# showlab/UniVTG

Measured on NVIDIA H100. Metric: video-query pairs/sec (fwd+bwd), higher is better.
Workload: dtype f16

## Files before the change

### __graft_entry__.py

```python
import os
import shutil
import subprocess
import sys

ROOT = os.path.dirname(os.path.abspath(__file__))
CSRC = os.path.join(ROOT, "univtg_b200", "csrc")
LIBDIR = os.path.join(ROOT, "univtg_b200", "lib")
LIB = os.path.join(LIBDIR, "libunivtg_b200.so")
SOURCES = ["gemm.cu", "rowops.cu", "attention.cu", "attention_bwd.cu", "backward.cu", "loss.cu", "optim.cu", "postproc.cu", "train.cu", "api.cu", "clip.cu",
           "hostio.cu", "metrics.cu", "task_eval.cu", "teacher.cu"]

NVCC_FLAGS = [
    "-gencode", "arch=compute_90a,code=sm_90a",
    "-lineinfo", "-O3", "-std=c++17",
    "-Xcompiler", "-fPIC",
    "--expt-relaxed-constexpr",
]


def _nvcc():
    for cand in (shutil.which("nvcc"), "/usr/local/cuda/bin/nvcc"):
        if cand and os.path.exists(cand):
            return cand
    raise RuntimeError("nvcc not found: the univtg_b200 CUDA library cannot be built")


def _needs_rebuild(srcs):
    if not os.path.exists(LIB):
        return True
    t = os.path.getmtime(LIB)
    deps = list(srcs)
    for f in os.listdir(CSRC):
        if f.endswith((".h", ".cuh")):
            deps.append(os.path.join(CSRC, f))
    deps.append(os.path.join(ROOT, "include", "univtg_b200.h"))
    return any(os.path.getmtime(d) > t for d in deps)


def build(force=False, verbose=False):
    srcs = [os.path.join(CSRC, s) for s in SOURCES if os.path.exists(os.path.join(CSRC, s))]
    if force or _needs_rebuild(srcs):
        os.makedirs(LIBDIR, exist_ok=True)
        nvcc = _nvcc()
        objs = []
        procs = []
        for s in srcs:
            o = os.path.join(LIBDIR, os.path.basename(s) + ".o")
            objs.append(o)
            cmd = [nvcc] + NVCC_FLAGS + ["-c", s, "-o", o]
            if verbose:
                cmd.insert(1, "-Xptxas")
                cmd.insert(2, "-v")
            procs.append((cmd, subprocess.Popen(cmd, stdout=subprocess.PIPE, stderr=subprocess.STDOUT, text=True)))
        for cmd, p in procs:
            out, _ = p.communicate()
            if verbose or p.returncode != 0:
                sys.stdout.write(out)
            if p.returncode != 0:
                raise RuntimeError("nvcc failed: " + " ".join(cmd))
        link = [nvcc, "-shared", "-gencode", "arch=compute_90a,code=sm_90a", "-o", LIB] + objs
        subprocess.check_call(link)
        for o in objs:
            os.remove(o)
    sys.path.insert(0, ROOT)
    import univtg_b200

    univtg_b200.load_library()


def smoke():
    sys.path.insert(0, ROOT)
    import torch

    assert torch.cuda.is_available(), "smoke() needs a GPU"
    from oracle import univtg_oracle as O
    from univtg_b200 import build_model, synth
    from univtg_b200.optim import FlatAdamW

    cfg = dict(synth.CONFIGS["tiny"], nheads=2, hidden_dim=256)
    args = synth.reference_args(cfg, device="cuda:0")
    model, crit = build_model(args)
    sd = synth.make_state_dict(cfg, seed=3)
    model.load_state_dict(sd, strict=True)
    model.to("cuda:0").eval()
    crit.to("cuda:0")
    inp = synth.make_inputs(cfg, seed=4, ragged=True)
    cinp = {k: v.cuda() for k, v in inp.items()}
    with torch.no_grad():
        out = model(**cinp)
    torch.cuda.synchronize()
    emu = O.forward(sd, cfg, **inp, opq=O.round_fp16)
    exact = O.forward(sd, cfg, **inp)
    for k in ("pred_logits", "pred_spans", "saliency_scores"):
        got = out[k].double().cpu()
        torch.testing.assert_close(got, emu[k], rtol=1e-4, atol=2e-5, msg=lambda m: f"smoke {k} vs fp16-emulating oracle: {m}")
        torch.testing.assert_close(got, exact[k], rtol=1e-3, atol=1e-4, msg=lambda m: f"smoke {k} vs exact oracle: {m}")

    tgt = synth.make_targets(inp, seed=5)
    ctgt = {k: (v.cuda() if torch.is_tensor(v) else v) for k, v in tgt.items()}
    model.train()
    crit.train()
    model.reference_rng_order = True
    model.keep_last_draw = True
    opt = FlatAdamW(model, lr=1e-3, weight_decay=1e-2, max_grad_norm=0.1)
    before = [p.detach().clone() for p in model._abi_params()]
    torch.manual_seed(11)
    tout = model(**cinp)
    loss = crit(tout, ctgt)
    total = crit.weighted_total(loss)
    opt.zero_grad()
    total.backward()
    grads = [p.grad.detach().clone() for p in model._abi_params()]
    opt.step()
    torch.cuda.synchronize()
    scales, masks = model._last_draw
    leaves = {k: v.double().requires_grad_(True) for k, v in sd.items()}
    oout = O.forward(leaves, cfg, **inp, dp_scale=scales.cpu(), drop_masks=[m.cpu() for m in masks])
    oloss = O.criterion(oout, tgt)
    O.weighted_total(oloss, crit.weight_dict).backward()
    for k, v in oloss.items():
        assert abs(float(loss[k]) - float(v)) <= 2e-3 * max(1.0, abs(float(v))), f"smoke train {k}: {float(loss[k])} vs oracle {float(v)}"
    named = dict(model.named_parameters())
    for n_ in ("transformer.encoder.layers.1.linear1.weight", "transformer.encoder.layers.0.self_attn.in_proj_weight",
               "input_vid_proj.0.net.1.weight", "span_embed.layers.1.weight", "class_embed.layers.2.weight"):
        g, og = named[n_].grad.double().cpu(), leaves[n_].grad
        rel = float((g - og).norm() / og.norm())
        assert rel < 8e-2, f"smoke train gradient {n_}: rel-L2 {rel:.3e} vs oracle autograd"
    ref_params = [b.clone().requires_grad_(True) for b in before]
    for rp, g in zip(ref_params, grads):
        rp.grad = g.clone()
    torch.nn.utils.clip_grad_norm_(ref_params, 0.1)
    ref_opt = torch.optim.AdamW(ref_params, lr=1e-3, weight_decay=1e-2)
    ref_opt.step()
    for p, rp in zip(model._abi_params(), ref_params):
        torch.testing.assert_close(p.detach(), rp.detach(), rtol=2e-5, atol=2e-7, msg=lambda m: f"smoke AdamW update: {m}")
    print("smoke ok:", {k: tuple(v.shape) for k, v in out.items()}, "train losses", {k: round(float(v), 5) for k, v in loss.items()})


if __name__ == "__main__":
    build(force="--force" in sys.argv, verbose="-v" in sys.argv)
    print("built", LIB)
```

### include/univtg_b200.h

```cpp
#ifndef UNIVTG_B200_H_
#define UNIVTG_B200_H_

#include <stddef.h>
#include <stdint.h>

#ifdef __cplusplus
extern "C" {
#endif

#define UNIVTG_ABI_VERSION 2
#define UNIVTG_ADAMW_SCRATCH_FLOATS 2048

typedef struct univtg_config {
  int32_t hidden_dim;
  int32_t nheads;
  int32_t dim_feedforward;
  int32_t enc_layers;
  int32_t n_input_proj;
  int32_t v_feat_dim;
  int32_t t_feat_dim;
  int32_t operand_format;
} univtg_config;

typedef struct univtg_shape {
// ... 48 lines not shown
  const float* table;
  int32_t max_q_l;
  const float* ln_weight;
  const float* ln_bias;
  const float* drop_mul;
  void* scratch;
} univtg_txt_pos;
int univtg_plan_set_txt_pos(univtg_plan* plan, const univtg_txt_pos* txt_pos);
size_t univtg_txt_pos_scratch_bytes(const univtg_config* cfg, const univtg_shape* shape);

int univtg_backward(univtg_plan* plan, void* train_ws, const float* src_txt, const float* src_vid, const float* droppath_scale,
                    const float* const* drop_masks, const univtg_rng* rng, const float* g_logits, const float* g_spans,
                    const float* g_vid_mem_proj, const float* g_txt_mem_proj, float grad_scale, float* const* grads,
                    int32_t n_grads, void* stream);

int univtg_backward_stages(const univtg_config* cfg, int32_t* ranges, int32_t max_stages);
int univtg_plan_set_backward_sm_budget(univtg_plan* plan, int32_t num_sms);
int univtg_plan_set_grad_events(univtg_plan* plan, void* const* events, int32_t n);

size_t univtg_loss_scratch_bytes(int32_t B, int32_t Lv);
int univtg_loss_forward(const float* pred_logits, const float* pred_spans, const float* vid_mem_proj, const float* txt_mem_proj,
                        const float* timestamp, const float* timestamp_mask, const float* timestamp_window,
                        const float* span_labels_nn, const float* saliency_scores, const int64_t* saliency_pos_idx, int32_t B,
                        int32_t Lv, int32_t d, float eos_coef, float temperature, float* losses5, void* scratch, void* stream);
int univtg_loss_backward(const float* w5, const float* vid_mem_proj, const float* txt_mem_proj, const int64_t* saliency_pos_idx,
                         int32_t B, int32_t Lv, int32_t d, const void* scratch, float* d_logits, float* d_spans,
                         float* d_vid_mem_proj, float* d_txt_mem_proj, void* stream);

int univtg_qfvs_loss_forward(const float* pred_logits, const float* vid_mem_proj, const float* txt_mem_proj, const float* src_vid_mask,
                             const uint8_t* mask_gt, const float* saliency_scores, int32_t has_pos_labels, int32_t B, int32_t Lv,
                             int32_t d, float temperature, float* losses5, void* scratch, void* stream);
int univtg_qfvs_loss_backward(const float* w5, const float* vid_mem_proj, const float* txt_mem_proj, int32_t B, int32_t Lv,
                              int32_t d, void* scratch, float* d_logits, float* d_vid_mem_proj, float* d_txt_mem_proj, void* stream);

int univtg_forward_num_launches(const univtg_plan* plan);
int64_t univtg_launch_count(void);

int univtg_plan_set_profiling(univtg_plan* plan, int32_t enable);
int univtg_plan_read_profile(univtg_plan* plan, float* ms, int32_t* kinds, int32_t cap);


int univtg_op_gemm(const void* a, const void* b, int32_t M, int32_t N, int32_t K, int32_t a_mn, int32_t b_mn, int32_t fmt,
                   int32_t bn, int32_t ksplit, const float* bias, int32_t act, float alpha, float* out32, void* out16,
                   void* stream);
int univtg_op_gemm_cluster(const void* a, const void* b, int32_t M, int32_t N, int32_t K, int32_t a_mn, int32_t b_mn,
                           int32_t fmt, int32_t bn, int32_t ksplit, const float* bias, int32_t act, float alpha, float* out32,
                           void* out16, void* stream);
typedef struct univtg_gemm_problem {
  const void* a;
  int32_t lda, a_mn;
  const void* b;
  int32_t ldb, b_mn;
  int32_t M, N, K, ksplit;
  int32_t a_fmt, b_fmt, out_fmt;
  int32_t conv, tap;
  const float* bias;
  int32_t act;
  float alpha;
  const float* row_scale;
  int32_t rps_in, rps_out, row_off, zero_sep, skip_sep;
  const float* resid;
  int32_t ld_resid;
  const float* addtab;
  int32_t ld_addtab;
  float* out32;
  int32_t ld32;
  float* out32_id;
  int32_t ld32_id;
  void* out16;
  void* out16p;
  int32_t ld16, accumulate;
  const void* mask16;
  int32_t ld_mask, mask_mul;
  void* dact16;
  int32_t ld_dact;
  float* colsum;
  float colsum_scale;
  int32_t vec_ok;
} univtg_gemm_problem;
int univtg_op_gemm_group(univtg_gemm_problem* problems, int32_t num, int32_t fmt, int32_t bn, int32_t cluster, int32_t* full,
                         void* stream);

typedef struct univtg_ln_bwd {
  const float* dout;
  int32_t ld_dout;
  const float* y;
  int32_t ld_y;
  const void* y16;
  int32_t y_fmt;
  const float* mean;
  const float* rstd;
  const float* gamma;
  int32_t rows, d;
  const float* row_scale;
  int32_t L, relu_mask_y;
  float* dy32;
  void* dbr16;
  int32_t ld16, fmt16;
  float* dgamma;
  float* dbeta;
  float* colsum;
  float pgrad_scale;
  const float* dout_mul;
} univtg_ln_bwd;
int univtg_op_layernorm_bwd(const univtg_ln_bwd* args, const univtg_rng* rng, int32_t mask_index, int32_t* kernel_used, void* stream);

typedef struct univtg_head_final_bwd {
  const float* g_logits;
  const float* g_spans;
  const float* pred_logits;
  const float* pred_spans;
  const void* h_cls;
  const void* h_span;
  const float* w_cls;
  const float* w_span;
  float* dz;
  void* dh_cls;
  void* dh_span;
  float* gw_cls;
  float* gb_cls;
  float* gw_span;
  float* gb_span;
  float* cs_cls;
  float* cs_span;
  float in_scale, pgrad_scale;
  int32_t B, Lv, d, fmt_act, fmt_grad;
} univtg_head_final_bwd;
int univtg_op_head_final_bwd(const univtg_head_final_bwd* args, void* stream);
int univtg_op_colsum16(const void* in16, int32_t ld, int32_t rows, int32_t cols, int32_t fmt, float* colsum, float scale, void* txt16,
                       int32_t L, int32_t Lv, int32_t txt_cols, void* stream);
int univtg_op_cvt16_colsum(const float* in32, int32_t ld_in, void* out16, int32_t ld_out, int32_t rows, int32_t cols, int32_t fmt,
                           float* colsum, float colsum_scale, void* txt16, int32_t L, int32_t Lv, int32_t txt_cols, void* stream);
int univtg_op_stream_gather(const float* dx, int32_t L, int32_t off, const float* extra, float extra_scale, void* out16, float* colsum,
                            float colsum_scale, int32_t B, int32_t Ls, int32_t d, int32_t fmt, void* stream);
int univtg_op_pool_bwd(const float* x_txt, const float* alpha, const float* w, const float* g_pooled, float* dx_txt, float* gw,
                       float out_scale, int32_t B, int32_t Lt, int32_t d, void* stream);
typedef struct univtg_txt_pos_bwd {
  const float* dpos;
  const float* xt;
  const float* table;
  const float* gamma;
  const float* mean;
  const float* rstd;
  const float* mul32;
  float* dx;
  float* dtable;
  float* dgamma;
  float* dbeta;
  float pgrad_scale;
  int32_t B, Lt, L, Lv, d;
} univtg_txt_pos_bwd;
int univtg_op_txt_pos_bwd(const univtg_txt_pos_bwd* args, const univtg_rng* rng, int32_t mask_index, void* stream);
int univtg_debug_gemm_timeline(void* buf);
int univtg_debug_choose_tile(const int32_t* Ms, const int32_t* Ns, const int32_t* kblocks, int32_t num, int32_t num_sms, int32_t step,
                             int32_t max_split, int32_t* bn, int32_t* ksplit);
int univtg_adamw_step(float* params, float* grads, float* exp_avg, float* exp_avg_sq, size_t n, float lr, float beta1,
                      float beta2, float eps, float weight_decay, int32_t step, float max_grad_norm,
                      int32_t write_clipped_grads, float* scratch3, const univtg_config* cfg, void* packed, void* stream);
int univtg_adamw_step_dev(float* params, float* grads, float* exp_avg, float* exp_avg_sq, size_t n, const float* lr_dev,
                          float beta1, float beta2, float eps, float weight_decay, int32_t* step_dev, float max_grad_norm,
                          int32_t write_clipped_grads, float* scratch3, const univtg_config* cfg, void* packed,
                          const float* bc_table, int32_t table_len, void* stream);
int univtg_adamw_bias_table(float beta1, float beta2, int32_t len, float* out_host);
int32_t univtg_adamw_bias_table_len(float beta1, float beta2);
int univtg_pack_vectors(const univtg_config* cfg, const float* const* params, int32_t n_params, void* packed, void* stream);

int univtg_host_assemble_batch(void* dst_vid, void* dst_txt, float* dst_vmask, float* dst_tmask, const void* src_vid,
                               const void* src_txt, const int64_t* vid_row0, const int64_t* txt_row0, const int32_t* vid_len,
                               const int32_t* txt_len, int32_t B, int32_t Lv, int32_t Lt, int32_t Dv, int32_t Dt, int32_t threads);

int univtg_host_register(void* base, size_t bytes, int32_t enable);
int univtg_h2d_gather_batch(void* dev_vid, void* dev_txt, float* dev_vmask, float* dev_tmask, float* mask_stage, const void* src_vid,
                            const void* src_txt, const int64_t* vid_row0, const int64_t* txt_row0, const int32_t* vid_len,
                            const int32_t* txt_len, int32_t B, int32_t Lv, int32_t Lt, int32_t Dv, int32_t Dt, void* stream);

int univtg_decode_mr(const float* pred_logits, const float* pred_spans, const float* timestamp, const float* timestamp_mask,
                     const float* duration, int32_t B, int32_t Lv, int32_t sort, float* windows, double* windows_r4, int32_t* order,
                     void* stream);
int univtg_temporal_nms(const double* windows, int32_t B, int32_t n, int32_t max_before_nms, double nms_thd, int32_t max_after_nms,
                        double* out, int32_t* counts, void* stream);

int univtg_eval_mr(const double* pred, const int32_t* n_pred, const double* gt, const int32_t* n_gt, int32_t Q, int32_t G, double* ap,
                   double* iou_r1, double* iou_r5, uint8_t* kept, void* stream);
int univtg_eval_hl(const double* sal, const int32_t* n_sal, const uint16_t* labels, const int32_t* n_clips, int32_t Q, int32_t S,
                   int32_t C, double* scratch, double* ap, double* hit, void* stream);

int univtg_eval_hl_topk(const float* scores, const int32_t* n_score, const int32_t* n_cut, const float* labels,
                        const int32_t* n_label, int32_t V, int32_t S, int32_t C, int32_t A, int32_t median, double* ap,
                        void* stream);
int univtg_qfvs_match(const uint64_t* a, const int32_t* a_off, const uint64_t* b, const int32_t* b_off, int32_t Q,
                      int32_t max_side, double* s, void* stream);

int univtg_op_layernorm(const float* in, int32_t rows, int32_t d, const float* gamma, const float* beta, float eps,
                        int32_t fmt, float* out32, void* out16, int32_t ld16, void* stream);
int univtg_op_attention(const void* qkv, const float* key_mask, void* out, float* lse, int32_t B, int32_t L, int32_t H,
                        int32_t dh, int32_t fmt, int32_t impl, void* stream);

typedef struct univtg_ln_fwd {
  const float* in;
  const void* in16;
  int32_t in_fmt, ld_in;
  const void* add16;
  int32_t ld_add16;
  float* sum_out;
  int32_t rows, d;
  const float* gamma;
  const float* beta;
  float eps;
  int32_t fmt;
  int64_t lo;
  int32_t L, Lv;
  float* out32;
  void* out16;
  void* out16p;
  int32_t ld16;
  const float* pos;
  const float* pos_txt;
  void* outc;
  const float* mul32;
  float* mean_out;
  float* rstd_out;
} univtg_ln_fwd;
int univtg_op_layernorm_fwd(const univtg_ln_fwd* args, const univtg_rng* rng, int32_t mask_index, int32_t* kernel_used, void* stream);

typedef struct univtg_txt_pos_fwd {
  const float* xt;
  const float* table;
  const float* gamma;
  const float* beta;
  const float* mul32;
  float* pos;
  float* mean_out;
  float* rstd_out;
  void* xpos16;
  int32_t B, Lt, L, Lv, d, fmt;
  int64_t lo;
} univtg_txt_pos_fwd;
int univtg_op_txt_pos(const univtg_txt_pos_fwd* args, const univtg_rng* rng, int32_t mask_index, void* stream);

int univtg_op_sine_pos(const float* vid_mask, const float* txt_mask, const float* dim_t, float* pos, float* key_mask, int32_t B, int32_t Lv,
                       int32_t Lt, int32_t d, const univtg_rng* rng, int32_t n_sites, float* dp_out, void* stream);

int univtg_op_pool_saliency(const float* x_txt, const float* x_vid, const float* txt_mask, const float* vid_mask, const float* w,
                            float* pooled, float* saliency, float* alpha_out, float* logits, int32_t B, int32_t Lt, int32_t Lv, int32_t d,
                            void* stream);

int univtg_op_conv_head_final(const void* h_cls, const void* h_span, const float* w_cls, const float* w_span, const float* b_cls,
                              const float* b_span, float* pred_logits, float* pred_spans, int32_t B, int32_t Lv, int32_t d, int32_t fmt,
                              void* stream);

typedef struct univtg_attn_fwd {
  const void* qkv;
  const float* key_mask;
  void* out;
  float* lse;
  int32_t B, L, H, dh, fmt, impl, causal;
} univtg_attn_fwd;
int univtg_op_attention_fwd(const univtg_attn_fwd* args, const univtg_rng* rng, float p, int32_t layer, int32_t* kernel_used, void* stream);

int univtg_op_attention_bwd(const void* qkv, const void* dO, const void* O, const float* key_mask, const float* lse,
                            float* delta_ws, float* dqkv32, int32_t B, int32_t L, int32_t H, int32_t dh, int32_t fmt_act,
                            int32_t impl, void* stream);

int univtg_op_attn_delta(const void* dO, int32_t fmt_do, const void* O, int32_t fmt_o, float* delta, int32_t B, int32_t L, int32_t H,
                         int32_t dh, int32_t* vec_used, void* stream);

typedef struct univtg_attn_bwd {
  const void* qkv;
  const void* dO;
  const float* key_mask;
  const float* lse;
  const float* delta;
  float* dqkv32;
  void* dqkv16;
  int32_t B, L, H, dh, fmt, impl;
} univtg_attn_bwd;
int univtg_op_attention_bwd_full(const univtg_attn_bwd* args, const univtg_rng* rng, float p, int32_t layer, int32_t* kernel_used,
                                 int32_t* dq_mode, void* stream);

typedef struct univtg_clip_config {
  int32_t embed_dim;
  int32_t vision_width;
  int32_t vision_layers;
  int32_t patch_size;
  int32_t image_resolution;
  int32_t text_width;
  int32_t text_layers;
  int32_t context_length;
  int32_t vocab_size;
  int32_t operand_format;
} univtg_clip_config;
int univtg_clip_num_params(const univtg_clip_config* cfg);
size_t univtg_clip_packed_bytes(const univtg_clip_config* cfg);
int univtg_clip_pack_weights(const univtg_clip_config* cfg, const void* const* params, int32_t n_params, int32_t src_dtype,
                             void* packed, void* stream);
size_t univtg_clip_workspace_bytes(const univtg_clip_config* cfg, int32_t n_images, int32_t n_texts, int32_t text_len);
int univtg_clip_encode_image(const univtg_clip_config* cfg, const void* packed, const void* pixels, int32_t pixel_kind, int32_t n,
                             void* ws, size_t ws_bytes, float* out, void* stream);
int univtg_clip_encode_text(const univtg_clip_config* cfg, const void* packed, const int64_t* tokens, int32_t n, int32_t ctx_used,
                            void* ws, size_t ws_bytes, float* last_hidden, float* pooled, void* stream);
int univtg_clip_num_launches(const univtg_clip_config* cfg, int32_t tower, int32_t text_outputs);

size_t univtg_teacher_class_bytes(int32_t C, int32_t D);
int univtg_teacher_prepare_classes(const float* cls, int32_t C, int32_t D, void* cls_ws, void* stream);
size_t univtg_teacher_chunk_bytes(int32_t V, int64_t S, int32_t C, int32_t D);
int univtg_teacher_label(const float* cls, const void* cls_ws, int32_t C, int32_t D, const float* feats, const int32_t* offsets,
// ... 8 lines not shown
```

### univtg_b200/_lib.py

```python
import ctypes
import os

_HERE = os.path.dirname(os.path.abspath(__file__))
LIB_PATH = os.environ.get("UNIVTG_LIB") or os.path.join(_HERE, "lib", "libunivtg_b200.so")
_lib = None

c_int = ctypes.c_int32
c_void_p = ctypes.c_void_p
c_size_t = ctypes.c_size_t
c_float = ctypes.c_float


class Config(ctypes.Structure):

    _fields_ = [
        ("hidden_dim", c_int),
        ("nheads", c_int),
        ("dim_feedforward", c_int),
        ("enc_layers", c_int),
        ("n_input_proj", c_int),
        ("v_feat_dim", c_int),
        ("t_feat_dim", c_int),
        ("operand_format", c_int),
    ]
# ... 7 lines not shown
class Rng(ctypes.Structure):

    _fields_ = [("seed", ctypes.c_uint64), ("input_dropout", c_float), ("droppath", c_float)]


class TxtPos(ctypes.Structure):

    _fields_ = [("table", c_void_p), ("max_q_l", c_int), ("ln_weight", c_void_p), ("ln_bias", c_void_p), ("drop_mul", c_void_p),
                ("scratch", c_void_p)]


class GemmProblem(ctypes.Structure):

    _fields_ = [("a", c_void_p), ("lda", c_int), ("a_mn", c_int), ("b", c_void_p), ("ldb", c_int), ("b_mn", c_int), ("M", c_int),
                ("N", c_int), ("K", c_int), ("ksplit", c_int), ("a_fmt", c_int), ("b_fmt", c_int), ("out_fmt", c_int), ("conv", c_int),
                ("tap", c_int), ("bias", c_void_p), ("act", c_int), ("alpha", c_float), ("row_scale", c_void_p), ("rps_in", c_int),
                ("rps_out", c_int), ("row_off", c_int), ("zero_sep", c_int), ("skip_sep", c_int), ("resid", c_void_p),
                ("ld_resid", c_int), ("addtab", c_void_p), ("ld_addtab", c_int), ("out32", c_void_p), ("ld32", c_int),
                ("out32_id", c_void_p), ("ld32_id", c_int), ("out16", c_void_p), ("out16p", c_void_p), ("ld16", c_int),
                ("accumulate", c_int), ("mask16", c_void_p), ("ld_mask", c_int), ("mask_mul", c_int), ("dact16", c_void_p),
                ("ld_dact", c_int), ("colsum", c_void_p), ("colsum_scale", c_float), ("vec_ok", c_int)]


class LnBwd(ctypes.Structure):

    _fields_ = [("dout", c_void_p), ("ld_dout", c_int), ("y", c_void_p), ("ld_y", c_int), ("y16", c_void_p), ("y_fmt", c_int),
                ("mean", c_void_p), ("rstd", c_void_p), ("gamma", c_void_p), ("rows", c_int), ("d", c_int), ("row_scale", c_void_p),
                ("L", c_int), ("relu_mask_y", c_int), ("dy32", c_void_p), ("dbr16", c_void_p), ("ld16", c_int), ("fmt16", c_int),
                ("dgamma", c_void_p), ("dbeta", c_void_p), ("colsum", c_void_p), ("pgrad_scale", c_float), ("dout_mul", c_void_p)]


class HeadFinalBwd(ctypes.Structure):

    _fields_ = [(n, c_void_p) for n in ("g_logits", "g_spans", "pred_logits", "pred_spans", "h_cls", "h_span", "w_cls", "w_span", "dz",
                                        "dh_cls", "dh_span", "gw_cls", "gb_cls", "gw_span", "gb_span", "cs_cls", "cs_span")] + \
        [("in_scale", c_float), ("pgrad_scale", c_float), ("B", c_int), ("Lv", c_int), ("d", c_int), ("fmt_act", c_int), ("fmt_grad", c_int)]


class TxtPosBwd(ctypes.Structure):

    _fields_ = [(n, c_void_p) for n in ("dpos", "xt", "table", "gamma", "mean", "rstd", "mul32", "dx", "dtable", "dgamma", "dbeta")] + \
        [("pgrad_scale", c_float), ("B", c_int), ("Lt", c_int), ("L", c_int), ("Lv", c_int), ("d", c_int)]


class LnFwd(ctypes.Structure):

    _fields_ = [("in_", c_void_p), ("in16", c_void_p), ("in_fmt", c_int), ("ld_in", c_int), ("add16", c_void_p), ("ld_add16", c_int),
                ("sum_out", c_void_p), ("rows", c_int), ("d", c_int), ("gamma", c_void_p), ("beta", c_void_p), ("eps", c_float),
                ("fmt", c_int), ("lo", ctypes.c_int64), ("L", c_int), ("Lv", c_int), ("out32", c_void_p), ("out16", c_void_p),
                ("out16p", c_void_p), ("ld16", c_int), ("pos", c_void_p), ("pos_txt", c_void_p), ("outc", c_void_p), ("mul32", c_void_p),
                ("mean_out", c_void_p), ("rstd_out", c_void_p)]


class TxtPosFwd(ctypes.Structure):

    _fields_ = [(n, c_void_p) for n in ("xt", "table", "gamma", "beta", "mul32", "pos", "mean_out", "rstd_out", "xpos16")] + \
        [(n, c_int) for n in ("B", "Lt", "L", "Lv", "d", "fmt")] + [("lo", ctypes.c_int64)]


class AttnFwd(ctypes.Structure):

    _fields_ = [("qkv", c_void_p), ("key_mask", c_void_p), ("out", c_void_p), ("lse", c_void_p)] + \
        [(n, c_int) for n in ("B", "L", "H", "dh", "fmt", "impl", "causal")]


class AttnBwd(ctypes.Structure):

    _fields_ = [(n, c_void_p) for n in ("qkv", "dO", "key_mask", "lse", "delta", "dqkv32", "dqkv16")] + \
        [(n, c_int) for n in ("B", "L", "H", "dh", "fmt", "impl")]


class ClipConfig(ctypes.Structure):

    _fields_ = [(n, c_int) for n in ("embed_dim", "vision_width", "vision_layers", "patch_size", "image_resolution", "text_width",
                                     "text_layers", "context_length", "vocab_size", "operand_format")]


SIGNATURES = {
    "univtg_last_error": (ctypes.c_char_p, []),
    "univtg_abi_version": (c_int, []),
    "univtg_num_params": (c_int, [ctypes.POINTER(Config)]),
    "univtg_packed_bytes": (c_size_t, [ctypes.POINTER(Config)]),
    "univtg_pack_weights": (c_int, [ctypes.POINTER(Config), ctypes.POINTER(c_void_p), c_int, c_void_p, c_void_p]),
    "univtg_workspace_bytes": (c_size_t, [ctypes.POINTER(Config), ctypes.POINTER(Shape)]),
    "univtg_prepare_workspace": (c_int, [ctypes.POINTER(Config), ctypes.POINTER(Shape), c_void_p, c_int, c_void_p]),
    "univtg_plan_create": (c_int, [ctypes.POINTER(Config), ctypes.POINTER(Shape), c_void_p, c_void_p, c_void_p, c_void_p,
                                   ctypes.POINTER(c_void_p)]),
    "univtg_plan_destroy": (None, [c_void_p]),
    "univtg_forward": (c_int, [c_void_p] * 12),
    "univtg_forward_num_launches": (c_int, [c_void_p]),
    "univtg_launch_count": (ctypes.c_int64, []),
    "univtg_host_register": (c_int, [c_void_p, c_size_t, c_int]),
    "univtg_h2d_gather_batch": (c_int, [c_void_p] * 11 + [c_int, c_int, c_int, c_int, c_int, c_void_p]),
    "univtg_host_assemble_batch": (c_int, [c_void_p, c_void_p, c_void_p, c_void_p, c_void_p, c_void_p, c_void_p, c_void_p, c_void_p,
                                           c_void_p, c_int, c_int, c_int, c_int, c_int, c_int]),
    "univtg_train_workspace_bytes": (c_size_t, [ctypes.POINTER(Config), ctypes.POINTER(Shape)]),
    "univtg_forward_train": (c_int, [c_void_p, c_void_p, c_void_p, c_void_p, c_void_p, c_void_p, c_void_p,
                                     ctypes.POINTER(c_void_p), ctypes.POINTER(Rng), c_void_p, c_void_p, c_void_p, c_void_p, c_void_p,
                                     c_void_p]),
    "univtg_backward": (c_int, [c_void_p, c_void_p, c_void_p, c_void_p, c_void_p, ctypes.POINTER(c_void_p), ctypes.POINTER(Rng),
                                c_void_p, c_void_p, c_void_p, c_void_p, c_float, ctypes.POINTER(c_void_p), c_int, c_void_p]),
    "univtg_dropout_mask": (c_int, [ctypes.POINTER(Rng), c_int, c_size_t, c_size_t, c_void_p, c_void_p]),
    "univtg_droppath_scales": (c_int, [ctypes.POINTER(Rng), c_int, c_int, c_void_p, c_void_p]),
    "univtg_plan_set_attention_dropout": (c_int, [c_void_p, c_float]),
    "univtg_plan_set_txt_pos": (c_int, [c_void_p, ctypes.POINTER(TxtPos)]),
    "univtg_txt_pos_scratch_bytes": (c_size_t, [ctypes.POINTER(Config), ctypes.POINTER(Shape)]),
    "univtg_attention_dropout_mask": (c_int, [ctypes.POINTER(Rng), c_float, c_int, c_int, c_int, c_int, c_void_p, c_void_p]),
    "univtg_loss_scratch_bytes": (c_size_t, [c_int, c_int]),
    "univtg_loss_forward": (c_int, [c_void_p] * 10 + [c_int, c_int, c_int, c_float, c_float, c_void_p, c_void_p, c_void_p]),
    "univtg_loss_backward": (c_int, [c_void_p, c_void_p, c_void_p, c_void_p, c_int, c_int, c_int, c_void_p, c_void_p, c_void_p,
                                     c_void_p, c_void_p, c_void_p]),
    "univtg_qfvs_loss_forward": (c_int, [c_void_p] * 6 + [c_int, c_int, c_int, c_int, c_float, c_void_p, c_void_p, c_void_p]),
    "univtg_qfvs_loss_backward": (c_int, [c_void_p, c_void_p, c_void_p, c_int, c_int, c_int, c_void_p, c_void_p, c_void_p, c_void_p,
                                          c_void_p]),
    "univtg_backward_stages":(c_int, [ctypes.POINTER(Config), c_void_p, c_int]),
    "univtg_plan_set_grad_events": (c_int, [c_void_p, ctypes.POINTER(c_void_p), c_int]),
    "univtg_plan_set_backward_sm_budget": (c_int, [c_void_p, c_int]),
    "univtg_decode_mr": (c_int, [c_void_p, c_void_p, c_void_p, c_void_p, c_void_p, c_int, c_int, c_int, c_void_p, c_void_p, c_void_p,
                                 c_void_p]),
    "univtg_temporal_nms": (c_int, [c_void_p, c_int, c_int, c_int, ctypes.c_double, c_int, c_void_p, c_void_p, c_void_p]),
    "univtg_eval_mr": (c_int, [c_void_p] * 4 + [c_int, c_int] + [c_void_p] * 5),
    "univtg_eval_hl": (c_int, [c_void_p] * 4 + [c_int, c_int, c_int] + [c_void_p] * 4),
    "univtg_eval_hl_topk": (c_int, [c_void_p] * 5 + [c_int] * 5 + [c_void_p, c_void_p]),
    "univtg_qfvs_match": (c_int, [c_void_p] * 4 + [c_int, c_int, c_void_p, c_void_p]),
    "univtg_adamw_step": (c_int, [c_void_p, c_void_p, c_void_p, c_void_p, ctypes.c_size_t, c_float, c_float, c_float, c_float,
                                  c_float, c_int, c_float, c_int, c_void_p, ctypes.POINTER(Config), c_void_p, c_void_p]),
    "univtg_pack_vectors": (c_int, [ctypes.POINTER(Config), ctypes.POINTER(c_void_p), c_int, c_void_p, c_void_p]),
    "univtg_adamw_step_dev": (c_int, [c_void_p, c_void_p, c_void_p, c_void_p, ctypes.c_size_t, c_void_p, c_float, c_float, c_float,
                                      c_float, c_void_p, c_float, c_int, c_void_p, ctypes.POINTER(Config), c_void_p, c_void_p, c_int,
                                      c_void_p]),
    "univtg_adamw_bias_table": (c_int, [c_float, c_float, c_int, c_void_p]),
    "univtg_adamw_bias_table_len": (c_int, [c_float, c_float]),
    "univtg_plan_set_seed_source": (c_int, [c_void_p, c_void_p]),
    "univtg_rng_advance": (c_int, [ctypes.c_uint64, c_void_p, c_void_p, c_void_p]),
    "univtg_rng_seed_at": (ctypes.c_uint64, [ctypes.c_uint64, ctypes.c_uint64]),
    "univtg_plan_set_profiling": (c_int, [c_void_p, c_int]),
    "univtg_plan_set_input_format": (c_int, [c_void_p, c_int]),
    "univtg_plan_read_profile": (c_int, [c_void_p, c_void_p, c_void_p, c_int]),
    "univtg_op_gemm": (c_int, [c_void_p, c_void_p, c_int, c_int, c_int, c_int, c_int, c_int, c_int, c_int, c_void_p, c_int,
                               c_float, c_void_p, c_void_p, c_void_p]),
    "univtg_op_gemm_cluster": (c_int, [c_void_p, c_void_p, c_int, c_int, c_int, c_int, c_int, c_int, c_int, c_int, c_void_p, c_int,
                                       c_float, c_void_p, c_void_p, c_void_p]),
    "univtg_op_gemm_group": (c_int, [ctypes.POINTER(GemmProblem), c_int, c_int, c_int, c_int, c_void_p, c_void_p]),
    "univtg_op_layernorm_bwd": (c_int, [ctypes.POINTER(LnBwd), ctypes.POINTER(Rng), c_int, c_void_p, c_void_p]),
    "univtg_op_head_final_bwd": (c_int, [ctypes.POINTER(HeadFinalBwd), c_void_p]),
    "univtg_op_colsum16": (c_int, [c_void_p, c_int, c_int, c_int, c_int, c_void_p, c_float, c_void_p, c_int, c_int, c_int, c_void_p]),
    "univtg_op_cvt16_colsum": (c_int, [c_void_p, c_int, c_void_p, c_int, c_int, c_int, c_int, c_void_p, c_float, c_void_p, c_int, c_int,
                                       c_int, c_void_p]),
    "univtg_op_stream_gather": (c_int, [c_void_p, c_int, c_int, c_void_p, c_float, c_void_p, c_void_p, c_float, c_int, c_int, c_int,
                                        c_int, c_void_p]),
    "univtg_op_pool_bwd": (c_int, [c_void_p] * 6 + [c_float, c_int, c_int, c_int, c_void_p]),
    "univtg_op_txt_pos_bwd": (c_int, [ctypes.POINTER(TxtPosBwd), ctypes.POINTER(Rng), c_int, c_void_p]),
    "univtg_debug_gemm_timeline": (c_int, [c_void_p]),
    "univtg_debug_choose_tile": (c_int, [c_void_p, c_void_p, c_void_p, c_int, c_int, c_int, c_int, c_void_p, c_void_p]),
    "univtg_op_layernorm": (c_int, [c_void_p, c_int, c_int, c_void_p, c_void_p, c_float, c_int, c_void_p, c_void_p, c_int,
                                    c_void_p]),
    "univtg_op_attention": (c_int, [c_void_p, c_void_p, c_void_p, c_void_p, c_int, c_int, c_int, c_int, c_int, c_int,
                                    c_void_p]),
    "univtg_op_attention_bwd": (c_int, [c_void_p] * 7 + [c_int, c_int, c_int, c_int, c_int, c_int, c_void_p]),
    "univtg_op_attn_delta": (c_int, [c_void_p, c_int, c_void_p, c_int, c_void_p, c_int, c_int, c_int, c_int, c_void_p, c_void_p]),
    "univtg_op_attention_bwd_full": (c_int, [ctypes.POINTER(AttnBwd), ctypes.POINTER(Rng), c_float, c_int, c_void_p, c_void_p,
                                             c_void_p]),
    "univtg_op_layernorm_fwd": (c_int, [ctypes.POINTER(LnFwd), ctypes.POINTER(Rng), c_int, c_void_p, c_void_p]),
    "univtg_op_txt_pos": (c_int, [ctypes.POINTER(TxtPosFwd), ctypes.POINTER(Rng), c_int, c_void_p]),
    "univtg_op_sine_pos": (c_int, [c_void_p] * 5 + [c_int, c_int, c_int, c_int, ctypes.POINTER(Rng), c_int, c_void_p, c_void_p]),
    "univtg_op_pool_saliency": (c_int, [c_void_p] * 9 + [c_int, c_int, c_int, c_int, c_void_p]),
    "univtg_op_conv_head_final": (c_int, [c_void_p] * 8 + [c_int, c_int, c_int, c_int, c_void_p]),
    "univtg_op_attention_fwd": (c_int, [ctypes.POINTER(AttnFwd), ctypes.POINTER(Rng), c_float, c_int, c_void_p, c_void_p]),
    "univtg_clip_num_params": (c_int, [ctypes.POINTER(ClipConfig)]),
    "univtg_clip_packed_bytes": (c_size_t, [ctypes.POINTER(ClipConfig)]),
    "univtg_clip_pack_weights": (c_int, [ctypes.POINTER(ClipConfig), ctypes.POINTER(c_void_p), c_int, c_int, c_void_p, c_void_p]),
    "univtg_clip_workspace_bytes": (c_size_t, [ctypes.POINTER(ClipConfig), c_int, c_int, c_int]),
    "univtg_clip_encode_image": (c_int, [ctypes.POINTER(ClipConfig), c_void_p, c_void_p, c_int, c_int, c_void_p, c_size_t, c_void_p,
                                         c_void_p]),
    "univtg_clip_encode_text": (c_int, [ctypes.POINTER(ClipConfig), c_void_p, c_void_p, c_int, c_int, c_void_p, c_size_t, c_void_p,
                                        c_void_p, c_void_p]),
    "univtg_clip_num_launches": (c_int, [ctypes.POINTER(ClipConfig), c_int, c_int]),
    "univtg_teacher_class_bytes": (c_size_t, [c_int, c_int]),
    "univtg_teacher_prepare_classes": (c_int, [c_void_p, c_int, c_int, c_void_p, c_void_p]),
    "univtg_teacher_chunk_bytes": (c_size_t, [c_int, ctypes.c_int64, c_int, c_int]),
    "univtg_teacher_label": (c_int, [c_void_p, c_void_p, c_int, c_int, c_void_p, c_void_p, c_int, ctypes.c_int64, c_int,
                                     ctypes.c_double, c_void_p, c_size_t, c_void_p, c_void_p]),
    "univtg_debug_py_floordiv": (c_int, [c_void_p, ctypes.c_int64, ctypes.c_double, c_void_p]),
}


def load_library():
    global _lib
    if _lib is not None:
        return _lib
    if not os.path.exists(LIB_PATH):
        raise RuntimeError(
            f"{LIB_PATH} not found: build it with `python __graft_entry__.py` (nvcc, sm_90a). "
            "univtg_b200 has no CPU or PyTorch fallback.")
    lib = ctypes.CDLL(LIB_PATH)
    for name, (res, args) in SIGNATURES.items():
        fn = getattr(lib, name)
        fn.restype = res
        fn.argtypes = args
    if lib.univtg_abi_version() != 2:
        raise RuntimeError("univtg_b200: ABI version mismatch between header and library")
    _lib = lib
    return lib


def last_error():
    lib = load_library()
    msg = lib.univtg_last_error()
    return msg.decode() if msg else ""


def check(rc, what):
    if rc != 0:
        raise RuntimeError(f"univtg_b200: {what} failed (rc={rc}): {last_error()}")


def ptr(t):
    if t is None:
        return None
    return c_void_p(t.data_ptr())


def stream_ptr():
    import torch

    return c_void_p(torch.cuda.current_stream().cuda_stream)
```

### univtg_b200/csrc/api.cu

```cuda
#include <math.h>
#include <stdio.h>
#include <string.h>

#include <new>
#include <vector>

#include "plan.h"
#include "ptx.cuh"

extern "C" {

const char* univtg_last_error(void) { return uv::last_error(); }
int univtg_abi_version(void) { return UNIVTG_ABI_VERSION; }

int univtg_num_params(const univtg_config* cfg) {
  if (!check_cfg(cfg)) return -1;
  return ParamIndex(*cfg).count();
}

size_t univtg_packed_bytes(const univtg_config* cfg) {
  if (!check_cfg(cfg)) return 0;
  return planes(*cfg) * make_layout(*cfg).total;
}

// ... 620 lines not shown
      if (l == c.enc_layers - 1) a.outc = W.hA;
      rc = marked(launch_layernorm(a, st), 0);
      if (rc) return rc;
    }
  }

  auto conv_problem = [&](GemmProblem& p, const uint16_t* A, int lda, const uint16_t* Wc, int N, const float* bias, uint16_t* out,
                          int ldo, int bn) -> int {
    const int r = conv_fwd_problem(p, P->Mh, A, lda, d, Wc, N, bn, ws_lo, pk_lo);
    p.bias = bias;
    p.act = ACT_RELU;
    p.rps_in = Lv + 1;
    p.rps_out = Lv + 1;
    p.row_off = 1;
    p.zero_sep = 1;
    p.out16 = out;
    p.ld16 = ldo;
    return r;
  };
  group(1);
  rc = conv_problem(g.p[0], W.hA, d, W16(Lw.conv1_w), 2 * d, F32(Lw.conv1_b), W.h1, 2 * d, P->bn_conv1);
  if (rc) return rc;
  rc = marked(launch_gemm_group(g, P->bn_conv1, sms, st), 1);
  if (rc) return rc;
  group(2);
  rc |= conv_problem(g.p[0], W.h1, 2 * d, W16(Lw.conv2c_w), d, F32(Lw.conv2c_b), W.hc2, d, P->bn_conv2);
  rc |= conv_problem(g.p[1], W.h1 + d, 2 * d, W16(Lw.conv2s_w), d, F32(Lw.conv2s_b), W.hs2, d, P->bn_conv2);
  if (rc) return rc;
  rc = marked(launch_gemm_group(g, P->bn_conv2, sms, st), 1);
  if (rc) return rc;
  {
    HeadFinalArgs a;
    a.h_cls = W.hc2;
    a.h_span = W.hs2;
    a.w_cls = F32(Lw.conv3c_w);
    a.w_span = F32(Lw.conv3s_w);
    a.b_cls = F32(Lw.conv3c_b);
    a.b_span = F32(Lw.conv3s_b);
    a.pred_logits = pred_logits;
    a.pred_spans = pred_spans;
    a.B = P->B;
    a.Lv = Lv;
    a.d = d;
    a.fmt = fmt;
    a.split = split;
    a.lo = ws_lo;
    rc = marked(launch_conv_head_final(a, st), 0);
    if (rc) return rc;
  }
  {
    PoolSalArgs a;
    a.x_txt = W.txtproj32;
    a.x_vid = vid_mem_proj;
    a.txt_mask = src_txt_mask;
    a.vid_mask = src_vid_mask;
    a.w = F32(Lw.pool_w);
    a.pooled = txt_mem_proj;
    a.saliency = saliency_scores;
    a.alpha_out = W.pool_alpha;
    a.logits_ws = W.pool_logits;
    a.B = P->B;
    a.Lt = Lt;
    a.Lv = Lv;
    a.d = d;
    rc = marked(launch_pool_saliency(a, st), 0);
    if (rc) return rc;
  }
  if (W.pred_logits) {
    cudaMemcpyAsync(W.pred_logits, pred_logits, (size_t)P->Mv * 4, cudaMemcpyDeviceToDevice, st);
    cudaMemcpyAsync(W.pred_spans, pred_spans, (size_t)P->Mv * 8, cudaMemcpyDeviceToDevice, st);
  }
  return 0;
}

extern "C" {

int univtg_forward(univtg_plan* P, const float* src_txt, const float* src_txt_mask, const float* src_vid,
                   const float* src_vid_mask, const float* droppath_scale, float* pred_logits, float* pred_spans,
                   float* vid_mem_proj, float* txt_mem_proj, float* saliency_scores, void* stream) {
  if (!P || !src_txt || !src_txt_mask || !src_vid || !src_vid_mask || !pred_logits || !pred_spans || !vid_mem_proj ||
      !txt_mem_proj || !saliency_scores) {
    set_error("univtg_forward: null argument");
    return 1;
  }
  return run_forward(P, make_infer_ws(P->cfg, P->shp, P->lay, P->ws), src_txt, src_txt_mask, src_vid, src_vid_mask, droppath_scale,
                     nullptr, nullptr, pred_logits, pred_spans, vid_mem_proj, txt_mem_proj, saliency_scores, (cudaStream_t)stream);
}

static int op_gemm_impl(const void* a, const void* b, int32_t M, int32_t N, int32_t K, int32_t a_mn, int32_t b_mn, int32_t fmt,
                        int32_t bn, int32_t ksplit, const float* bias, int32_t act, float alpha, float* out32, void* out16,
                        int32_t cluster, void* stream) {
  if (!a || !b || M < 1 || N < 1 || K < 1 || bn < 32 || bn > 256 || bn % 16 != 0) {
    set_error("univtg_op_gemm: bad argument");
    return 1;
  }
  if (cluster == 2 && b_mn) {
    set_error("univtg_op_gemm_cluster: cluster launches need a K-major B operand (b_mn = 0)");
    return 1;
  }
  const bool split = fmt == 2;
  if (split && (a_mn || b_mn || cluster == 2)) {
    set_error("univtg_op_gemm: fmt 2 (fp16x3) needs K-major A and B (a_mn = b_mn = 0) and no cluster");
    return 1;
  }
  if (split && ksplit > 1 && out16) {
    set_error("univtg_op_gemm: fmt 2 (fp16x3) out16 cannot be combined with ksplit > 1");
    return 1;
  }
  GemmGroup g;
  reset_group(g, 1, split ? 0 : fmt, split ? 1 : 0, split ? (long long)M * N : 0);
  g.cluster = cluster;
  GemmProblem& p = g.p[0];
  const uint16_t *a16 = reinterpret_cast<const uint16_t*>(a), *b16 = reinterpret_cast<const uint16_t*>(b);
  const Mat16 A = a_mn ? Mat16{a16, K, M, M} : Mat16{a16, M, K, K};
  const Mat16 Bm = b_mn ? Mat16{b16, K, N, N} : Mat16{b16, N, K, K};
  const int rc = setup_gemm(p, A, a_mn, Bm, b_mn, M, N, K, cluster == 2 ? bn / 2 : bn, split ? (long long)M * K : 0,
                            split ? (long long)N * K : 0);
  if (rc) return rc;
  p.ksplit = ksplit < 1 ? 1 : ksplit;
  p.bias = bias;
  p.act = act;
  p.alpha = alpha;
  p.out32 = out32;
  p.ld32 = N;
  p.out16 = reinterpret_cast<uint16_t*>(out16);
  p.ld16 = N;
  int dev = 0, sms = 0;
  cudaGetDevice(&dev);
  cudaDeviceGetAttribute(&sms, cudaDevAttrMultiProcessorCount, dev);
  return launch_gemm_group(g, bn, sms, (cudaStream_t)stream);
}

int univtg_op_gemm(const void* a, const void* b, int32_t M, int32_t N, int32_t K, int32_t a_mn, int32_t b_mn, int32_t fmt,
                   int32_t bn, int32_t ksplit, const float* bias, int32_t act, float alpha, float* out32, void* out16,
                   void* stream) {
  return op_gemm_impl(a, b, M, N, K, a_mn, b_mn, fmt, bn, ksplit, bias, act, alpha, out32, out16, 1, stream);
}

int univtg_op_gemm_cluster(const void* a, const void* b, int32_t M, int32_t N, int32_t K, int32_t a_mn, int32_t b_mn,
                           int32_t fmt, int32_t bn, int32_t ksplit, const float* bias, int32_t act, float alpha, float* out32,
                           void* out16, void* stream) {
  return op_gemm_impl(a, b, M, N, K, a_mn, b_mn, fmt, bn, ksplit, bias, act, alpha, out32, out16, 2, stream);
}

int univtg_debug_choose_tile(const int32_t* Ms, const int32_t* Ns, const int32_t* kblocks, int32_t num, int32_t num_sms, int32_t step,
                              int32_t max_split, int32_t* bn, int32_t* ksplit) {
  if (!Ms || !Ns || !kblocks || !bn || !ksplit || num < 1 || num > GEMM_MAX_GROUP || num_sms < 1 || (step != 16 && step != 64) || max_split < 1) {
    set_error("univtg_debug_choose_tile: bad argument");
    return 1;
  }
  const uv::TileChoice t = uv::choose_tile(Ms, Ns, kblocks, num, num_sms, step, max_split);
  *bn = t.bn;
  *ksplit = t.ksplit;
  return 0;
}

int univtg_debug_gemm_timeline(void* buf) {
  uv::set_gemm_timeline_buffer(reinterpret_cast<unsigned long long*>(buf));
  return 0;
}

int univtg_op_layernorm(const float* in, int32_t rows, int32_t d, const float* gamma, const float* beta, float eps,
                        int32_t fmt, float* out32, void* out16, int32_t ld16, void* stream) {
  if (!in || !gamma || !beta || rows < 1 || d < 1) {
    set_error("univtg_op_layernorm: bad argument");
    return 1;
  }
  LnArgs a;
  memset(&a, 0, sizeof(a));
  a.in = in;
  a.ld_in = d;
  a.rows = rows;
  a.d = d;
  a.gamma = gamma;
  a.beta = beta;
  a.eps = eps;
  a.fmt = fmt == 2 ? 0 : fmt;
  a.out32 = out32;
  a.out16 = reinterpret_cast<uint16_t*>(out16);
  a.ld16 = out16 ? ld16 : d;
  a.split = fmt == 2;
  a.lo = fmt == 2 ? (long long)rows * a.ld16 : 0;
  return launch_layernorm(a, (cudaStream_t)stream);
}

int univtg_op_layernorm_fwd(const univtg_ln_fwd* q, const univtg_rng* rng, int32_t mask_index, int32_t* kernel_used, void* stream) {
  const char* fn = "univtg_op_layernorm_fwd";
  UV_REQ(q != nullptr, "%s: null args", fn);
  UV_REQ((q->in || q->in16) && q->gamma && q->beta, "%s: null in / in16, gamma or beta", fn);
  UV_REQ(q->rows >= 1 && q->d >= 1, "%s: rows %d / d %d", fn, q->rows, q->d);
  UV_REQ(q->ld_in >= q->d, "%s: ld_in %d smaller than d %d", fn, q->ld_in, q->d);
  UV_REQ(!q->in16 || q->in_fmt == 0 || q->in_fmt == 1, "%s: in_fmt %d (0 fp16, 1 bf16)", fn, q->in_fmt);
  UV_REQ(q->fmt >= 0 && q->fmt <= 2, "%s: fmt %d (0 fp16, 1 bf16, 2 fp16x3)", fn, q->fmt);
  UV_REQ(!q->add16 || q->ld_add16 >= q->d, "%s: ld_add16 %d smaller than d %d", fn, q->ld_add16, q->d);
  UV_REQ(!q->add16 || q->d % 4 != 0 || q->ld_add16 % 4 == 0, "%s: ld_add16 %d must be a multiple of 4 (64-bit loads)", fn, q->ld_add16);
  UV_REQ(!q->sum_out || q->add16, "%s: sum_out needs add16", fn);
  UV_REQ(!(q->out16 || q->out16p) || q->ld16 >= q->d, "%s: ld16 %d smaller than d %d", fn, q->ld16, q->d);
  UV_REQ(q->L >= 0 && q->Lv >= 0 && q->Lv <= q->L && (q->L == 0 || q->rows % q->L == 0), "%s: L %d / Lv %d (rows %% L == 0)", fn, q->L,
         q->Lv);
  UV_REQ(!(q->pos || q->pos_txt || q->outc) || q->L >= 1, "%s: pos, pos_txt and outc need the token structure (L >= 1)", fn);
  UV_REQ(!q->pos || q->out16p, "%s: pos is only used with out16p", fn);
  UV_REQ(q->fmt != 2 || (q->lo > 0 && q->lo % 4 == 0), "%s: fmt 2 needs lo > 0, a multiple of 4", fn);
  UV_REQ(q->fmt != 2 || (!q->mul32 && !(rng && rng->input_dropout > 0.f)), "%s: fmt 2 (fp16x3) takes no dropout (mul32 / rng)", fn);
  UV_REQ(!rng || !(rng->input_dropout > 0.f) || mask_index >= 0, "%s: mask_index %d", fn, mask_index);
  UV_REQ(al_(q->in, 16) && al_(q->gamma, 16) && al_(q->beta, 16) && al_(q->sum_out, 16) && al_(q->out32, 16) && al_(q->pos, 16) &&
             al_(q->pos_txt, 16) && al_(q->mul32, 16) && al_(q->mean_out, 4) && al_(q->rstd_out, 4),
         "%s: fp32 pointers must be 16-byte aligned", fn);
  UV_REQ(al_(q->in16, 8) && al_(q->add16, 8) && al_(q->out16, 8) && al_(q->out16p, 8) && al_(q->outc, 8),
         "%s: in16, add16, out16, out16p and outc must be 8-byte aligned", fn);
  LnArgs a;
  memset(&a, 0, sizeof(a));
  a.in = q->in;
  a.ld_in = q->ld_in;
  a.in16 = reinterpret_cast<const uint16_t*>(q->in16);
  a.in_fmt = q->in_fmt;
  a.add16 = reinterpret_cast<const uint16_t*>(q->add16);
  a.ld_add16 = q->ld_add16;
  a.sum_out = q->sum_out;
  a.rows = q->rows;
  a.d = q->d;
  a.gamma = q->gamma;
  a.beta = q->beta;
  a.eps = q->eps;
  a.fmt = q->fmt == 2 ? 0 : q->fmt;
  a.split = q->fmt == 2;
  a.lo = q->fmt == 2 ? (long long)q->lo : 0;
  a.L = q->L;
  a.Lv = q->Lv;
  a.out32 = q->out32;
  a.out16 = reinterpret_cast<uint16_t*>(q->out16);
  a.out16p = reinterpret_cast<uint16_t*>(q->out16p);
  a.ld16 = (q->out16 || q->out16p) ? q->ld16 : q->d;
  a.pos = q->pos;
  a.pos_txt = q->pos_txt;
  a.outc = reinterpret_cast<uint16_t*>(q->outc);
  a.mul32 = q->mul32;
  if (!a.mul32 && rng && rng->input_dropout > 0.f) a.drop = make_drop_spec(rng->seed, (unsigned int)mask_index, rng->input_dropout);
  a.mean_out = q->mean_out;
  a.rstd_out = q->rstd_out;
  int used = -1;
  const int rc = launch_layernorm(a, (cudaStream_t)stream, &used);
  if (kernel_used) *kernel_used = used;
  return rc;
}

int univtg_op_txt_pos(const univtg_txt_pos_fwd* q, const univtg_rng* rng, int32_t mask_index, void* stream) {
  const char* fn = "univtg_op_txt_pos";
  UV_REQ(q != nullptr, "%s: null args", fn);
  UV_REQ(q->xt && q->table && q->gamma && q->beta && q->pos && q->xpos16, "%s: null xt, table, gamma, beta, pos or xpos16", fn);
  UV_REQ((q->mean_out == nullptr) == (q->rstd_out == nullptr), "%s: mean_out and rstd_out must both be given or both be NULL", fn);
  UV_REQ(q->B >= 1 && q->Lt >= 1 && q->Lv >= 0 && q->L >= q->Lv + q->Lt, "%s: B %d / Lt %d / L %d / Lv %d (L >= Lv + Lt)", fn, q->B,
         q->Lt, q->L, q->Lv);
  UV_REQ(q->fmt >= 0 && q->fmt <= 2, "%s: fmt %d (0 fp16, 1 bf16, 2 fp16x3)", fn, q->fmt);
  UV_REQ(q->fmt != 2 || (q->lo > 0 && q->lo % 2 == 0), "%s: fmt 2 needs lo > 0, a multiple of 2", fn);
  UV_REQ(q->fmt != 2 || (!q->mul32 && !(rng && rng->input_dropout > 0.f)), "%s: fmt 2 (fp16x3) takes no dropout (mul32 / rng)", fn);
  UV_REQ(!rng || !(rng->input_dropout > 0.f) || mask_index >= 0, "%s: mask_index %d", fn, mask_index);
  UV_REQ(al_(q->xt, 8) && al_(q->table, 8) && al_(q->gamma, 8) && al_(q->beta, 8) && al_(q->mul32, 8) && al_(q->pos, 8) &&
             al_(q->mean_out, 4) && al_(q->rstd_out, 4) && al_(q->xpos16, 4),
         "%s: fp32 pointers must be 8-byte and xpos16 4-byte aligned", fn);
  TxtPosArgs a;
  memset(&a, 0, sizeof(a));
  a.xt = q->xt;
  a.table = q->table;
  a.gamma = q->gamma;
  a.beta = q->beta;
  a.mul32 = q->mul32;
  if (!a.mul32 && rng && rng->input_dropout > 0.f) a.drop = make_drop_spec(rng->seed, (unsigned int)mask_index, rng->input_dropout);
  a.pos = q->pos;
  a.mean_out = q->mean_out;
  a.rstd_out = q->rstd_out;
  a.xpos16 = reinterpret_cast<uint16_t*>(q->xpos16);
  a.B = q->B;
  a.Lt = q->Lt;
  a.L = q->L;
  a.Lv = q->Lv;
  a.d = q->d;
  a.fmt = q->fmt == 2 ? 0 : q->fmt;
  a.split = q->fmt == 2;
  a.lo = q->fmt == 2 ? (long long)q->lo : 0;
  return launch_txt_pos(a, (cudaStream_t)stream);
}

int univtg_op_sine_pos(const float* vid_mask, const float* txt_mask, const float* dim_t, float* pos, float* key_mask, int32_t B, int32_t Lv,
                       int32_t Lt, int32_t d, const univtg_rng* rng, int32_t n_sites, float* dp_out, void* stream) {
  const char* fn = "univtg_op_sine_pos";
  UV_REQ(vid_mask && dim_t && pos, "%s: null vid_mask, dim_t or pos", fn);
  UV_REQ(B >= 1 && Lv >= 1 && Lv <= 12288 && Lt >= 0, "%s: B %d / Lv %d / Lt %d (1 <= Lv <= 12288)", fn, B, Lv, Lt);
  UV_REQ(d >= 2 && d % 2 == 0, "%s: d %d must be even (sin / cos column pairs)", fn, d);
  UV_REQ(!key_mask || Lt == 0 || txt_mask, "%s: key_mask needs txt_mask", fn);
  UV_REQ(!dp_out || (rng && n_sites >= 1), "%s: dp_out needs rng and n_sites >= 1", fn);
  UV_REQ(al_(pos, 8) && al_(vid_mask, 4) && al_(txt_mask, 4) && al_(dim_t, 4) && al_(key_mask, 4) && al_(dp_out, 4),
         "%s: pos must be 8-byte aligned", fn);
  return launch_sine_pos(vid_mask, txt_mask, dim_t, pos, key_mask, B, Lv, Lt, d, (cudaStream_t)stream, dp_out, dp_out ? n_sites : 0,
                         rng ? rng->seed : 0ull, rng ? 1.0f - rng->droppath : 1.f);
}

int univtg_op_pool_saliency(const float* x_txt, const float* x_vid, const float* txt_mask, const float* vid_mask, const float* w,
                            float* pooled, float* saliency, float* alpha_out, float* logits, int32_t B, int32_t Lt, int32_t Lv, int32_t d,
                            void* stream) {
  const char* fn = "univtg_op_pool_saliency";
  UV_REQ(x_txt && x_vid && txt_mask && vid_mask && w && pooled && saliency && logits, "%s: null pointer argument", fn);
  UV_REQ(B >= 1 && Lt >= 1 && Lt <= 12288 && Lv >= 1, "%s: B %d / Lt %d / Lv %d (1 <= Lt <= 12288)", fn, B, Lt, Lv);
  UV_REQ(d >= 4 && d % 4 == 0, "%s: d %d must be a positive multiple of 4 (128-bit loads)", fn, d);
  UV_REQ(al_(x_txt, 16) && al_(x_vid, 16) && al_(w, 16) && al_(pooled, 16) && al_(saliency, 4) && al_(alpha_out, 4) && al_(logits, 4) &&
             al_(txt_mask, 4) && al_(vid_mask, 4),
         "%s: x_txt, x_vid, w and pooled must be 16-byte aligned", fn);
// ... 117 lines not shown
```

### univtg_b200/csrc/gemm.cu

```cuda
#include <stdarg.h>
#include <stdio.h>
#include <stdlib.h>
#include <string.h>

#include "kernels.h"
#include "ptx.cuh"
#include "wgmma.cuh"

namespace uv {

template <int CL>
struct GemmCfg {
  static constexpr int kMaxStages = 8;
  static constexpr int kABytes = GEMM_BM * 128;
  static constexpr int kRingBytes = 4 * (kABytes + 256 * 128);
  static constexpr int kEpiStride = 36;
  static constexpr int kEpiFloats = 2 * 64 * kEpiStride;
  static constexpr int kSmemBytes = 1024  + kRingBytes + kEpiFloats * 4 + 256;
  __host__ __device__ static constexpr int stage_bytes(int bn) { return kABytes + bn * 128; }
  __host__ __device__ static constexpr int num_stages(int bn) {
    return kRingBytes / stage_bytes(bn) < kMaxStages ? kRingBytes / stage_bytes(bn) : kMaxStages;
  }
};

constexpr int kGemmThreads = 384;

struct TileInfo {
  int p, m_blk, n_blk, kb0, kb1, split;
};

template <int CL, bool SPLIT>
__device__ __forceinline__ bool decode_tile(const GemmGroup& g, int bn, int t, int rank, TileInfo& ti) {
  for (int p = 0; p < g.num; ++p) {
    const GemmProblem& pr = g.p[p];
    const int tm_real = (pr.M + GEMM_BM - 1) / GEMM_BM;
    const int tm = (tm_real + CL - 1) / CL;
    const int tn = (pr.N + bn - 1) / bn;
    const int cnt = tm * tn * pr.ksplit;
    if (t < cnt) {
      ti.p = p;
      ti.n_blk = t % tn;
      const int rest = t / tn;
      ti.m_blk = (rest % tm) * CL + rank;
      ti.split = rest / tm;
      const int total_kb = pr.taps * pr.kblk_per_tap * (SPLIT ? 3 : 1);
      const int per = (total_kb + pr.ksplit - 1) / pr.ksplit;
      ti.kb0 = ti.split * per;
      ti.kb1 = min(total_kb, ti.kb0 + per);
      return true;
    }
    t -= cnt;
  }
  return false;
}

__device__ __forceinline__ void stamp(unsigned long long* dbg, int slot) {
  if (dbg != nullptr) {
    unsigned long long t;
    asm volatile("mov.u64 %0, %globaltimer;" : "=l"(t));
    dbg[(size_t)blockIdx.x * 8 + slot] = t;
  }
}

template <int N, int OFF, int BF, int TA, int TB>
__device__ __forceinline__ void mma_cols(float* acc, uint64_t da, uint64_t db, uint32_t scale_d) {
  constexpr int W = N >= 256 ? 256 : N >= 128 ? 128 : N >= 64 ? 64 : N >= 32 ? 32 : 16;
  WG<W, BF>::template ss<TA, TB>(acc + OFF / 2, da, db, scale_d);
  if constexpr (N > W) {
    constexpr uint32_t adv = TB ? (W / 64) * 8192 / 16 : W * 128 / 16;
    mma_cols<N - W, OFF + W, BF, TA, TB>(acc, da, db + adv, scale_d);
  }
}

struct Ring {
  uint8_t* base;
  uint64_t* full;
  uint64_t* empty;
  int stage_bytes, stages;
  int stage;
  uint32_t phase;
};

template <int CL>
__device__ __forceinline__ void release_stage(const Ring& ring, int s, int tid, int crank) {
  if (tid == 0) {
    mbar_arrive(&ring.empty[s]);
    if (CL > 1) mbar_arrive_cluster(mapa_shared(smem_u32(&ring.empty[s]), (uint32_t)(crank ^ 1)));
  }
}

template <int CL, int BN, int BF, int TA, int TB>
__device__ __forceinline__ void tile_mainloop(float* acc, Ring& ring, int kb0, int kb1, int cw, int tid, int crank) {
  const uint64_t da_hi = TA ? make_smem_desc_sw128(0, 8192, 1024) : make_smem_desc_sw128(0, 16, 1024);
  const uint64_t db_hi = TB ? make_smem_desc_sw128(0, 8192, 1024) : make_smem_desc_sw128(0, 16, 1024);
  constexpr uint32_t a_step = TA ? 128u : 2u, b_step = TB ? 128u : 2u;
  int prev = -1;
  for (int kb = kb0; kb < kb1; ++kb) {
    mbar_wait(&ring.full[ring.stage], ring.phase);
    const uint32_t sa = smem_u32(ring.base + ring.stage * ring.stage_bytes);
    const uint64_t da = da_hi + (uint64_t)((sa + cw * 8192) >> 4);
    const uint64_t db = db_hi + (uint64_t)((sa + GemmCfg<CL>::kABytes) >> 4);
    wgmma_fence();
#pragma unroll
    for (int k = 0; k < GEMM_BK / 16; ++k)
      mma_cols<BN, 0, BF, TA, TB>(acc, da + k * a_step, db + k * b_step, (kb > kb0 || k > 0) ? 1u : 0u);
    wgmma_commit();
    wgmma_wait<1>();
    if (prev >= 0) release_stage<CL>(ring, prev, tid, crank);
    prev = ring.stage;
    if (++ring.stage == ring.stages) {
      ring.stage = 0;
      ring.phase ^= 1;
    }
  }
  wgmma_wait<0>();
#pragma unroll
  for (int i = 0; i < BN / 2; ++i) reg_fence(acc[i]);
  if (prev >= 0) release_stage<CL>(ring, prev, tid, crank);
}

template <int CL, bool SPLIT, int BN>
__device__ __forceinline__ void tile_mainloop_any(float* acc, Ring& ring, int bf, int a_mn, int b_mn, int kb0, int kb1, int cw, int tid,
                                                  int crank) {
  if constexpr (SPLIT) {
    tile_mainloop<CL, BN, 0, 0, 0>(acc, ring, kb0, kb1, cw, tid, crank);
  } else {
    if constexpr (CL == 1 && BN % 64 == 0) {
      if (b_mn) {
        if (bf) {
          if (a_mn) tile_mainloop<CL, BN, 1, 1, 1>(acc, ring, kb0, kb1, cw, tid, crank);
          else tile_mainloop<CL, BN, 1, 0, 1>(acc, ring, kb0, kb1, cw, tid, crank);
        } else {
          if (a_mn) tile_mainloop<CL, BN, 0, 1, 1>(acc, ring, kb0, kb1, cw, tid, crank);
          else tile_mainloop<CL, BN, 0, 0, 1>(acc, ring, kb0, kb1, cw, tid, crank);
        }
        return;
      }
    }
    if (bf) {
      if (a_mn) tile_mainloop<CL, BN, 1, 1, 0>(acc, ring, kb0, kb1, cw, tid, crank);
      else tile_mainloop<CL, BN, 1, 0, 0>(acc, ring, kb0, kb1, cw, tid, crank);
    } else {
      if (a_mn) tile_mainloop<CL, BN, 0, 1, 0>(acc, ring, kb0, kb1, cw, tid, crank);
      else tile_mainloop<CL, BN, 0, 0, 0>(acc, ring, kb0, kb1, cw, tid, crank);
    }
  }
}

struct EpiRow {
  bool valid;
  float rsc;
  const float* resid_row;
  const float* aux_row;
  const uint16_t* mask_row;
  const float* add_row;
  float* o32_row;
  float* o32i_row;
  uint16_t* o16_row;
  uint16_t* o16p_row;
  float* pre_row;
  uint16_t* dact_row;
};

__device__ __forceinline__ void ld16f(const float* p, float (&v)[16]) {
#pragma unroll
  for (int q = 0; q < 4; ++q) {
    const float4 t4 = reinterpret_cast<const float4*>(p)[q];
    v[4 * q] = t4.x; v[4 * q + 1] = t4.y; v[4 * q + 2] = t4.z; v[4 * q + 3] = t4.w;
  }
}

template <bool FULL, bool SPLIT>
__device__ __forceinline__ void epi_step(const GemmProblem& pr, const EpiRow& r, float (&v)[16], int n0, int fmt, int lane,
                                         long long lo16) {
  const int pN = pr.N;
  const int act = pr.act;
  const int ofmt = pr.out_fmt < 0 ? fmt : pr.out_fmt;
  const bool vec = FULL ? pr.vec_ok != 0 : true;
  const bool atomic = (pr.accumulate != 0) || (pr.ksplit > 1);
  const bool mask_mul = FULL && pr.mask_mul != 0;
  const float rsc = r.rsc;
  if (FULL && r.pre_row != nullptr && r.valid) {
    if (vec) {
      st_global_256f(r.pre_row + n0, v[0], v[1], v[2], v[3], v[4], v[5], v[6], v[7]);
      st_global_256f(r.pre_row + n0 + 8, v[8], v[9], v[10], v[11], v[12], v[13], v[14], v[15]);
    } else {
#pragma unroll
      for (int q = 0; q < 4; ++q)
        if (n0 + 4 * q < pN)
          *reinterpret_cast<float4*>(r.pre_row + n0 + 4 * q) = make_float4(v[4 * q], v[4 * q + 1], v[4 * q + 2], v[4 * q + 3]);
    }
  }
  if (FULL && act == ACT_GELU && r.dact_row != nullptr) {
    float dg[16];
#pragma unroll
    for (int j = 0; j < 16; ++j) {
      float gj;
      gelu_erf_both(v[j], gj, dg[j]);
      v[j] = gj * rsc;
    }
    if (r.valid) {
      if (vec) {
        uint32_t w8[8];
#pragma unroll
        for (int q = 0; q < 8; ++q) w8[q] = cvt16x2(dg[2 * q], dg[2 * q + 1], ofmt);
        st_global_256(r.dact_row + n0, w8);
      } else {
#pragma unroll
        for (int j = 0; j < 16; ++j)
          if (n0 + j < pN) r.dact_row[n0 + j] = cvt16(dg[j], ofmt);
      }
    }
  } else if (act == ACT_GELU) {
#pragma unroll
    for (int j = 0; j < 16; ++j) v[j] = gelu_erf(v[j]) * rsc;
  } else if (act == ACT_RELU) {
#pragma unroll
    for (int j = 0; j < 16; ++j) v[j] = fmaxf(v[j], 0.f) * rsc;
  } else if (act == ACT_QUICKGELU) {
#pragma unroll
    for (int j = 0; j < 16; ++j) v[j] = v[j] / (1.f + expf(-1.702f * v[j])) * rsc;
  } else {
#pragma unroll
    for (int j = 0; j < 16; ++j) v[j] *= rsc;
  }
  if (vec) {
    if (r.valid) {
      if (r.resid_row != nullptr) {
        float rv[16];
        ld16f(r.resid_row + n0, rv);
#pragma unroll
        for (int j = 0; j < 16; ++j) v[j] += rv[j];
      }
      if (FULL && r.aux_row != nullptr) {
        float av[16];
        ld16f(r.aux_row + n0, av);
        if (pr.aux_mode == 1) {
#pragma unroll
          for (int j = 0; j < 16; ++j) v[j] *= gelu_erf_grad(av[j]);
        } else {
#pragma unroll
          for (int j = 0; j < 16; ++j) v[j] *= av[j];
        }
      }
      if (FULL && r.mask_row != nullptr) {
#pragma unroll
        for (int q = 0; q < 2; ++q) {
          const uint4 mk = reinterpret_cast<const uint4*>(r.mask_row + n0)[q];
          const uint32_t w4[4] = {mk.x, mk.y, mk.z, mk.w};
#pragma unroll
          for (int e = 0; e < 4; ++e) {
            if (mask_mul) {
              v[8 * q + 2 * e] *= ld16((uint16_t)(w4[e] & 0xffff), fmt);
              v[8 * q + 2 * e + 1] *= ld16((uint16_t)(w4[e] >> 16), fmt);
            } else {
              if (!pos16((uint16_t)(w4[e] & 0xffff))) v[8 * q + 2 * e] = 0.f;
              if (!pos16((uint16_t)(w4[e] >> 16))) v[8 * q + 2 * e + 1] = 0.f;
            }
          }
        }
      }
      if (r.o32_row != nullptr) {
        if (FULL && atomic) {
#pragma unroll
          for (int q = 0; q < 4; ++q)
            red_add_f32x4(r.o32_row + n0 + 4 * q, make_float4(v[4 * q], v[4 * q + 1], v[4 * q + 2], v[4 * q + 3]));
        } else {
          st_global_256f(r.o32_row + n0, v[0], v[1], v[2], v[3], v[4], v[5], v[6], v[7]);
          st_global_256f(r.o32_row + n0 + 8, v[8], v[9], v[10], v[11], v[12], v[13], v[14], v[15]);
        }
      }
      if ((FULL || SPLIT) && r.o32i_row != nullptr) {
        st_global_256f(r.o32i_row + n0, v[0], v[1], v[2], v[3], v[4], v[5], v[6], v[7]);
        st_global_256f(r.o32i_row + n0 + 8, v[8], v[9], v[10], v[11], v[12], v[13], v[14], v[15]);
      }
      if (r.o16_row != nullptr) {
        uint32_t w8[8];
#pragma unroll
        for (int q = 0; q < 8; ++q) w8[q] = cvt16x2(v[2 * q], v[2 * q + 1], ofmt);
        st_global_256(r.o16_row + n0, w8);
        if constexpr (SPLIT) {
#pragma unroll
          for (int q = 0; q < 8; ++q) w8[q] = cvt16x2_lo(v[2 * q], v[2 * q + 1]);
          st_global_256(r.o16_row + lo16 + n0, w8);
        }
      }
      if (r.o16p_row != nullptr) {
        float p[16];
#pragma unroll
        for (int j = 0; j < 16; ++j) p[j] = v[j];
        if (r.add_row != nullptr) {
          float av[16];
          ld16f(r.add_row + n0, av);
#pragma unroll
          for (int j = 0; j < 16; ++j) p[j] += av[j];
        }
        uint32_t w8[8];
#pragma unroll
        for (int q = 0; q < 8; ++q) w8[q] = cvt16x2(p[2 * q], p[2 * q + 1], ofmt);
        st_global_256(r.o16p_row + n0, w8);
        if constexpr (SPLIT) {
#pragma unroll
          for (int q = 0; q < 8; ++q) w8[q] = cvt16x2_lo(p[2 * q], p[2 * q + 1]);
          st_global_256(r.o16p_row + lo16 + n0, w8);
        }
      }
    } else {
#pragma unroll
      for (int j = 0; j < 16; ++j) v[j] = 0.f;
    }
  } else if constexpr (FULL) {
    const int cs32 = pr.cs32 > 1 ? pr.cs32 : 1;
#pragma unroll
    for (int j = 0; j < 16; ++j) {
      const int n = n0 + j;
      float x = v[j];
      if (r.valid && n < pN) {
        if (r.resid_row != nullptr) x += r.resid_row[n];
        if (r.aux_row != nullptr) x *= (pr.aux_mode == 1) ? gelu_erf_grad(r.aux_row[n]) : r.aux_row[n];
        if (r.mask_row != nullptr) {
          if (mask_mul) x *= ld16(r.mask_row[n], fmt);
          else if (!pos16(r.mask_row[n])) x = 0.f;
        }
        if (r.o32_row != nullptr) {
          float* dst = r.o32_row + (size_t)n * cs32;
          if (atomic) atomicAdd(dst, x);
          else *dst = x;
        }
        if (r.o32i_row != nullptr) r.o32i_row[n] = x;
        if (r.o16_row != nullptr) {
          r.o16_row[n] = cvt16(x, ofmt);
          if constexpr (SPLIT) r.o16_row[lo16 + n] = cvt16_lo(x);
        }
        if (r.o16p_row != nullptr) {
          const float xp = x + (r.add_row ? r.add_row[n] : 0.f);
          r.o16p_row[n] = cvt16(xp, ofmt);
          if constexpr (SPLIT) r.o16p_row[lo16 + n] = cvt16_lo(xp);
        }
      } else {
        x = 0.f;
      }
      v[j] = x;
    }
  }
  if (FULL && pr.colsum != nullptr) {
    const float sj = warp_colsum16(v, lane);
    if (lane < 16 && n0 + lane < pN) atomicAdd(pr.colsum + n0 + lane, sj * pr.colsum_scale);
  }
}

template <int CL, bool FULL, bool SPLIT, int BN>
__device__ __forceinline__ void consumer_tiles(const GemmGroup& g, Ring& ring, float* epi_buf, int tile0, int tstep, int crank, int cw,
                                               int lane) {
  using Cfg = GemmCfg<CL>;
  const int tid = threadIdx.x & 127;
  const int fr = 16 * (tid >> 5) + (lane >> 2);
  const int fc = 2 * (lane & 3);
  const int erow = tid & 63, ehalf = tid >> 6;
  float* ebuf = epi_buf + cw * 64 * Cfg::kEpiStride;
  const int fmt = g.fmt;
  float acc[BN / 2];
#pragma unroll
  for (int i = 0; i < BN / 2; ++i) acc[i] = 0.f;
  TileInfo ti;
  bool first_tile = true;
  for (int t = tile0; decode_tile<CL, SPLIT>(g, BN, t, crank, ti); t += tstep) {
    const GemmProblem& pr = g.p[ti.p];
    const int bf = pr.a_fmt < 0 ? fmt : pr.a_fmt;
    if (first_tile && g.dbg != nullptr && ti.kb0 < ti.kb1) {
      mbar_wait(&ring.full[ring.stage], ring.phase);
      if (tid == 0 && cw == 0) stamp(g.dbg, 3);
    }
    tile_mainloop_any<CL, SPLIT, BN>(acc, ring, bf, pr.a_mn, pr.b_mn, ti.kb0, ti.kb1, cw, tid, crank);
    if (tid == 0 && cw == 0) stamp(g.dbg, 4);
    first_tile = false;

    const int pM = pr.M, pN = pr.N, rps_in = pr.rps_in;
    const int m = ti.m_blk * GEMM_BM + cw * 64 + erow;
    int b = 0, l = m;
    if (rps_in > 0) {
      b = m / rps_in;
      l = m - b * rps_in;
    }
    const bool is_sep = (rps_in > 0) && (l == rps_in - 1);
    EpiRow r;
    r.valid = (m < pM) && !(pr.skip_sep && is_sep);
    r.rsc = pr.alpha;
    if (pr.row_scale != nullptr && m < pM) r.rsc *= pr.row_scale[b];
    if (pr.zero_sep && is_sep) r.rsc = 0.f;
    const size_t orow = (size_t)((rps_in > 0 ? b * pr.rps_out + l : m) + pr.row_off);
    r.resid_row = pr.resid ? pr.resid + orow * pr.ld_resid : nullptr;
    r.aux_row = (FULL && pr.aux32) ? pr.aux32 + orow * pr.ld_aux : nullptr;
    r.mask_row = (FULL && pr.mask16) ? pr.mask16 + orow * pr.ld_mask : nullptr;
    r.add_row = pr.addtab ? pr.addtab + (size_t)m * pr.ld_addtab : nullptr;
    r.o32_row = pr.out32 ? pr.out32 + orow * pr.ld32 : nullptr;
    r.o32i_row = ((FULL || SPLIT) && pr.out32_id) ? pr.out32_id + (size_t)m * pr.ld32_id : nullptr;
    r.o16_row = pr.out16 ? pr.out16 + orow * pr.ld16 : nullptr;
    r.o16p_row = pr.out16p ? pr.out16p + orow * pr.ld16 : nullptr;
    r.pre_row = (FULL && pr.pre32) ? pr.pre32 + orow * pr.ld_pre : nullptr;
    r.dact_row = (FULL && pr.dact16) ? pr.dact16 + orow * pr.ld_dact : nullptr;
    const float* __restrict__ bias = (ti.split == 0) ? pr.bias : nullptr;
    const int nt0 = ti.n_blk * BN;
#pragma unroll 1
    for (int cc = 0; cc < (BN + 31) / 32 && nt0 + cc * 32 < pN; ++cc) {
#pragma unroll
      for (int c = 0; c < (BN + 31) / 32; ++c) {
        if (c == cc) {
#pragma unroll
          for (int ii = 0; ii < 4; ++ii) {
            const int i = 4 * c + ii;
            if (8 * i < BN) {
              *reinterpret_cast<float2*>(ebuf + fr * Cfg::kEpiStride + 8 * ii + fc) = make_float2(acc[4 * i], acc[4 * i + 1]);
              *reinterpret_cast<float2*>(ebuf + (fr + 8) * Cfg::kEpiStride + 8 * ii + fc) = make_float2(acc[4 * i + 2], acc[4 * i + 3]);
            }
          }
        }
      }
      named_bar_sync(1 + cw, 128);
      const int n0 = nt0 + cc * 32 + ehalf * 16;
      if (cc * 32 + ehalf * 16 < BN && n0 < pN) {
        float v[16];
        ld16f(ebuf + erow * Cfg::kEpiStride + ehalf * 16, v);
        if (bias != nullptr) {
#pragma unroll
          for (int j = 0; j < 16; ++j) v[j] += (n0 + j < pN) ? __ldg(bias + n0 + j) : 0.f;
        }
        epi_step<FULL, SPLIT>(pr, r, v, n0, fmt, lane, g.lo16);
      }
      named_bar_sync(1 + cw, 128);
    }
    if (tid == 0 && cw == 1) stamp(g.dbg, 6);
  }
}

template <int CL, bool FULL, bool SPLIT = false>
__global__ void __launch_bounds__(kGemmThreads, 1) gemm_wgmma_kernel(const __grid_constant__ GemmGroup g) {
  using Cfg = GemmCfg<CL>;
  const int BN = g.bn;
  const int kStageBytes = Cfg::stage_bytes(BN);
  const int kStages = Cfg::num_stages(BN);
  const int crank = (CL > 1) ? (int)cluster_ctarank() : 0;
  const int tile0 = (CL > 1) ? (int)(blockIdx.x / CL) : (int)blockIdx.x;
  const int tstep = (int)(gridDim.x / CL);
  extern __shared__ __align__(1024) uint8_t smem_raw[];
  const uint32_t raw_addr = smem_u32(smem_raw);
  const uint32_t align_off = (1024u - (raw_addr & 1023u)) & 1023u;
  uint8_t* smem = smem_raw + align_off;

  uint8_t* stage_base = smem;
  float* epi_buf = reinterpret_cast<float*>(smem + Cfg::kRingBytes);
  uint64_t* bars = reinterpret_cast<uint64_t*>(epi_buf + Cfg::kEpiFloats);
  uint64_t* full_bar = bars;
  uint64_t* empty_bar = bars + Cfg::kMaxStages;

  const int warp = threadIdx.x >> 5;
  const int lane = threadIdx.x & 31;
  const int wg = threadIdx.x >> 7;
  if (threadIdx.x == 0) stamp(g.dbg, 0);

  if (warp == 8 && lane == 0) {
    for (int p = 0; p < g.num; ++p) {
      tma_prefetch_desc(&g.p[p].tm_a);
      tma_prefetch_desc(&g.p[p].tm_b);
    }
  }
  if (warp == 0 && lane == 0) {
    for (int s = 0; s < kStages; ++s) {
      mbar_init(&full_bar[s], 1);
      mbar_init(&empty_bar[s], 2 * CL);
    }
    fence_barrier_init();
  }
  __syncthreads();
  if (CL > 1) cluster_sync_all();
  pdl_launch_dependents();
  pdl_wait();
  if (threadIdx.x == 0) stamp(g.dbg, 1);

  if (wg == 2) {
    setmaxnreg_dec<40>();
    if (warp == 8) {
      int stage = 0;
      uint32_t phase = 0;
      TileInfo ti;
      for (int t = tile0; decode_tile<CL, SPLIT>(g, BN, t, crank, ti); t += tstep) {
        const GemmProblem& pr = g.p[ti.p];
        const int m0 = ti.m_blk * GEMM_BM;
        const int n0 = ti.n_blk * BN;
        for (int kb = ti.kb0; kb < ti.kb1; ++kb) {
          int kbt = kb, plane_a = 0, plane_b = 0;
          if constexpr (SPLIT) {
            const int per_product = pr.taps * pr.kblk_per_tap;
            const int prod = kb / per_product;
            kbt = kb - prod * per_product;
            plane_a = prod == 1;
            plane_b = prod == 2;
          }
          const int tap = kbt / pr.kblk_per_tap;
          const int kk = (kbt - tap * pr.kblk_per_tap) * GEMM_BK;
          mbar_wait(&empty_bar[stage], phase ^ 1);
          uint8_t* sa = stage_base + stage * kStageBytes;
          uint8_t* sb = sa + Cfg::kABytes;
          const int a0 = pr.ca.base0 + m0 * pr.ca.mn0s + tap * pr.ca.tap0 + kk * pr.ca.k0s;
          const int a1 = pr.ca.base1 + m0 * pr.ca.mn1s + tap * pr.ca.tap1 + kk * pr.ca.k1s;
          const int b0 = pr.cb.base0 + n0 * pr.cb.mn0s + tap * pr.cb.tap0 + kk * pr.cb.k0s;
          const int b1 = pr.cb.base1 + n0 * pr.cb.mn1s + tap * pr.cb.tap1 + kk * pr.cb.k1s;
          if (elect_one()) {
            mbar_arrive_expect_tx(&full_bar[stage], Cfg::kABytes + BN * 128);
            if constexpr (SPLIT) {
              tma_load_3d(sa, &pr.tm_a, &full_bar[stage], a0, a1, plane_a);
              tma_load_3d(sb, &pr.tm_b, &full_bar[stage], b0, b1, plane_b);
            } else if (!pr.a_mn) {
              tma_load_2d(sa, &pr.tm_a, &full_bar[stage], a0, a1);
            } else {
#pragma unroll
              for (int j = 0; j < GEMM_BM / 64; ++j) tma_load_2d(sa + j * 8192, &pr.tm_a, &full_bar[stage], a0 + 64 * j, a1);
            }
            if constexpr (SPLIT) {
            } else if (CL == 1) {
              if (!pr.b_mn) {
                tma_load_2d(sb, &pr.tm_b, &full_bar[stage], b0, b1);
              } else if (pr.b_3d) {
                tma_load_3d(sb, &pr.tm_b, &full_bar[stage], 0, b1, b0 >> 6);
              } else {
                for (int j = 0; j < BN / 64; ++j) tma_load_2d(sb + j * 8192, &pr.tm_b, &full_bar[stage], b0 + 64 * j, b1);
              }
            } else {
              const int hr = BN / 2;
              tma_load_2d_mc(sb + crank * hr * 128, &pr.tm_b, &full_bar[stage], b0, b1 + crank * hr, (uint16_t)0x3);
            }
          }
          __syncwarp();
          if (++stage == kStages) {
            stage = 0;
            phase ^= 1;
          }
        }
      }
      if (lane == 0) stamp(g.dbg, 2);
    }
  } else {
    setmaxnreg_inc<232>();
    Ring ring{stage_base, full_bar, empty_bar, kStageBytes, kStages, 0, 0u};
    switch (BN >> 4) {
#define UV_BN_CASE(k) \
  case k: consumer_tiles<CL, FULL, SPLIT, 16 * k>(g, ring, epi_buf, tile0, tstep, crank, wg, lane); break;
#define UV_BN_CASE_ODD(k) \
  case k: if constexpr (CL == 1) consumer_tiles<CL, FULL, SPLIT, 16 * k>(g, ring, epi_buf, tile0, tstep, crank, wg, lane); break;
      UV_BN_CASE(2) UV_BN_CASE_ODD(3) UV_BN_CASE(4) UV_BN_CASE_ODD(5) UV_BN_CASE(6) UV_BN_CASE_ODD(7) UV_BN_CASE(8)
      UV_BN_CASE_ODD(9) UV_BN_CASE(10) UV_BN_CASE_ODD(11) UV_BN_CASE(12) UV_BN_CASE_ODD(13) UV_BN_CASE(14) UV_BN_CASE_ODD(15)
      UV_BN_CASE(16)
#undef UV_BN_CASE_ODD
#undef UV_BN_CASE
      default: __trap();
    }
  }

  __syncthreads();
  if (CL > 1) cluster_sync_all();
  if (threadIdx.x == 0) stamp(g.dbg, 7);
}

static unsigned long long* g_timeline = nullptr;
void set_gemm_timeline_buffer(unsigned long long* buf) { g_timeline = buf; }
bool pdl_enabled() {
  static int on = -1;
  if (on < 0) {
    const char* e = getenv("UNIVTG_PDL");
    on = (e != nullptr && e[0] == '0') ? 0 : 1;
  }
  return on == 1;
}
long long* launch_counter() {
  static long long n = 0;
  return &n;
}
static thread_local char g_err[512] = "";
const char* last_error() { return g_err; }
void set_error(const char* fmt, ...) {
  va_list ap;
  va_start(ap, fmt);
  vsnprintf(g_err, sizeof(g_err), fmt, ap);
  va_end(ap);
}

typedef CUresult (*EncodeTiledFn)(CUtensorMap*, CUtensorMapDataType, cuuint32_t, void*, const cuuint64_t*, const cuuint64_t*,
                                  const cuuint32_t*, const cuuint32_t*, CUtensorMapInterleave, CUtensorMapSwizzle,
                                  CUtensorMapL2promotion, CUtensorMapFloatOOBfill);

static EncodeTiledFn get_encode_fn() {
  static EncodeTiledFn fn = nullptr;
  if (fn) return fn;
  void* p = nullptr;
  cudaDriverEntryPointQueryResult q;
  cudaError_t e = cudaGetDriverEntryPoint("cuTensorMapEncodeTiled", &p, cudaEnableDefault, &q);
  if (e != cudaSuccess || q != cudaDriverEntryPointSuccess || p == nullptr) {
    set_error("cuTensorMapEncodeTiled entry point unavailable (cudaError %d)", (int)e);
    return nullptr;
  }
  fn = reinterpret_cast<EncodeTiledFn>(p);
  return fn;
}

struct TmapKey {
  const void* base;
  uint64_t rows, cols, ld;
  uint32_t box_rows, box_cols, kind;
  uint64_t plane;
  bool operator==(const TmapKey& o) const {
    return base == o.base && rows == o.rows && cols == o.cols && ld == o.ld && box_rows == o.box_rows && box_cols == o.box_cols && kind == o.kind &&
           plane == o.plane;
  }
};
struct TmapSlot {
  TmapKey key;
  CUtensorMap map;
  bool used;
};
constexpr int kTmapCacheSlots = 4096;
static thread_local TmapSlot* g_tmap_cache = nullptr;
static inline TmapSlot* tmap_slot(const TmapKey& k) {
  if (g_tmap_cache == nullptr) g_tmap_cache = static_cast<TmapSlot*>(calloc(kTmapCacheSlots, sizeof(TmapSlot)));
  uint64_t h = reinterpret_cast<uintptr_t>(k.base) * 0x9E3779B97F4A7C15ull;
  h ^= (k.rows * 0xC2B2AE3D27D4EB4Full) ^ (k.cols << 17) ^ (k.ld << 29) ^ ((uint64_t)k.box_rows << 41) ^ ((uint64_t)k.box_cols << 47) ^ ((uint64_t)k.kind << 55);
  h ^= k.plane * 0x94D049BB133111EBull;
  h ^= h >> 29;
  return g_tmap_cache ? &g_tmap_cache[h & (kTmapCacheSlots - 1)] : nullptr;
}

static int make_tmap_cached(CUtensorMap* out, const TmapKey& key, cuuint32_t rank, const cuuint64_t* dims, const cuuint64_t* strides,
                            const cuuint32_t* box) {
  TmapSlot* slot = tmap_slot(key);
  if (slot != nullptr && slot->used && slot->key == key) {
    *out = slot->map;
    return 0;
  }
  EncodeTiledFn fn = get_encode_fn();
  if (!fn) return 1;
  const char* what = key.kind == 4 ? "fp16x3 pair" : key.kind == 3 ? "3-D MN-major B" : "2-D";
  bool aligned = (reinterpret_cast<uintptr_t>(key.base) & 15) == 0;
  for (cuuint32_t i = 0; i + 1 < rank; ++i) aligned = aligned && strides[i] % 16 == 0;
  if (!aligned) {
    set_error("tensor map (%s): base %p, pitch %llu B and lo-plane offset %llu B must be 16-byte aligned", what, key.base,
              (unsigned long long)(key.ld * 2), (unsigned long long)(key.plane * 2));
    return 2;
  }
  const cuuint32_t estr[3] = {1, 1, 1};
  CUresult r = fn(out, CU_TENSOR_MAP_DATA_TYPE_UINT16, rank, const_cast<void*>(key.base), dims, strides, box, estr,
                  CU_TENSOR_MAP_INTERLEAVE_NONE, CU_TENSOR_MAP_SWIZZLE_128B, CU_TENSOR_MAP_L2_PROMOTION_L2_256B,
                  CU_TENSOR_MAP_FLOAT_OOB_FILL_NONE);
  if (r != CUDA_SUCCESS) {
    set_error("cuTensorMapEncodeTiled (%s) failed: CUresult %d (rows %llu cols %llu ld %llu lo %llu box %ux%u)", what, (int)r,
              (unsigned long long)key.rows, (unsigned long long)key.cols, (unsigned long long)key.ld, (unsigned long long)key.plane,
              key.box_rows, key.box_cols);
    return 3;
  }
  if (slot != nullptr) {
    slot->key = key;
    slot->map = *out;
    slot->used = true;
  }
  return 0;
}

int make_tmap_2d(CUtensorMap* out, const void* base, uint64_t rows, uint64_t cols, uint64_t ld_elems, uint32_t box_rows,
                 uint32_t box_cols) {
  const cuuint64_t dims[2] = {cols, rows}, strides[1] = {ld_elems * 2};
  const cuuint32_t box[2] = {box_cols, box_rows};
  return make_tmap_cached(out, TmapKey{base, rows, cols, ld_elems, box_rows, box_cols, 2u, 0}, 2, dims, strides, box);
}

int make_tmap_split(CUtensorMap* out, const void* base, uint64_t rows, uint64_t cols, uint64_t ld_elems, uint32_t box_rows,
                    uint32_t box_cols, uint64_t lo_elems) {
  const cuuint64_t dims[3] = {cols, rows, 2}, strides[2] = {ld_elems * 2, lo_elems * 2};
  const cuuint32_t box[3] = {box_cols, box_rows, 1};
  return make_tmap_cached(out, TmapKey{base, rows, cols, ld_elems, box_rows, box_cols, 4u, lo_elems}, 3, dims, strides, box);
}

int make_tmap_b_mn(GemmProblem& p, const void* base, uint64_t rows, uint64_t cols, uint64_t ld_elems, int bn) {
  p.b_3d = 0;
  if (cols % 64 != 0 || bn % 64 != 0 || bn < 64) return make_tmap_2d(&p.tm_b, base, rows, cols, ld_elems, 64, 64);
  const cuuint64_t dims[3] = {64, rows, cols / 64}, strides[2] = {ld_elems * 2, 128};
  const cuuint32_t box[3] = {64, 64, (cuuint32_t)(bn / 64)};
  const int rc = make_tmap_cached(&p.tm_b, TmapKey{base, rows, cols, ld_elems, (uint32_t)bn, 64u, 3u, 0}, 3, dims, strides, box);
  if (rc == 0) p.b_3d = bn / 64;
  return rc;
}

int launch_gemm_group(GemmGroup& g, int bn, int num_sms, cudaStream_t stream, int* used_full) {
  using Cfg = GemmCfg<1>;
  static_assert(GemmCfg<1>::kSmemBytes == GemmCfg<2>::kSmemBytes, "both variants use the same dynamic shared memory size");
  if (g.num < 1 || g.num > GEMM_MAX_GROUP) {
    set_error("gemm group size %d out of range", g.num);
    return (int)cudaErrorInvalidValue;
  }
  if (bn < 32 || bn > 256 || bn % 16 != 0) {
    set_error("unsupported BN %d (multiple of 16 in [32, 256])", bn);
    return (int)cudaErrorInvalidValue;
  }
  const int cl = g.cluster == 2 ? 2 : 1;
  static bool attr_set = false;
  if (!attr_set) {
    cudaError_t e = cudaFuncSetAttribute(gemm_wgmma_kernel<1, true>, cudaFuncAttributeMaxDynamicSharedMemorySize, Cfg::kSmemBytes);
    if (e == cudaSuccess)
      e = cudaFuncSetAttribute(gemm_wgmma_kernel<1, false>, cudaFuncAttributeMaxDynamicSharedMemorySize, Cfg::kSmemBytes);
    if (e == cudaSuccess)
      e = cudaFuncSetAttribute(gemm_wgmma_kernel<2, true>, cudaFuncAttributeMaxDynamicSharedMemorySize, Cfg::kSmemBytes);
    if (e == cudaSuccess)
      e = cudaFuncSetAttribute(gemm_wgmma_kernel<2, false>, cudaFuncAttributeMaxDynamicSharedMemorySize, Cfg::kSmemBytes);
    if (e == cudaSuccess)
      e = cudaFuncSetAttribute(gemm_wgmma_kernel<1, false, true>, cudaFuncAttributeMaxDynamicSharedMemorySize, Cfg::kSmemBytes);
    if (e != cudaSuccess) {
      set_error("cudaFuncSetAttribute(gemm, smem=%d): %s", Cfg::kSmemBytes, cudaGetErrorString(e));
      return (int)e;
    }
    attr_set = true;
  }
  if (cl == 2 && (bn % 32 != 0)) {
    set_error("cluster GEMM needs BN %% 32 == 0 (got %d)", bn);
    return (int)cudaErrorInvalidValue;
  }
  if (g.split && (cl != 1 || g.fmt != 0)) {
    set_error("fp16x3 gemm group: needs cluster 1 and group format 0 (got cluster %d, fmt %d)", cl, g.fmt);
    return (int)cudaErrorInvalidValue;
  }
  int total = 0;
  for (int p = 0; p < g.num; ++p) {
    const GemmProblem& pr = g.p[p];
    if (g.split && (pr.a_mn || pr.b_mn || pr.a_fmt > 0 || pr.b_fmt > 0 || pr.out_fmt > 0)) {
      set_error("gemm problem %d: fp16x3 problems need K-major fp16 operands and output", p);
      return (int)cudaErrorInvalidValue;
    }
    if (pr.ksplit < 1 || pr.taps < 1 || pr.kblk_per_tap < 1 || pr.ksplit > pr.taps * pr.kblk_per_tap * (g.split ? 3 : 1)) {
      set_error("gemm problem %d: bad k configuration (taps %d kblk %d ksplit %d)", p, pr.taps, pr.kblk_per_tap, pr.ksplit);
      return (int)cudaErrorInvalidValue;
    }
    if (!pr.b_mn && pr.b_box_rows != bn / cl) {
      set_error("gemm problem %d: B tensor-map box has %d rows but the launch uses bn %d (cluster %d)", p, pr.b_box_rows, bn, cl);
      return (int)cudaErrorInvalidValue;
    }
    if (cl == 2 && pr.b_mn) {
      set_error("gemm problem %d: cluster launches need a K-major B operand", p);
      return (int)cudaErrorInvalidValue;
    }
    if (pr.b_mn && pr.b_3d != 0 && pr.b_3d != bn / 64) {
      set_error("gemm problem %d: 3-D B tensor map was built for bn %d (got bn %d)", p, 64 * pr.b_3d, bn);
      return (int)cudaErrorInvalidValue;
    }
    if (pr.b_mn && bn % (64 * cl) != 0) {
      set_error("gemm problem %d: MN-major B needs BN %% %d == 0 (got %d)", p, 64 * cl, bn);
      return (int)cudaErrorInvalidValue;
    }
    if (pr.ksplit > 1 || pr.accumulate) {
      const char* bad = pr.dact16 ? "dact16" : pr.act != ACT_NONE ? "act" : pr.resid ? "resid" : pr.out16 ? "out16"
                        : pr.out16p ? "out16p" : pr.out32_id ? "out32_id" : nullptr;
      if (bad != nullptr) {
        set_error("gemm problem %d: %s cannot be combined with %s (each split would apply it to a partial sum)", p, bad,
                  pr.ksplit > 1 ? "ksplit > 1" : "accumulate");
        return (int)cudaErrorInvalidValue;
      }
    }
    const int fa = pr.a_fmt < 0 ? g.fmt : pr.a_fmt, fb = pr.b_fmt < 0 ? g.fmt : pr.b_fmt;
    if (fa != fb) {
      set_error("gemm problem %d: A and B must share one 16-bit format (wgmma), got %d and %d", p, fa, fb);
      return (int)cudaErrorInvalidValue;
    }
    const int total_kb = pr.taps * pr.kblk_per_tap * (g.split ? 3 : 1);
    const int per = (total_kb + pr.ksplit - 1) / pr.ksplit;
    if ((pr.ksplit - 1) * per >= total_kb) {
      set_error("gemm problem %d: ksplit %d leaves an empty split for %d k-blocks", p, pr.ksplit, total_kb);
      return (int)cudaErrorInvalidValue;
    }
    total += ((((pr.M + GEMM_BM - 1) / GEMM_BM) + cl - 1) / cl) * ((pr.N + bn - 1) / bn) * pr.ksplit;
    auto al16 = [](const void* q) { return (reinterpret_cast<uintptr_t>(q) & 15) == 0; };
    GemmProblem& w = g.p[p];
    w.vec_ok = (pr.N % 16 == 0) && (pr.cs32 <= 1) && (!pr.aux32 || (al16(pr.aux32) && pr.ld_aux % 4 == 0)) &&
               (!pr.pre32 || (al16(pr.pre32) && pr.ld_pre % 4 == 0)) && (!pr.dact16 || (al16(pr.dact16) && pr.ld_dact % 8 == 0)) && (!pr.mask16 || (al16(pr.mask16) && pr.ld_mask % 8 == 0)) &&
               (!pr.resid || (al16(pr.resid) && pr.ld_resid % 4 == 0)) && (!pr.addtab || (al16(pr.addtab) && pr.ld_addtab % 4 == 0)) &&
               (!pr.out32 || (al16(pr.out32) && pr.ld32 % 4 == 0)) && (!pr.out32_id || (al16(pr.out32_id) && pr.ld32_id % 4 == 0)) &&
               ((!pr.out16 && !pr.out16p) || (pr.ld16 % 8 == 0 && al16(pr.out16) && al16(pr.out16p) && g.lo16 % 8 == 0));
    auto al32 = [](const void* q) { return (reinterpret_cast<uintptr_t>(q) & 31) == 0; };
    if (w.vec_ok && (!pr.pre32 || (al32(pr.pre32) && pr.ld_pre % 8 == 0)) && (!pr.dact16 || (al32(pr.dact16) && pr.ld_dact % 16 == 0)) && (!pr.aux32 || (al32(pr.aux32) && pr.ld_aux % 8 == 0)) && (!pr.addtab || (al32(pr.addtab) && pr.ld_addtab % 8 == 0)) && (!pr.resid || (al32(pr.resid) && pr.ld_resid % 8 == 0)) &&
        (!pr.out32 || (al32(pr.out32) && pr.ld32 % 8 == 0)) && (!pr.out32_id || (al32(pr.out32_id) && pr.ld32_id % 8 == 0)) &&
        ((!pr.out16 && !pr.out16p) || (pr.ld16 % 16 == 0 && al32(pr.out16) && al32(pr.out16p) && g.lo16 % 16 == 0)))
      w.vec_ok = 2;
  }
  if (total == 0) return 0;
  bool full = false;
  for (int p = 0; p < g.num; ++p) {
    const GemmProblem& pr = g.p[p];
    full = full || pr.vec_ok != 2 || pr.pre32 || pr.dact16 || pr.aux32 || pr.mask16 || pr.accumulate || pr.ksplit > 1 ||
           (pr.out32_id && !g.split) || pr.colsum || pr.cs32 > 1;
  }
  if (g.split && full) {
    set_error("fp16x3 gemm group: needs the lean epilogue (N %% 16 == 0, 32-byte aligned outputs and lo planes, no training options or split-K)");
    return (int)cudaErrorInvalidValue;
  }
  if (used_full) *used_full = full ? 1 : 0;
  g.bn = bn;
  g.dbg = g_timeline;
  cudaError_t e;
  if (cl == 1) {
    const int grid = total < num_sms ? total : num_sms;
    if (g.split) {
      launch_k(gemm_wgmma_kernel<1, false, true>, dim3(grid), dim3(kGemmThreads), Cfg::kSmemBytes, stream, g);
    } else if (full) {
      launch_k(gemm_wgmma_kernel<1, true>, dim3(grid), dim3(kGemmThreads), Cfg::kSmemBytes, stream, g);
    } else {
      launch_k(gemm_wgmma_kernel<1, false>, dim3(grid), dim3(kGemmThreads), Cfg::kSmemBytes, stream, g);
    }
    e = cudaGetLastError();
  } else {
    const int max_clusters = num_sms / 2;
    const int clusters = total < max_clusters ? total : max_clusters;
    cudaLaunchConfig_t cfg;
    memset(&cfg, 0, sizeof(cfg));
    cfg.gridDim = dim3(2 * clusters);
    cfg.blockDim = dim3(kGemmThreads);
    cfg.dynamicSmemBytes = Cfg::kSmemBytes;
    cfg.stream = stream;
    cudaLaunchAttribute attr[2];
    attr[0].id = cudaLaunchAttributeClusterDimension;
    attr[0].val.clusterDim.x = 2;
    attr[0].val.clusterDim.y = 1;
    attr[0].val.clusterDim.z = 1;
    attr[1].id = cudaLaunchAttributeProgrammaticStreamSerialization;
    attr[1].val.programmaticStreamSerializationAllowed = 1;
    cfg.attrs = attr;
    cfg.numAttrs = pdl_enabled() ? 2 : 1;
    ++*launch_counter();
    e = full ? cudaLaunchKernelEx(&cfg, gemm_wgmma_kernel<2, true>, g) : cudaLaunchKernelEx(&cfg, gemm_wgmma_kernel<2, false>, g);
  }
  if (e != cudaSuccess) {
    set_error("gemm launch failed: %s", cudaGetErrorString(e));
    return (int)e;
  }
  return 0;
}

TileChoice choose_tile(const int* Ms, const int* Ns, const int* kblocks, int num, int num_sms, int step, int max_split) {
  TileChoice best{256, 1};
  double best_t = -1.0;
  for (int ks = 1; ks <= max_split; ks *= 2) {
    bool ok = true;
    for (int p = 0; p < num; ++p) ok = ok && (ks == 1 || ks * 4 <= kblocks[p]);
    if (!ok) break;
    for (int bn = 256; bn >= 64; bn -= step) {
      long tiles = 0;
      long load[256];
      const int ncta = num_sms < 256 ? num_sms : 256;
      for (int i = 0; i < ncta; ++i) load[i] = 0;
      for (int p = 0; p < num; ++p) {
        const long t = (long)((Ms[p] + GEMM_BM - 1) / GEMM_BM) * ((Ns[p] + bn - 1) / bn) * ks;
        const int kb = (kblocks[p] + ks - 1) / ks;
        for (long i = 0; i < t; ++i) load[(tiles + i) % ncta] += kb;
        tiles += t;
      }
      long kb_cta = 0;
      for (int i = 0; i < ncta; ++i) kb_cta = load[i] > kb_cta ? load[i] : kb_cta;
      const long rounds = (tiles + ncta - 1) / ncta;
      const double epi = 0.5 + bn * (ks > 1 ? 3.0 : 2.0) / 256.0;
      const double t = 1.0 + (0.15 + 0.0018 * bn) * (double)kb_cta + epi * (1.0 + 0.3 * (double)(rounds - 1));
      if (best_t < 0 || t < best_t - 1e-9) {
        best_t = t;
        best = TileChoice{bn, ks};
      }
    }
  }
  return best;
}

}
```

### univtg_b200/csrc/kernels.h

```cpp
#pragma once
#include <string.h>
#include <cuda.h>
#include <cuda_runtime.h>
#include <stdint.h>

namespace uv {

constexpr int GEMM_BM = 128;
constexpr int GEMM_BK = 64;
constexpr int GEMM_MAX_GROUP = 4;

enum Act { ACT_NONE = 0, ACT_RELU = 1, ACT_GELU = 2, ACT_QUICKGELU = 3 };

struct OperandCoord {
  int base0, mn0s, tap0, k0s;
  int base1, mn1s, tap1, k1s;
};

struct GemmProblem {
  CUtensorMap tm_a;
  CUtensorMap tm_b;
  OperandCoord ca, cb;
  int a_mn, b_mn;
  int b_box_rows;
  int M, N;
  int taps;
  int kblk_per_tap;
  int ksplit;
  const float* bias;
  float alpha;
  int act;
  const float* row_scale;
  int rps_in;
  int rps_out;
  int row_off;
  int zero_sep;
  const float* resid;
  int ld_resid;
  const float* addtab;
  int ld_addtab;
  float* out32;
  int ld32;
  float* out32_id;
  int ld32_id;
  uint16_t* out16;
  uint16_t* out16p;
  int ld16;
  int accumulate;
  int a_fmt, b_fmt;
  int out_fmt;
  const float* aux32;
  int ld_aux;
  int aux_mode;
  const uint16_t* mask16;
  int ld_mask;
  float* pre32;
  int ld_pre;
  uint16_t* dact16;
  int ld_dact;
  int mask_mul;
  float colsum_scale;
  float* colsum;
  int cs32;
  int skip_sep;
  int b_3d;
  int vec_ok;
};

struct GemmGroup {
  int num;
  int fmt;
  int bn;
  int cluster;
  int split;
  long long lo16;
  unsigned long long* dbg;
  GemmProblem p[GEMM_MAX_GROUP];
};

int launch_gemm_group(GemmGroup& g, int bn, int num_sms, cudaStream_t stream, int* used_full = nullptr);
struct TileChoice {
  int bn, ksplit;
};
TileChoice choose_tile(const int* Ms, const int* Ns, const int* kblocks, int num, int num_sms, int step, int max_split);
int make_tmap_b_mn(GemmProblem& p, const void* base, uint64_t rows, uint64_t cols, uint64_t ld_elems, int bn);

int make_tmap_2d(CUtensorMap* out, const void* base, uint64_t rows, uint64_t cols, uint64_t ld_elems, uint32_t box_rows,
                 uint32_t box_cols);

int make_tmap_split(CUtensorMap* out, const void* base, uint64_t rows, uint64_t cols, uint64_t ld_elems, uint32_t box_rows,
                    uint32_t box_cols, uint64_t lo_elems);

void set_gemm_timeline_buffer(unsigned long long* buf);
const char* last_error();
void set_error(const char* fmt, ...);
bool pdl_enabled();
long long* launch_counter();
template <typename... KArgs, typename... Args>
inline cudaError_t launch_k(void (*kern)(KArgs...), dim3 grid, dim3 block, size_t smem, cudaStream_t stream, Args&&... args) {
  ++*launch_counter();
  cudaLaunchConfig_t cfg;
  memset(&cfg, 0, sizeof(cfg));
  cfg.gridDim = grid;
  cfg.blockDim = block;
  cfg.dynamicSmemBytes = smem;
  cfg.stream = stream;
  cudaLaunchAttribute attr[1];
  attr[0].id = cudaLaunchAttributeProgrammaticStreamSerialization;
  attr[0].val.programmaticStreamSerializationAllowed = 1;
  cfg.attrs = attr;
  cfg.numAttrs = pdl_enabled() ? 1 : 0;
  return cudaLaunchKernelEx(&cfg, kern, static_cast<KArgs>(args)...);
}

struct PackSeg {
  long long start4, end4;
  void* dst;
  int kind, rows, cols, ld;
};
constexpr int kMaxPackSegs = 40;
struct PackSegTable {
  int n, fmt;
  PackSeg s[kMaxPackSegs];
};

struct AdamDevState {
  const float* lr;
  int32_t* step;
  const float* bc_table;
  int32_t table_len;
};
void adamw_bias_row(float beta1, float beta2, int32_t step, float* bc1, float* bc2_sqrt);
int adamw_step_impl(float* params, float* grads, float* exp_avg, float* exp_avg_sq, size_t n, float lr, float beta1, float beta2,
                    float eps, float weight_decay, int32_t step, float max_grad_norm, int32_t write_clipped_grads, float* scratch3,
                    const PackSegTable* segs, void* stream, const AdamDevState* dev = nullptr);


}
```

### univtg_b200/csrc/plan.h

```cpp
#pragma once
#include <math.h>
#include <stdio.h>
#include <string.h>

#include "../../include/univtg_b200.h"
#include "backward.h"
#include "kernels.h"
#include "loss.h"
#include "ptx.cuh"
#include "rowops.h"

using namespace uv;

namespace {

inline size_t align_up(size_t v, size_t a) { return (v + a - 1) / a * a; }

#define UV_REQ(cond, ...)      \
  do {                         \
    if (!(cond)) {             \
      set_error(__VA_ARGS__);  \
      return 1;                \
    }                          \
  } while (0)
// ... 280 lines not shown
  float *pmean_v[3], *prstd_v[3], *pmean_t[3], *prstd_t[3];
  float *p_vid32[3], *p_txt32[3];
  float* txtproj32;
  float* pool_alpha;
  float *pos, *key_mask, *pool_logits;
  float* dp_scale;
  uint16_t *xin16[17], *xpos16[17];
  uint16_t *qkv16[16], *attn16[16], *x1_16[16], *h16[16];
  float *lse[16], *y1[16], *mean1[16], *rstd1[16], *y2[16], *mean2[16], *rstd2[16];
  uint16_t* dgelu16[16];
  float *x32, *x1_32;
  uint16_t *hA, *h1, *hc2, *hs2;
  uint16_t* br16;
  float *pred_logits, *pred_spans;
  size_t total;
};

constexpr int kMaxMarks = 640;
struct univtg_plan {
  univtg_config cfg;
  univtg_shape shp;
  PackedLayout lay;
  const uint8_t* packed;
  uint8_t* ws;
  const float* dim_t;
  int num_sms;
  int in_fmt;
  int num_sms_bwd;
  float attn_dropout;
  const unsigned long long* seed_dev = nullptr;
  int txt_pos_on;
  long long pk_lo, ws_lo;
  univtg_txt_pos txt_pos;
  int B, Lv, Lt, L, d, ff, H, dh, M, Mv, Mt, Mh;
  int bn_proj[3];
  int bn_qkv, bn_out, bn_ffn1, bn_ffn2, bn_conv1, bn_conv2;
  int launches;
  int n_grad_events;
  cudaEvent_t grad_events[24];
  int profiling;
  int n_marks;
  cudaEvent_t marks[kMaxMarks];
  int mark_kind[kMaxMarks];
};

namespace {
inline uv::DropSpec plan_drop_spec(const univtg_plan* P, const univtg_rng* rng, unsigned int stream, float p) {
  uv::DropSpec s = uv::make_drop_spec(rng->seed, stream, p);
  s.seed_ptr = P->seed_dev;
  return s;
}

inline void prof_begin(univtg_plan* P, cudaStream_t st) {
  if (!P->profiling) return;
  P->n_marks = 0;
  if (!P->marks[0]) cudaEventCreate(&P->marks[0]);
  cudaEventRecord(P->marks[0], st);
  P->mark_kind[0] = -1;
  P->n_marks = 1;
}
inline void prof_mark(univtg_plan* P, cudaStream_t st, int kind) {
  if (!P->profiling || P->n_marks >= kMaxMarks) return;
  const int i = P->n_marks;
  if (!P->marks[i]) cudaEventCreate(&P->marks[i]);
  cudaEventRecord(P->marks[i], st);
  P->mark_kind[i] = kind;
  P->n_marks = i + 1;
}
inline int gemm_launch(univtg_plan* P, GemmGroup& g, int bn, int sms, cudaStream_t st) {
  prof_mark(P, st, 3);
  const int rc = launch_gemm_group(g, bn, sms, st);
  prof_mark(P, st, 1);
  return rc;
}

inline void reset_group(GemmGroup& g, int num, int fmt, int split = 0, long long lo16 = 0) {
  memset(&g, 0, sizeof(g));
  g.num = num;
  g.fmt = fmt;
  g.split = split;
  g.lo16 = lo16;
}

inline int attention_bwd_simt_max_L() {
  int dev = 0, optin = 0;
  if (cudaGetDevice(&dev) != cudaSuccess || cudaDeviceGetAttribute(&optin, cudaDevAttrMaxSharedMemoryPerBlockOptin, dev) != cudaSuccess ||
      optin <= 0) {
    cudaGetLastError();
    optin = 227 * 1024;
  }
  return (int)((size_t)optin / attention_bwd_simt_smem(1));
}

inline AttnBwdArgs attention_bwd_args(const void* qkv, const void* dO, const float* key_mask, const float* lse, const float* delta,
                                      float* dqkv32, int B, int L, int H, int dh, int fmt) {
  AttnBwdArgs a;
  memset(&a, 0, sizeof(a));
  a.qkv = reinterpret_cast<const uint16_t*>(qkv);
  a.dO = reinterpret_cast<const uint16_t*>(dO);
  a.key_mask = key_mask;
  a.lse = lse;
  a.delta = delta;
  a.dqkv32 = dqkv32;
  a.scale = 1.0f / sqrtf((float)dh);
  a.B = B;
  a.L = L;
  a.H = H;
  a.dh = dh;
  a.d = H * dh;
  a.fmt_act = a.fmt_grad = fmt;
  return a;
}

inline int attention_bwd_route(AttnBwdArgs& a, bool tc, uint16_t* dqkv16, cudaStream_t st, int* dq_mode, int* kernel_used = nullptr,
                               univtg_plan* P = nullptr) {
  const int M = a.B * a.L, d = a.d;
  a.dq_atomic = (!tc || a.L > 128) ? 1 : 0;
  a.dqkv16 = a.dq_atomic ? nullptr : dqkv16;
  if (dq_mode) *dq_mode = a.dq_atomic ? 2 : (a.dqkv16 ? 0 : 1);
  if (a.dq_atomic) cudaMemsetAsync(a.dqkv32, 0, (size_t)M * 3 * d * 4, st);
  if (!tc) return launch_attention_bwd_simt(a, st, kernel_used);
  if (make_tmap_2d(&a.tm_qkv, a.qkv, (uint64_t)M, (uint64_t)3 * d, (uint64_t)3 * d, 128, 64)) return 1;
  if (make_tmap_2d(&a.tm_do, a.dO, (uint64_t)M, (uint64_t)d, (uint64_t)d, 128, 64)) return 1;
  if (P) prof_mark(P, st, 3);
  const int rc = launch_attention_bwd(a, st, kernel_used);
  if (P) prof_mark(P, st, 2);
  return rc;
}
}

namespace {

void init_problem(GemmProblem& p) {
  memset(&p, 0, sizeof(p));
  p.taps = 1;
  p.ksplit = 1;
  p.alpha = 1.f;
  p.a_fmt = p.b_fmt = p.out_fmt = -1;
  p.colsum_scale = 1.f;
  p.ca = OperandCoord{0, 0, 0, 1, 0, 1, 0, 0};
  p.cb = OperandCoord{0, 0, 0, 1, 0, 1, 0, 0};
}

struct Mat16 {
  const uint16_t* p;
  int rows, cols, ld;
};

inline int make_tmap_op(CUtensorMap* m, const void* base, uint64_t rows, uint64_t cols, uint64_t ld, uint32_t box_rows, uint32_t box_cols,
                        long long lo) {
  return lo ? make_tmap_split(m, base, rows, cols, ld, box_rows, box_cols, (uint64_t)lo) : make_tmap_2d(m, base, rows, cols, ld, box_rows, box_cols);
}

int setup_gemm(GemmProblem& p, Mat16 A, int a_mn, Mat16 B, int b_mn, int M, int N, int K, int bn, long long lo_a = 0,
               long long lo_b = 0) {
  init_problem(p);
  if ((lo_a || lo_b) && (a_mn || b_mn || !lo_a || !lo_b)) {
    set_error("fp16x3 GEMM operands must both be split and K-major");
    return 1;
  }
  p.M = M;
  p.N = N;
  p.a_mn = a_mn;
  p.b_mn = b_mn;
  p.kblk_per_tap = (K + 63) / 64;
  int rc = 0;
  if (!a_mn) {
    rc |= make_tmap_op(&p.tm_a, A.p, (uint64_t)A.rows, (uint64_t)A.cols, (uint64_t)A.ld, GEMM_BM, 64, lo_a);
  } else {
    rc |= make_tmap_2d(&p.tm_a, A.p, (uint64_t)A.rows, (uint64_t)A.cols, (uint64_t)A.ld, 64, 64);
    p.ca = OperandCoord{0, 1, 0, 0, 0, 0, 0, 1};
  }
  if (!b_mn) {
    rc |= make_tmap_op(&p.tm_b, B.p, (uint64_t)B.rows, (uint64_t)B.cols, (uint64_t)B.ld, (uint32_t)bn, 64, lo_b);
    p.b_box_rows = bn;
  } else {
    rc |= make_tmap_b_mn(p, B.p, (uint64_t)B.rows, (uint64_t)B.cols, (uint64_t)B.ld, bn);
    p.cb = OperandCoord{0, 1, 0, 0, 0, 0, 0, 1};
  }
  return rc;
}

int conv_fwd_problem(GemmProblem& p, int Mh, const uint16_t* X, int lda, int Cin, const uint16_t* Wp, int N, int bn, long long lo_a = 0,
                     long long lo_b = 0) {
  init_problem(p);
  p.M = Mh;
  p.N = N;
  p.taps = 3;
  p.kblk_per_tap = Cin / 64;
  p.ca = OperandCoord{0, 0, 0, 1, 0, 1, 1, 0};
  p.cb = OperandCoord{0, 0, Cin, 1, 0, 1, 0, 0};
  int r = make_tmap_op(&p.tm_a, X, (uint64_t)Mh + 2, (uint64_t)Cin, (uint64_t)lda, GEMM_BM, 64, lo_a);
  r |= make_tmap_op(&p.tm_b, Wp, (uint64_t)N, (uint64_t)3 * Cin, (uint64_t)3 * Cin, (uint32_t)bn, 64, lo_b);
  p.b_box_rows = bn;
  return r;
}

int conv_dgrad_problem(GemmProblem& p, int Mh, const uint16_t* dY, int ldy, int Kc, const uint16_t* Wp, int Cin, int bn) {
  init_problem(p);
  p.M = Mh;
  p.N = Cin;
  p.taps = 3;
  p.kblk_per_tap = Kc / 64;
  p.b_mn = 1;
  p.ca = OperandCoord{0, 0, 0, 1, 0, 1, 1, 0};
  p.cb = OperandCoord{2 * Cin, 1, -Cin, 0, 0, 0, 0, 1};
  int r = make_tmap_2d(&p.tm_a, dY, (uint64_t)Mh + 2, (uint64_t)Kc, (uint64_t)ldy, GEMM_BM, 64);
  r |= make_tmap_b_mn(p, Wp, (uint64_t)Kc, (uint64_t)3 * Cin, (uint64_t)3 * Cin, bn);
  return r;
}
int conv_wgrad_problem(GemmProblem& p, int Mh, const uint16_t* dY, int ldy, int Nc, const uint16_t* X, int ldx, int Cin, int t, int bn) {
  init_problem(p);
  p.M = Nc;
  p.N = Cin;
  p.a_mn = 1;
  p.b_mn = 1;
  p.kblk_per_tap = (Mh + 63) / 64;
  p.ca = OperandCoord{0, 1, 0, 0, 1, 0, 0, 1};
  p.cb = OperandCoord{0, 1, 0, 0, t, 0, 0, 1};
  int r = make_tmap_2d(&p.tm_a, dY, (uint64_t)Mh + 2, (uint64_t)Nc, (uint64_t)ldy, 64, 64);
  r |= make_tmap_b_mn(p, X, (uint64_t)Mh + 2, (uint64_t)Cin, (uint64_t)ldx, bn);
  return r;
}

inline int setup_linear(GemmProblem& p, const uint16_t* A, int M, int K, int lda, const uint16_t* W, int N, int ldw, int bn,
                        long long lo_a = 0, long long lo_w = 0) {
  return setup_gemm(p, Mat16{A, M, K, lda}, 0, Mat16{W, N, K, ldw}, 0, M, N, K, bn, lo_a, lo_w);
}

struct MNK {
  int M, N, K;
};
inline TileChoice tile_for(int sms, int step, int max_split, MNK a, MNK b = MNK{0, 0, 0}, MNK c3 = MNK{0, 0, 0}) {
  const int Ms[3] = {a.M, b.M, c3.M}, Ns[3] = {a.N, b.N, c3.N}, kb[3] = {(a.K + 63) / 64, (b.K + 63) / 64, (c3.K + 63) / 64};
  const int num = c3.M > 0 ? 3 : (b.M > 0 ? 2 : 1);
  return choose_tile(Ms, Ns, kb, num, sms, step, max_split);
}

FwdBufs make_infer_ws(const univtg_config& c, const univtg_shape& s, const PackedLayout& L, uint8_t* base) {
  FwdBufs w;
  memset(&w, 0, sizeof(w));
  Cursor cur;
  const size_t d = c.hidden_dim, ff = c.dim_feedforward;
  const size_t B = s.batch, Lv = s.l_vid, Lt = s.l_txt, Lc = Lv + Lt;
  const size_t M = B * Lc, Mv = B * Lv, Mt = B * Lt, Mh = B * (Lv + 1);
  auto take16 = [&](size_t elems) { return reinterpret_cast<uint16_t*>(base + cur.take(elems * 2)); };
  auto take32 = [&](size_t elems) { return reinterpret_cast<float*>(base + cur.take(elems * 4)); };
  for (int i = 0; i < c.n_input_proj; ++i) {
    w.a_vid[i] = take16(Mv * L.vid[i].kpad);
    w.a_txt[i] = take16(Mt * L.txt[i].kpad);
  }
  float* p_vid32 = take32(Mv * d);
  float* p_txt32 = take32(Mt * d);
  w.txtproj32 = take32(Mt * d);
  w.pos = take32(Mv * d);
  w.key_mask = take32(B * Lc);
  w.pool_logits = take32(B * Lt);
  w.x32 = w.x1_32 = take32(M * d);
  w.br16 = take16(M * d);
  uint16_t* x16 = take16(M * d);
  uint16_t* xpos16 = take16(M * d);
  uint16_t* qkv16 = take16(M * 3 * d);
  uint16_t* attn16 = take16(M * d);
  uint16_t* h16 = take16(M * ff);
  w.hA = take16((Mh + 2) * d);
  w.h1 = take16((Mh + 2) * 2 * d);
  w.hc2 = take16((Mh + 2) * d);
  w.hs2 = take16((Mh + 2) * d);
  w.total = cur.off;
  for (int i = 0; i < c.n_input_proj; ++i) {
    w.p_vid32[i] = p_vid32;
    w.p_txt32[i] = p_txt32;
  }
  for (int l = 0; l <= c.enc_layers; ++l) {
    w.xin16[l] = x16;
    w.xpos16[l] = xpos16;
  }
  for (int l = 0; l < c.enc_layers; ++l) {
    w.qkv16[l] = qkv16;
    w.attn16[l] = attn16;
    w.x1_16[l] = x16;
    w.h16[l] = h16;
  }
  return w;
}

struct TxtPosWs {
  float* pos;
  float *mean, *rstd;
  float* dpos;
  uint16_t* dqk16;
  size_t total;
};
inline TxtPosWs make_txt_pos_ws(const univtg_config& c, const univtg_shape& s, void* base_) {
  TxtPosWs w;
  memset(&w, 0, sizeof(w));
  uint8_t* base = reinterpret_cast<uint8_t*>(base_);
  Cursor cur;
  const size_t d = c.hidden_dim, Mt = (size_t)s.batch * s.l_txt;
  w.pos = reinterpret_cast<float*>(base + cur.take(Mt * d * 4));
  if (s.training) {
    w.mean = reinterpret_cast<float*>(base + cur.take(Mt * 4));
    w.rstd = reinterpret_cast<float*>(base + cur.take(Mt * 4));
    w.dpos = reinterpret_cast<float*>(base + cur.take(Mt * d * 4));
    w.dqk16 = reinterpret_cast<uint16_t*>(base + cur.take(Mt * 2 * d * 2));
  }
  w.total = cur.off;
  return w;
}

bool check_shape(const univtg_shape* s) {
  if (!s || s->batch < 1 || s->l_vid < 1 || s->l_txt < 1) {
    set_error("bad shape");
    return false;
  }
  return true;
}

}

int run_forward(univtg_plan* P, const FwdBufs& W, const float* src_txt, const float* src_txt_mask, const float* src_vid,
                const float* src_vid_mask, const float* droppath_scale, const float* const* drop_masks, const univtg_rng* rng,
                float* pred_logits, float* pred_spans, float* vid_mem_proj, float* txt_mem_proj, float* saliency_scores,
                cudaStream_t st);
```

### univtg_b200/csrc/ptx.cuh

```cuda
#pragma once
#include <cuda.h>
#include <cuda_fp16.h>
#include <cuda_bf16.h>
#include <cuda_runtime.h>
#include <stdint.h>

namespace uv {

#define UV_DEVINL __device__ __forceinline__

UV_DEVINL uint32_t smem_u32(const void* p) { return (uint32_t)__cvta_generic_to_shared(p); }

UV_DEVINL uint32_t lane_id() { return threadIdx.x & 31; }

UV_DEVINL bool elect_one() {
  uint32_t pred = 0;
  asm volatile(
      "{\n\t"
      ".reg .pred P;\n\t"
      "elect.sync _|P, 0xffffffff;\n\t"
      "selp.b32 %0, 1, 0, P;\n\t"
      "}\n"
      : "=r"(pred));
  return pred != 0;
}

UV_DEVINL void pdl_launch_dependents() { asm volatile("griddepcontrol.launch_dependents;" ::: "memory"); }
UV_DEVINL void pdl_wait() { asm volatile("griddepcontrol.wait;" ::: "memory"); }
UV_DEVINL void pdl_prologue() {
  pdl_launch_dependents();
  pdl_wait();
}

UV_DEVINL void mbar_init(uint64_t* bar, uint32_t count) {
  asm volatile("mbarrier.init.shared::cta.b64 [%0], %1;" ::"r"(smem_u32(bar)), "r"(count) : "memory");
}
UV_DEVINL void fence_barrier_init() { asm volatile("fence.mbarrier_init.release.cluster;" ::: "memory"); }
UV_DEVINL void fence_proxy_async_smem() { asm volatile("fence.proxy.async.shared::cta;" ::: "memory"); }

UV_DEVINL void mbar_arrive_expect_tx(uint64_t* bar, uint32_t bytes) {
  asm volatile("mbarrier.arrive.expect_tx.shared::cta.b64 _, [%0], %1;" ::"r"(smem_u32(bar)), "r"(bytes) : "memory");
}
UV_DEVINL void mbar_arrive(uint64_t* bar) {
  asm volatile("mbarrier.arrive.shared::cta.b64 _, [%0];" ::"r"(smem_u32(bar)) : "memory");
}
UV_DEVINL bool mbar_try_wait(uint64_t* bar, uint32_t parity) {
  uint32_t ok;
  asm volatile(
      "{\n\t"
      ".reg .pred P;\n\t"
      "mbarrier.try_wait.parity.shared::cta.b64 P, [%1], %2;\n\t"
      "selp.b32 %0, 1, 0, P;\n\t"
      "}\n"
      : "=r"(ok)
      : "r"(smem_u32(bar)), "r"(parity)
      : "memory");
  return ok != 0;
}
UV_DEVINL void mbar_wait(uint64_t* bar, uint32_t parity) {
  while (!mbar_try_wait(bar, parity)) {
  }
}

UV_DEVINL void tma_prefetch_desc(const CUtensorMap* m) {
  asm volatile("prefetch.tensormap [%0];" ::"l"(reinterpret_cast<uint64_t>(m)) : "memory");
}
UV_DEVINL void tma_load_2d(void* smem_dst, const CUtensorMap* m, uint64_t* bar, int c0, int c1) {
  asm volatile(
      "cp.async.bulk.tensor.2d.shared::cluster.global.mbarrier::complete_tx::bytes [%0], [%1, {%3, %4}], [%2];"
      :
      : "r"(smem_u32(smem_dst)), "l"(reinterpret_cast<uint64_t>(m)), "r"(smem_u32(bar)), "r"(c0), "r"(c1)
      : "memory");
}
UV_DEVINL uint32_t cluster_ctarank() {
  uint32_t r;
  asm volatile("mov.u32 %0, %%cluster_ctarank;" : "=r"(r));
  return r;
}
UV_DEVINL void cluster_sync_all() {
  asm volatile("barrier.cluster.arrive.release.aligned;" ::: "memory");
  asm volatile("barrier.cluster.wait.acquire.aligned;" ::: "memory");
}
UV_DEVINL uint32_t mapa_shared(uint32_t smem_addr, uint32_t rank) {
  uint32_t r;
  asm volatile("mapa.shared::cluster.u32 %0, %1, %2;" : "=r"(r) : "r"(smem_addr), "r"(rank));
  return r;
}
UV_DEVINL void mbar_arrive_cluster(uint32_t cluster_addr) {
  asm volatile("mbarrier.arrive.release.cluster.shared::cluster.b64 _, [%0];" ::"r"(cluster_addr) : "memory");
}
UV_DEVINL void tma_load_2d_mc(void* smem_dst, const CUtensorMap* m, uint64_t* bar, int c0, int c1, uint16_t cta_mask) {
  asm volatile(
      "cp.async.bulk.tensor.2d.shared::cluster.global.mbarrier::complete_tx::bytes.multicast::cluster [%0], [%1, {%3, %4}], [%2], %5;"
      :
      : "r"(smem_u32(smem_dst)), "l"(reinterpret_cast<uint64_t>(m)), "r"(smem_u32(bar)), "r"(c0), "r"(c1), "h"(cta_mask)
      : "memory");
}
UV_DEVINL void tma_load_3d(void* smem_dst, const CUtensorMap* m, uint64_t* bar, int c0, int c1, int c2) {
  asm volatile(
      "cp.async.bulk.tensor.3d.shared::cluster.global.mbarrier::complete_tx::bytes [%0], [%1, {%3, %4, %5}], [%2];"
      :
      : "r"(smem_u32(smem_dst)), "l"(reinterpret_cast<uint64_t>(m)), "r"(smem_u32(bar)), "r"(c0), "r"(c1), "r"(c2)
      : "memory");
}

UV_DEVINL void wgmma_fence() { asm volatile("wgmma.fence.sync.aligned;" ::: "memory"); }
UV_DEVINL void wgmma_commit() { asm volatile("wgmma.commit_group.sync.aligned;" ::: "memory"); }
template <int N>
UV_DEVINL void wgmma_wait() {
  asm volatile("wgmma.wait_group.sync.aligned %0;" ::"n"(N) : "memory");
}
UV_DEVINL void reg_fence(float& r) { asm volatile("" : "+f"(r)::"memory"); }
UV_DEVINL void reg_fence(uint32_t& r) { asm volatile("" : "+r"(r)::"memory"); }
template <uint32_t kRegs>
UV_DEVINL void setmaxnreg_inc() {
  asm volatile("setmaxnreg.inc.sync.aligned.u32 %0;" ::"n"(kRegs));
}
template <uint32_t kRegs>
UV_DEVINL void setmaxnreg_dec() {
  asm volatile("setmaxnreg.dec.sync.aligned.u32 %0;" ::"n"(kRegs));
}
UV_DEVINL void named_bar_sync(int id, int count) { asm volatile("bar.sync %0, %1;" ::"r"(id), "r"(count) : "memory"); }

UV_DEVINL uint64_t make_smem_desc_sw128(uint32_t smem_addr, uint32_t lbo_bytes, uint32_t sbo_bytes) {
  uint64_t d = 0;
  d |= (uint64_t)((smem_addr & 0x3FFFF) >> 4);
  d |= (uint64_t)((lbo_bytes >> 4) & 0x3FFF) << 16;
  d |= (uint64_t)((sbo_bytes >> 4) & 0x3FFF) << 32;
  d |= (uint64_t)1 << 62;
  return d;
}

UV_DEVINL float warp_sum(float v) {
#pragma unroll
  for (int o = 16; o > 0; o >>= 1) v += __shfl_xor_sync(0xffffffffu, v, o);
  return v;
}
UV_DEVINL void st_global_256(void* p, const uint32_t (&w)[8]) {
  uint4* q = reinterpret_cast<uint4*>(p);
  q[0] = make_uint4(w[0], w[1], w[2], w[3]);
  q[1] = make_uint4(w[4], w[5], w[6], w[7]);
}
UV_DEVINL void st_global_256f(float* p, float a0, float a1, float a2, float a3, float a4, float a5, float a6, float a7) {
  float4* q = reinterpret_cast<float4*>(p);
  q[0] = make_float4(a0, a1, a2, a3);
  q[1] = make_float4(a4, a5, a6, a7);
}
UV_DEVINL void ld_global_256f(const float* p, float* v) {
  const float4 a = reinterpret_cast<const float4*>(p)[0];
  const float4 b = reinterpret_cast<const float4*>(p)[1];
  v[0] = a.x; v[1] = a.y; v[2] = a.z; v[3] = a.w;
  v[4] = b.x; v[5] = b.y; v[6] = b.z; v[7] = b.w;
}
UV_DEVINL void red_add_f32x4(float* addr, float4 v) {
  asm volatile("red.global.add.v4.f32 [%0], {%1, %2, %3, %4};" ::"l"(addr), "f"(v.x), "f"(v.y), "f"(v.z), "f"(v.w) : "memory");
}
UV_DEVINL float warp_colsum16(float (&v)[16], int lane) {
#pragma unroll
  for (int off = 8; off >= 1; off >>= 1) {
    const bool hi = (lane & off) != 0;
#pragma unroll
    for (int k = 0; k < off; ++k) {
      const float send = hi ? v[k] : v[k + off];
      const float keep = hi ? v[k + off] : v[k];
      v[k] = keep + __shfl_xor_sync(0xffffffffu, send, off);
    }
  }
  return v[0] + __shfl_xor_sync(0xffffffffu, v[0], 16);
}
UV_DEVINL float warp_max(float v) {
#pragma unroll
  for (int o = 16; o > 0; o >>= 1) v = fmaxf(v, __shfl_xor_sync(0xffffffffu, v, o));
  return v;
}
UV_DEVINL float erf_fast(float x) {
  const float ax = fabsf(x);
  const float t = __fdividef(1.0f, fmaf(0.3275911f, ax, 1.0f));
  float y = fmaf(1.061405429f, t, -1.453152027f);
  y = fmaf(y, t, 1.421413741f);
  y = fmaf(y, t, -0.284496736f);
  y = fmaf(y, t, 0.254829592f);
  y = y * t;
  const float r = fmaf(-y, __expf(-ax * ax), 1.0f);
  return copysignf(r, x);
}
UV_DEVINL float gelu_erf(float x) {
  const float ax = fabsf(x);
  const float t = __fdividef(1.0f, fmaf(0.3275911f * 0.70710678118654752440f, ax, 1.0f));
  float y = fmaf(1.061405429f, t, -1.453152027f);
  y = fmaf(y, t, 1.421413741f);
  y = fmaf(y, t, -0.284496736f);
  y = fmaf(y, t, 0.254829592f);
  y = y * t;
  const float e = exp2f(ax * ax * (-0.5f * 1.4426950408889634f));
  const float r = fmaf(-y, e, 1.0f);
  return 0.5f * fmaf(ax, r, x);
}
UV_DEVINL float gelu_erf_grad(float x) {
  const float ax = fabsf(x);
  const float t = __fdividef(1.0f, fmaf(0.3275911f * 0.70710678118654752440f, ax, 1.0f));
  float y = fmaf(1.061405429f, t, -1.453152027f);
  y = fmaf(y, t, 1.421413741f);
  y = fmaf(y, t, -0.284496736f);
  y = fmaf(y, t, 0.254829592f);
  y = y * t;
  const float e = exp2f(ax * ax * (-0.5f * 1.4426950408889634f));
  const float r = fmaf(-y, e, 1.0f);
  return fmaf(0.5f, copysignf(r, x), 0.5f) + x * 0.3989422804014327f * e;
}
UV_DEVINL void gelu_erf_both(float x, float& g, float& dg) {
  const float ax = fabsf(x);
  const float t = __fdividef(1.0f, fmaf(0.3275911f * 0.70710678118654752440f, ax, 1.0f));
  float y = fmaf(1.061405429f, t, -1.453152027f);
  y = fmaf(y, t, 1.421413741f);
  y = fmaf(y, t, -0.284496736f);
  y = fmaf(y, t, 0.254829592f);
  y = y * t;
  const float e = exp2f(ax * ax * (-0.5f * 1.4426950408889634f));
  const float r = fmaf(-y, e, 1.0f);
  g = 0.5f * fmaf(ax, r, x);
  dg = fmaf(0.5f, copysignf(r, x), 0.5f) + x * 0.3989422804014327f * e;
}
UV_DEVINL bool pos16(uint16_t h) { return (h & 0x8000u) == 0 && (h & 0x7fffu) != 0; }

UV_DEVINL uint16_t cvt16(float v, int fmt) {
  return fmt ? __bfloat16_as_ushort(__float2bfloat16_rn(v)) : __half_as_ushort(__float2half_rn(v));
}
UV_DEVINL uint32_t cvt16x2(float lo, float hi, int fmt) {
  return (uint32_t)cvt16(lo, fmt) | ((uint32_t)cvt16(hi, fmt) << 16);
}
UV_DEVINL float ld16(uint16_t v, int fmt) {
  return fmt ? __bfloat162float(__ushort_as_bfloat16(v)) : __half2float(__ushort_as_half(v));
}
UV_DEVINL uint16_t cvt16_lo(float v) { return cvt16(v - ld16(cvt16(v, 0), 0), 0); }
UV_DEVINL uint32_t cvt16x2_lo(float a, float b) { return (uint32_t)cvt16_lo(a) | ((uint32_t)cvt16_lo(b) << 16); }
UV_DEVINL float ld16x3(uint16_t hi, uint16_t lo) { return ld16(hi, 0) + ld16(lo, 0); }

}
```

Measured before the change: 6371.

## Add ping-pong warpgroup GEMM schedule alongside cooperative kernel

Adds a second persistent GEMM kernel in which two consumer warpgroups each own a whole 64-row tile and alternate mainloop and epilogue. While one warpgroup runs its epilogue, the other keeps the tensor cores busy. The change adds a 64-row A tensor map per problem, moves shared GEMM code into a common header, and adds an auto/cooperative/ping-pong schedule selector with debug hooks. The risks are that the smaller 64-row tiles lower operand reuse and that the auto heuristic may pick the worse schedule for some shapes.

```diff
diff --git a/__graft_entry__.py b/__graft_entry__.py
--- a/__graft_entry__.py
+++ b/__graft_entry__.py
@@ -7,7 +7,7 @@
 CSRC = os.path.join(ROOT, "univtg_b200", "csrc")
 LIBDIR = os.path.join(ROOT, "univtg_b200", "lib")
 LIB = os.path.join(LIBDIR, "libunivtg_b200.so")
-SOURCES = ["gemm.cu", "rowops.cu", "attention.cu", "attention_bwd.cu", "backward.cu", "loss.cu", "optim.cu", "postproc.cu", "train.cu", "api.cu", "clip.cu",
+SOURCES = ["gemm.cu", "gemm_pp.cu", "rowops.cu", "attention.cu", "attention_bwd.cu", "backward.cu", "loss.cu", "optim.cu", "postproc.cu", "train.cu", "api.cu", "clip.cu",
            "hostio.cu", "metrics.cu", "task_eval.cu", "teacher.cu"]
 
 NVCC_FLAGS = [
diff --git a/include/univtg_b200.h b/include/univtg_b200.h
--- a/include/univtg_b200.h
+++ b/include/univtg_b200.h
@@ -224,6 +224,8 @@
 } univtg_txt_pos_bwd;
 int univtg_op_txt_pos_bwd(const univtg_txt_pos_bwd* args, const univtg_rng* rng, int32_t mask_index, void* stream);
 int univtg_debug_gemm_timeline(void* buf);
+int univtg_debug_set_gemm_schedule(int32_t mode);
+int univtg_debug_last_gemm_schedule(int32_t* schedule, int32_t* bn);
 int univtg_debug_choose_tile(const int32_t* Ms, const int32_t* Ns, const int32_t* kblocks, int32_t num, int32_t num_sms, int32_t step,
                              int32_t max_split, int32_t* bn, int32_t* ksplit);
 int univtg_adamw_step(float* params, float* grads, float* exp_avg, float* exp_avg_sq, size_t n, float lr, float beta1,
diff --git a/univtg_b200/_lib.py b/univtg_b200/_lib.py
--- a/univtg_b200/_lib.py
+++ b/univtg_b200/_lib.py
@@ -183,6 +183,8 @@
     "univtg_op_pool_bwd": (c_int, [c_void_p] * 6 + [c_float, c_int, c_int, c_int, c_void_p]),
     "univtg_op_txt_pos_bwd": (c_int, [ctypes.POINTER(TxtPosBwd), ctypes.POINTER(Rng), c_int, c_void_p]),
     "univtg_debug_gemm_timeline": (c_int, [c_void_p]),
+    "univtg_debug_set_gemm_schedule": (c_int, [c_int]),
+    "univtg_debug_last_gemm_schedule": (c_int, [c_void_p, c_void_p]),
     "univtg_debug_choose_tile": (c_int, [c_void_p, c_void_p, c_void_p, c_int, c_int, c_int, c_int, c_void_p, c_void_p]),
     "univtg_op_layernorm": (c_int, [c_void_p, c_int, c_int, c_void_p, c_void_p, c_float, c_int, c_void_p, c_void_p, c_int,
                                     c_void_p]),
diff --git a/univtg_b200/csrc/api.cu b/univtg_b200/csrc/api.cu
--- a/univtg_b200/csrc/api.cu
+++ b/univtg_b200/csrc/api.cu
@@ -796,6 +796,26 @@
   const uv::TileChoice t = uv::choose_tile(Ms, Ns, kblocks, num, num_sms, step, max_split);
   *bn = t.bn;
   *ksplit = t.ksplit;
+  return 0;
+}
+
+int univtg_debug_set_gemm_schedule(int32_t mode) {
+  if (uv::set_gemm_schedule(mode) != 0) {
+    set_error("univtg_debug_set_gemm_schedule: mode %d (0 auto, 1 cooperative, 2 ping-pong)", mode);
+    return 1;
+  }
+  return 0;
+}
+
+int univtg_debug_last_gemm_schedule(int32_t* schedule, int32_t* bn) {
+  if (!schedule || !bn) {
+    set_error("univtg_debug_last_gemm_schedule: null argument");
+    return 1;
+  }
+  int s = 0, w = 0;
+  uv::last_gemm_schedule(&s, &w);
+  *schedule = s;
+  *bn = w;
   return 0;
 }
 
diff --git a/univtg_b200/csrc/gemm.cu b/univtg_b200/csrc/gemm.cu
--- a/univtg_b200/csrc/gemm.cu
+++ b/univtg_b200/csrc/gemm.cu
@@ -3,360 +3,15 @@
 #include <stdlib.h>
 #include <string.h>
 
-#include "kernels.h"
-#include "ptx.cuh"
-#include "wgmma.cuh"
+#include "gemm_common.cuh"
 
 namespace uv {
-
-template <int CL>
-struct GemmCfg {
-  static constexpr int kMaxStages = 8;
-  static constexpr int kABytes = GEMM_BM * 128;
-  static constexpr int kRingBytes = 4 * (kABytes + 256 * 128);
-  static constexpr int kEpiStride = 36;
-  static constexpr int kEpiFloats = 2 * 64 * kEpiStride;
-  static constexpr int kSmemBytes = 1024  + kRingBytes + kEpiFloats * 4 + 256;
-  __host__ __device__ static constexpr int stage_bytes(int bn) { return kABytes + bn * 128; }
-  __host__ __device__ static constexpr int num_stages(int bn) {
-    return kRingBytes / stage_bytes(bn) < kMaxStages ? kRingBytes / stage_bytes(bn) : kMaxStages;
-  }
-};
-
-constexpr int kGemmThreads = 384;
-
-struct TileInfo {
-  int p, m_blk, n_blk, kb0, kb1, split;
-};
-
-template <int CL, bool SPLIT>
-__device__ __forceinline__ bool decode_tile(const GemmGroup& g, int bn, int t, int rank, TileInfo& ti) {
-  for (int p = 0; p < g.num; ++p) {
-    const GemmProblem& pr = g.p[p];
-    const int tm_real = (pr.M + GEMM_BM - 1) / GEMM_BM;
-    const int tm = (tm_real + CL - 1) / CL;
-    const int tn = (pr.N + bn - 1) / bn;
-    const int cnt = tm * tn * pr.ksplit;
-    if (t < cnt) {
-      ti.p = p;
-      ti.n_blk = t % tn;
-      const int rest = t / tn;
-      ti.m_blk = (rest % tm) * CL + rank;
-      ti.split = rest / tm;
-      const int total_kb = pr.taps * pr.kblk_per_tap * (SPLIT ? 3 : 1);
-      const int per = (total_kb + pr.ksplit - 1) / pr.ksplit;
-      ti.kb0 = ti.split * per;
-      ti.kb1 = min(total_kb, ti.kb0 + per);
-      return true;
-    }
-    t -= cnt;
-  }
-  return false;
-}
-
-__device__ __forceinline__ void stamp(unsigned long long* dbg, int slot) {
-  if (dbg != nullptr) {
-    unsigned long long t;
-    asm volatile("mov.u64 %0, %globaltimer;" : "=l"(t));
-    dbg[(size_t)blockIdx.x * 8 + slot] = t;
-  }
-}
-
-template <int N, int OFF, int BF, int TA, int TB>
-__device__ __forceinline__ void mma_cols(float* acc, uint64_t da, uint64_t db, uint32_t scale_d) {
-  constexpr int W = N >= 256 ? 256 : N >= 128 ? 128 : N >= 64 ? 64 : N >= 32 ? 32 : 16;
-  WG<W, BF>::template ss<TA, TB>(acc + OFF / 2, da, db, scale_d);
-  if constexpr (N > W) {
-    constexpr uint32_t adv = TB ? (W / 64) * 8192 / 16 : W * 128 / 16;
-    mma_cols<N - W, OFF + W, BF, TA, TB>(acc, da, db + adv, scale_d);
-  }
-}
-
-struct Ring {
-  uint8_t* base;
-  uint64_t* full;
-  uint64_t* empty;
-  int stage_bytes, stages;
-  int stage;
-  uint32_t phase;
-};
-
-template <int CL>
-__device__ __forceinline__ void release_stage(const Ring& ring, int s, int tid, int crank) {
-  if (tid == 0) {
-    mbar_arrive(&ring.empty[s]);
-    if (CL > 1) mbar_arrive_cluster(mapa_shared(smem_u32(&ring.empty[s]), (uint32_t)(crank ^ 1)));
-  }
-}
-
-template <int CL, int BN, int BF, int TA, int TB>
-__device__ __forceinline__ void tile_mainloop(float* acc, Ring& ring, int kb0, int kb1, int cw, int tid, int crank) {
-  const uint64_t da_hi = TA ? make_smem_desc_sw128(0, 8192, 1024) : make_smem_desc_sw128(0, 16, 1024);
-  const uint64_t db_hi = TB ? make_smem_desc_sw128(0, 8192, 1024) : make_smem_desc_sw128(0, 16, 1024);
-  constexpr uint32_t a_step = TA ? 128u : 2u, b_step = TB ? 128u : 2u;
-  int prev = -1;
-  for (int kb = kb0; kb < kb1; ++kb) {
-    mbar_wait(&ring.full[ring.stage], ring.phase);
-    const uint32_t sa = smem_u32(ring.base + ring.stage * ring.stage_bytes);
-    const uint64_t da = da_hi + (uint64_t)((sa + cw * 8192) >> 4);
-    const uint64_t db = db_hi + (uint64_t)((sa + GemmCfg<CL>::kABytes) >> 4);
-    wgmma_fence();
-#pragma unroll
-    for (int k = 0; k < GEMM_BK / 16; ++k)
-      mma_cols<BN, 0, BF, TA, TB>(acc, da + k * a_step, db + k * b_step, (kb > kb0 || k > 0) ? 1u : 0u);
-    wgmma_commit();
-    wgmma_wait<1>();
-    if (prev >= 0) release_stage<CL>(ring, prev, tid, crank);
-    prev = ring.stage;
-    if (++ring.stage == ring.stages) {
-      ring.stage = 0;
-      ring.phase ^= 1;
-    }
-  }
-  wgmma_wait<0>();
-#pragma unroll
-  for (int i = 0; i < BN / 2; ++i) reg_fence(acc[i]);
-  if (prev >= 0) release_stage<CL>(ring, prev, tid, crank);
-}
-
-template <int CL, bool SPLIT, int BN>
-__device__ __forceinline__ void tile_mainloop_any(float* acc, Ring& ring, int bf, int a_mn, int b_mn, int kb0, int kb1, int cw, int tid,
-                                                  int crank) {
-  if constexpr (SPLIT) {
-    tile_mainloop<CL, BN, 0, 0, 0>(acc, ring, kb0, kb1, cw, tid, crank);
-  } else {
-    if constexpr (CL == 1 && BN % 64 == 0) {
-      if (b_mn) {
-        if (bf) {
-          if (a_mn) tile_mainloop<CL, BN, 1, 1, 1>(acc, ring, kb0, kb1, cw, tid, crank);
-          else tile_mainloop<CL, BN, 1, 0, 1>(acc, ring, kb0, kb1, cw, tid, crank);
-        } else {
-          if (a_mn) tile_mainloop<CL, BN, 0, 1, 1>(acc, ring, kb0, kb1, cw, tid, crank);
-          else tile_mainloop<CL, BN, 0, 0, 1>(acc, ring, kb0, kb1, cw, tid, crank);
-        }
-        return;
-      }
-    }
-    if (bf) {
-      if (a_mn) tile_mainloop<CL, BN, 1, 1, 0>(acc, ring, kb0, kb1, cw, tid, crank);
-      else tile_mainloop<CL, BN, 1, 0, 0>(acc, ring, kb0, kb1, cw, tid, crank);
-    } else {
-      if (a_mn) tile_mainloop<CL, BN, 0, 1, 0>(acc, ring, kb0, kb1, cw, tid, crank);
-      else tile_mainloop<CL, BN, 0, 0, 0>(acc, ring, kb0, kb1, cw, tid, crank);
-    }
-  }
-}
-
-struct EpiRow {
-  bool valid;
-  float rsc;
-  const float* resid_row;
-  const float* aux_row;
-  const uint16_t* mask_row;
-  const float* add_row;
-  float* o32_row;
-  float* o32i_row;
-  uint16_t* o16_row;
-  uint16_t* o16p_row;
-  float* pre_row;
-  uint16_t* dact_row;
-};
-
-__device__ __forceinline__ void ld16f(const float* p, float (&v)[16]) {
-#pragma unroll
-  for (int q = 0; q < 4; ++q) {
-    const float4 t4 = reinterpret_cast<const float4*>(p)[q];
-    v[4 * q] = t4.x; v[4 * q + 1] = t4.y; v[4 * q + 2] = t4.z; v[4 * q + 3] = t4.w;
-  }
-}
-
-template <bool FULL, bool SPLIT>
-__device__ __forceinline__ void epi_step(const GemmProblem& pr, const EpiRow& r, float (&v)[16], int n0, int fmt, int lane,
-                                         long long lo16) {
-  const int pN = pr.N;
-  const int act = pr.act;
-  const int ofmt = pr.out_fmt < 0 ? fmt : pr.out_fmt;
-  const bool vec = FULL ? pr.vec_ok != 0 : true;
-  const bool atomic = (pr.accumulate != 0) || (pr.ksplit > 1);
-  const bool mask_mul = FULL && pr.mask_mul != 0;
-  const float rsc = r.rsc;
-  if (FULL && r.pre_row != nullptr && r.valid) {
-    if (vec) {
-      st_global_256f(r.pre_row + n0, v[0], v[1], v[2], v[3], v[4], v[5], v[6], v[7]);
-      st_global_256f(r.pre_row + n0 + 8, v[8], v[9], v[10], v[11], v[12], v[13], v[14], v[15]);
-    } else {
-#pragma unroll
-      for (int q = 0; q < 4; ++q)
-        if (n0 + 4 * q < pN)
-          *reinterpret_cast<float4*>(r.pre_row + n0 + 4 * q) = make_float4(v[4 * q], v[4 * q + 1], v[4 * q + 2], v[4 * q + 3]);
-    }
-  }
-  if (FULL && act == ACT_GELU && r.dact_row != nullptr) {
-    float dg[16];
-#pragma unroll
-    for (int j = 0; j < 16; ++j) {
-      float gj;
-      gelu_erf_both(v[j], gj, dg[j]);
-      v[j] = gj * rsc;
-    }
-    if (r.valid) {
-      if (vec) {
-        uint32_t w8[8];
-#pragma unroll
-        for (int q = 0; q < 8; ++q) w8[q] = cvt16x2(dg[2 * q], dg[2 * q + 1], ofmt);
-        st_global_256(r.dact_row + n0, w8);
-      } else {
-#pragma unroll
-        for (int j = 0; j < 16; ++j)
-          if (n0 + j < pN) r.dact_row[n0 + j] = cvt16(dg[j], ofmt);
-      }
-    }
-  } else if (act == ACT_GELU) {
-#pragma unroll
-    for (int j = 0; j < 16; ++j) v[j] = gelu_erf(v[j]) * rsc;
-  } else if (act == ACT_RELU) {
-#pragma unroll
-    for (int j = 0; j < 16; ++j) v[j] = fmaxf(v[j], 0.f) * rsc;
-  } else if (act == ACT_QUICKGELU) {
-#pragma unroll
-    for (int j = 0; j < 16; ++j) v[j] = v[j] / (1.f + expf(-1.702f * v[j])) * rsc;
-  } else {
-#pragma unroll
-    for (int j = 0; j < 16; ++j) v[j] *= rsc;
-  }
-  if (vec) {
-    if (r.valid) {
-      if (r.resid_row != nullptr) {
-        float rv[16];
-        ld16f(r.resid_row + n0, rv);
-#pragma unroll
-        for (int j = 0; j < 16; ++j) v[j] += rv[j];
-      }
-      if (FULL && r.aux_row != nullptr) {
-        float av[16];
-        ld16f(r.aux_row + n0, av);
-        if (pr.aux_mode == 1) {
-#pragma unroll
-          for (int j = 0; j < 16; ++j) v[j] *= gelu_erf_grad(av[j]);
-        } else {
-#pragma unroll
-          for (int j = 0; j < 16; ++j) v[j] *= av[j];
-        }
-      }
-      if (FULL && r.mask_row != nullptr) {
-#pragma unroll
-        for (int q = 0; q < 2; ++q) {
-          const uint4 mk = reinterpret_cast<const uint4*>(r.mask_row + n0)[q];
-          const uint32_t w4[4] = {mk.x, mk.y, mk.z, mk.w};
-#pragma unroll
-          for (int e = 0; e < 4; ++e) {
-            if (mask_mul) {
-              v[8 * q + 2 * e] *= ld16((uint16_t)(w4[e] & 0xffff), fmt);
-              v[8 * q + 2 * e + 1] *= ld16((uint16_t)(w4[e] >> 16), fmt);
-            } else {
-              if (!pos16((uint16_t)(w4[e] & 0xffff))) v[8 * q + 2 * e] = 0.f;
-              if (!pos16((uint16_t)(w4[e] >> 16))) v[8 * q + 2 * e + 1] = 0.f;
-            }
-          }
-        }
-      }
-      if (r.o32_row != nullptr) {
-        if (FULL && atomic) {
-#pragma unroll
-          for (int q = 0; q < 4; ++q)
-            red_add_f32x4(r.o32_row + n0 + 4 * q, make_float4(v[4 * q], v[4 * q + 1], v[4 * q + 2], v[4 * q + 3]));
-        } else {
-          st_global_256f(r.o32_row + n0, v[0], v[1], v[2], v[3], v[4], v[5], v[6], v[7]);
-          st_global_256f(r.o32_row + n0 + 8, v[8], v[9], v[10], v[11], v[12], v[13], v[14], v[15]);
-        }
-      }
-      if ((FULL || SPLIT) && r.o32i_row != nullptr) {
-        st_global_256f(r.o32i_row + n0, v[0], v[1], v[2], v[3], v[4], v[5], v[6], v[7]);
-        st_global_256f(r.o32i_row + n0 + 8, v[8], v[9], v[10], v[11], v[12], v[13], v[14], v[15]);
-      }
-      if (r.o16_row != nullptr) {
-        uint32_t w8[8];
-#pragma unroll
-        for (int q = 0; q < 8; ++q) w8[q] = cvt16x2(v[2 * q], v[2 * q + 1], ofmt);
-        st_global_256(r.o16_row + n0, w8);
-        if constexpr (SPLIT) {
-#pragma unroll
-          for (int q = 0; q < 8; ++q) w8[q] = cvt16x2_lo(v[2 * q], v[2 * q + 1]);
-          st_global_256(r.o16_row + lo16 + n0, w8);
-        }
-      }
-      if (r.o16p_row != nullptr) {
-        float p[16];
-#pragma unroll
-        for (int j = 0; j < 16; ++j) p[j] = v[j];
-        if (r.add_row != nullptr) {
-          float av[16];
-          ld16f(r.add_row + n0, av);
-#pragma unroll
-          for (int j = 0; j < 16; ++j) p[j] += av[j];
-        }
-        uint32_t w8[8];
-#pragma unroll
-        for (int q = 0; q < 8; ++q) w8[q] = cvt16x2(p[2 * q], p[2 * q + 1], ofmt);
-        st_global_256(r.o16p_row + n0, w8);
-        if constexpr (SPLIT) {
-#pragma unroll
-          for (int q = 0; q < 8; ++q) w8[q] = cvt16x2_lo(p[2 * q], p[2 * q + 1]);
-          st_global_256(r.o16p_row + lo16 + n0, w8);
-        }
-      }
-    } else {
-#pragma unroll
-      for (int j = 0; j < 16; ++j) v[j] = 0.f;
-    }
-  } else if constexpr (FULL) {
-    const int cs32 = pr.cs32 > 1 ? pr.cs32 : 1;
-#pragma unroll
-    for (int j = 0; j < 16; ++j) {
-      const int n = n0 + j;
-      float x = v[j];
-      if (r.valid && n < pN) {
-        if (r.resid_row != nullptr) x += r.resid_row[n];
-        if (r.aux_row != nullptr) x *= (pr.aux_mode == 1) ? gelu_erf_grad(r.aux_row[n]) : r.aux_row[n];
-        if (r.mask_row != nullptr) {
-          if (mask_mul) x *= ld16(r.mask_row[n], fmt);
-          else if (!pos16(r.mask_row[n])) x = 0.f;
-        }
-        if (r.o32_row != nullptr) {
-          float* dst = r.o32_row + (size_t)n * cs32;
-          if (atomic) atomicAdd(dst, x);
-          else *dst = x;
-        }
-        if (r.o32i_row != nullptr) r.o32i_row[n] = x;
-        if (r.o16_row != nullptr) {
-          r.o16_row[n] = cvt16(x, ofmt);
-          if constexpr (SPLIT) r.o16_row[lo16 + n] = cvt16_lo(x);
-        }
-        if (r.o16p_row != nullptr) {
-          const float xp = x + (r.add_row ? r.add_row[n] : 0.f);
-          r.o16p_row[n] = cvt16(xp, ofmt);
-          if constexpr (SPLIT) r.o16p_row[lo16 + n] = cvt16_lo(xp);
-        }
-      } else {
-        x = 0.f;
-      }
-      v[j] = x;
-    }
-  }
-  if (FULL && pr.colsum != nullptr) {
-    const float sj = warp_colsum16(v, lane);
-    if (lane < 16 && n0 + lane < pN) atomicAdd(pr.colsum + n0 + lane, sj * pr.colsum_scale);
-  }
-}
 
 template <int CL, bool FULL, bool SPLIT, int BN>
 __device__ __forceinline__ void consumer_tiles(const GemmGroup& g, Ring& ring, float* epi_buf, int tile0, int tstep, int crank, int cw,
                                                int lane) {
   using Cfg = GemmCfg<CL>;
   const int tid = threadIdx.x & 127;
-  const int fr = 16 * (tid >> 5) + (lane >> 2);
-  const int fc = 2 * (lane & 3);
-  const int erow = tid & 63, ehalf = tid >> 6;
   float* ebuf = epi_buf + cw * 64 * Cfg::kEpiStride;
   const int fmt = g.fmt;
   float acc[BN / 2];
@@ -375,60 +30,7 @@
     if (tid == 0 && cw == 0) stamp(g.dbg, 4);
     first_tile = false;
 
-    const int pM = pr.M, pN = pr.N, rps_in = pr.rps_in;
-    const int m = ti.m_blk * GEMM_BM + cw * 64 + erow;
-    int b = 0, l = m;
-    if (rps_in > 0) {
-      b = m / rps_in;
-      l = m - b * rps_in;
-    }
-    const bool is_sep = (rps_in > 0) && (l == rps_in - 1);
-    EpiRow r;
-    r.valid = (m < pM) && !(pr.skip_sep && is_sep);
-    r.rsc = pr.alpha;
-    if (pr.row_scale != nullptr && m < pM) r.rsc *= pr.row_scale[b];
-    if (pr.zero_sep && is_sep) r.rsc = 0.f;
-    const size_t orow = (size_t)((rps_in > 0 ? b * pr.rps_out + l : m) + pr.row_off);
-    r.resid_row = pr.resid ? pr.resid + orow * pr.ld_resid : nullptr;
-    r.aux_row = (FULL && pr.aux32) ? pr.aux32 + orow * pr.ld_aux : nullptr;
-    r.mask_row = (FULL && pr.mask16) ? pr.mask16 + orow * pr.ld_mask : nullptr;
-    r.add_row = pr.addtab ? pr.addtab + (size_t)m * pr.ld_addtab : nullptr;
-    r.o32_row = pr.out32 ? pr.out32 + orow * pr.ld32 : nullptr;
-    r.o32i_row = ((FULL || SPLIT) && pr.out32_id) ? pr.out32_id + (size_t)m * pr.ld32_id : nullptr;
-    r.o16_row = pr.out16 ? pr.out16 + orow * pr.ld16 : nullptr;
-    r.o16p_row = pr.out16p ? pr.out16p + orow * pr.ld16 : nullptr;
-    r.pre_row = (FULL && pr.pre32) ? pr.pre32 + orow * pr.ld_pre : nullptr;
-    r.dact_row = (FULL && pr.dact16) ? pr.dact16 + orow * pr.ld_dact : nullptr;
-    const float* __restrict__ bias = (ti.split == 0) ? pr.bias : nullptr;
-    const int nt0 = ti.n_blk * BN;
-#pragma unroll 1
-    for (int cc = 0; cc < (BN + 31) / 32 && nt0 + cc * 32 < pN; ++cc) {
-#pragma unroll
-      for (int c = 0; c < (BN + 31) / 32; ++c) {
-        if (c == cc) {
-#pragma unroll
-          for (int ii = 0; ii < 4; ++ii) {
-            const int i = 4 * c + ii;
-            if (8 * i < BN) {
-              *reinterpret_cast<float2*>(ebuf + fr * Cfg::kEpiStride + 8 * ii + fc) = make_float2(acc[4 * i], acc[4 * i + 1]);
-              *reinterpret_cast<float2*>(ebuf + (fr + 8) * Cfg::kEpiStride + 8 * ii + fc) = make_float2(acc[4 * i + 2], acc[4 * i + 3]);
-            }
-          }
-        }
-      }
-      named_bar_sync(1 + cw, 128);
-      const int n0 = nt0 + cc * 32 + ehalf * 16;
-      if (cc * 32 + ehalf * 16 < BN && n0 < pN) {
-        float v[16];
-        ld16f(ebuf + erow * Cfg::kEpiStride + ehalf * 16, v);
-        if (bias != nullptr) {
-#pragma unroll
-          for (int j = 0; j < 16; ++j) v[j] += (n0 + j < pN) ? __ldg(bias + n0 + j) : 0.f;
-        }
-        epi_step<FULL, SPLIT>(pr, r, v, n0, fmt, lane, g.lo16);
-      }
-      named_bar_sync(1 + cw, 128);
-    }
+    tile_epilogue<FULL, SPLIT, BN>(g, pr, ti, acc, ebuf, ti.m_blk * GEMM_BM + cw * 64, tid, lane);
     if (tid == 0 && cw == 1) stamp(g.dbg, 6);
   }
 }
@@ -687,6 +289,101 @@
   return rc;
 }
 
+static int g_schedule = 0;
+static int g_last_schedule = 0, g_last_bn = 0;
+int set_gemm_schedule(int mode) {
+  if (mode < 0 || mode > 2) return 1;
+  g_schedule = mode;
+  return 0;
+}
+void last_gemm_schedule(int* schedule, int* bn) {
+  *schedule = g_last_schedule;
+  *bn = g_last_bn;
+}
+
+static int group_tiles(const GemmGroup& g, int bm, int bn) {
+  int total = 0;
+  for (int p = 0; p < g.num; ++p) total += ((g.p[p].M + bm - 1) / bm) * ((g.p[p].N + bn - 1) / bn) * g.p[p].ksplit;
+  return total;
+}
+
+static double epi_chunk_us(const GemmProblem& p) {
+  int bytes = 0;
+  bytes += p.out16 ? 2 : 0;
+  bytes += p.out16p ? 2 : 0;
+  bytes += p.out32 ? 4 : 0;
+  bytes += p.out32_id ? 4 : 0;
+  bytes += p.pre32 ? 4 : 0;
+  bytes += p.dact16 ? 2 : 0;
+  bytes += p.resid ? 4 : 0;
+  bytes += p.aux32 ? 4 : 0;
+  bytes += p.mask16 ? 2 : 0;
+  return 0.65 + 0.22 * bytes + (p.act == ACT_GELU ? 0.3 : 0.0);
+}
+
+static double model_us(const GemmGroup& g, int bn, int num_sms, bool pp) {
+  const int bm = pp ? 64 : GEMM_BM;
+  const int total = group_tiles(g, bm, bn);
+  const int grid = total < num_sms ? total : num_sms;
+  const double kb_us = pp ? 0.0018 * (64 + bn) : 0.15 + 0.0018 * bn;
+  double t_ml = 1.6, wg_free[2] = {1.6, 1.6}, t = 1.6;
+  int j = 0, p = 0, base = 0;
+  for (int tile = 0; tile < total; tile += grid, ++j) {
+    int cnt = 0;
+    for (;; ++p) {
+      const GemmProblem& pr = g.p[p];
+      cnt = ((pr.M + bm - 1) / bm) * ((pr.N + bn - 1) / bn) * pr.ksplit;
+      if (tile < base + cnt) break;
+      base += cnt;
+    }
+    const GemmProblem& pr = g.p[p];
+    const int kb = (pr.taps * pr.kblk_per_tap + pr.ksplit - 1) / pr.ksplit;
+    const double ml = kb * kb_us, epi = ((bn + 31) / 32) * epi_chunk_us(pr);
+    if (!pp) {
+      t += ml + epi;
+    } else {
+      const double start = t_ml > wg_free[j & 1] ? t_ml : wg_free[j & 1];
+      t_ml = start + ml;
+      wg_free[j & 1] = t_ml + epi;
+    }
+  }
+  return pp ? (wg_free[0] > wg_free[1] ? wg_free[0] : wg_free[1]) : t;
+}
+
+static int choose_schedule(const GemmGroup& g, int bn, int num_sms, bool full, int* pp_bn) {
+  *pp_bn = 0;
+  bool ok = g.cluster != 2 && !g.split, retile = true, b_mn = false;
+  for (int p = 0; p < g.num; ++p) {
+    ok = ok && (g.p[p].a_mn || g.p[p].a64);
+    retile = retile && g.p[p].b_base != nullptr;
+    b_mn = b_mn || g.p[p].b_mn;
+  }
+  if (g_schedule == 1 || (g_schedule == 0 && !ok)) return 0;
+  if (!ok) {
+    set_error("gemm schedule 2 (ping-pong) needs CTA clusters off, 16-bit operands and 64-row A maps");
+    return (int)cudaErrorInvalidValue;
+  }
+  const int max_bn = full ? kPingPongFullMaxBn : 256;
+  if (g_schedule == 2) {
+    if (bn > max_bn) {
+      set_error("gemm schedule 2 (ping-pong): the FULL epilogue runs up to bn %d (got %d)", max_bn, bn);
+      return (int)cudaErrorInvalidValue;
+    }
+    *pp_bn = bn;
+    return 0;
+  }
+  double best = 0.95 * model_us(g, bn, num_sms, false);
+  for (int w = 64; w <= max_bn; w += b_mn ? 64 : 16) {
+    if (w != bn && !retile) continue;
+    const double t = model_us(g, w, num_sms, true);
+    if (t < best) {
+      best = t;
+      *pp_bn = w;
+    }
+  }
+  return 0;
+}
+
 int launch_gemm_group(GemmGroup& g, int bn, int num_sms, cudaStream_t stream, int* used_full) {
   using Cfg = GemmCfg<1>;
   static_assert(GemmCfg<1>::kSmemBytes == GemmCfg<2>::kSmemBytes, "both variants use the same dynamic shared memory size");
@@ -797,10 +494,26 @@
     return (int)cudaErrorInvalidValue;
   }
   if (used_full) *used_full = full ? 1 : 0;
-  g.bn = bn;
+  int pp_bn = 0;
+  const int rc = choose_schedule(g, bn, num_sms, full, &pp_bn);
+  if (rc != 0) return rc;
+  g_last_schedule = pp_bn > 0 ? 2 : 1;
+  g_last_bn = pp_bn > 0 ? pp_bn : bn;
   g.dbg = g_timeline;
   cudaError_t e;
-  if (cl == 1) {
+  if (pp_bn > 0) {
+    for (int p = 0; p < g.num && pp_bn != bn; ++p) {
+      GemmProblem& w = g.p[p];
+      const int r = w.b_mn ? make_tmap_b_mn(w, w.b_base, w.b_rows, w.b_cols, w.b_ld, pp_bn)
+                           : make_tmap_2d(&w.tm_b, w.b_base, w.b_rows, w.b_cols, w.b_ld, (uint32_t)pp_bn, 64);
+      if (r != 0) return (int)cudaErrorInvalidValue;
+      w.b_box_rows = pp_bn;
+    }
+    g.bn = pp_bn;
+    const int tiles = group_tiles(g, 64, pp_bn);
+    e = launch_gemm_pingpong(g, tiles < num_sms ? tiles : num_sms, full, stream);
+  } else if (cl == 1) {
+    g.bn = bn;
     const int grid = total < num_sms ? total : num_sms;
     if (g.split) {
       launch_k(gemm_wgmma_kernel<1, false, true>, dim3(grid), dim3(kGemmThreads), Cfg::kSmemBytes, stream, g);
@@ -811,6 +524,7 @@
     }
     e = cudaGetLastError();
   } else {
+    g.bn = bn;
     const int max_clusters = num_sms / 2;
     const int clusters = total < max_clusters ? total : max_clusters;
     cudaLaunchConfig_t cfg;
diff --git a/univtg_b200/csrc/gemm_common.cuh b/univtg_b200/csrc/gemm_common.cuh
--- /dev/null
+++ b/univtg_b200/csrc/gemm_common.cuh
@@ -0,0 +1,412 @@
+#pragma once
+#include "kernels.h"
+#include "ptx.cuh"
+#include "wgmma.cuh"
+
+namespace uv {
+
+template <int CL>
+struct GemmCfg {
+  static constexpr int kMaxStages = 8;
+  static constexpr int kABytes = GEMM_BM * 128;
+  static constexpr int kRingBytes = 4 * (kABytes + 256 * 128);
+  static constexpr int kEpiStride = 36;
+  static constexpr int kEpiFloats = 2 * 64 * kEpiStride;
+  static constexpr int kSmemBytes = 1024  + kRingBytes + kEpiFloats * 4 + 256;
+  __host__ __device__ static constexpr int stage_bytes(int bn) { return kABytes + bn * 128; }
+  __host__ __device__ static constexpr int num_stages(int bn) {
+    return kRingBytes / stage_bytes(bn) < kMaxStages ? kRingBytes / stage_bytes(bn) : kMaxStages;
+  }
+};
+
+constexpr int kGemmThreads = 384;
+
+struct TileInfo {
+  int p, m_blk, n_blk, kb0, kb1, split;
+};
+
+template <int CL, bool SPLIT, int BM = GEMM_BM>
+__device__ __forceinline__ bool decode_tile(const GemmGroup& g, int bn, int t, int rank, TileInfo& ti) {
+  for (int p = 0; p < g.num; ++p) {
+    const GemmProblem& pr = g.p[p];
+    const int tm_real = (pr.M + BM - 1) / BM;
+    const int tm = (tm_real + CL - 1) / CL;
+    const int tn = (pr.N + bn - 1) / bn;
+    const int cnt = tm * tn * pr.ksplit;
+    if (t < cnt) {
+      ti.p = p;
+      ti.n_blk = t % tn;
+      const int rest = t / tn;
+      ti.m_blk = (rest % tm) * CL + rank;
+      ti.split = rest / tm;
+      const int total_kb = pr.taps * pr.kblk_per_tap * (SPLIT ? 3 : 1);
+      const int per = (total_kb + pr.ksplit - 1) / pr.ksplit;
+      ti.kb0 = ti.split * per;
+      ti.kb1 = min(total_kb, ti.kb0 + per);
+      return true;
+    }
+    t -= cnt;
+  }
+  return false;
+}
+
+__device__ __forceinline__ void stamp(unsigned long long* dbg, int slot) {
+  if (dbg != nullptr) {
+    unsigned long long t;
+    asm volatile("mov.u64 %0, %globaltimer;" : "=l"(t));
+    dbg[(size_t)blockIdx.x * 8 + slot] = t;
+  }
+}
+
+template <int N, int OFF, int BF, int TA, int TB>
+__device__ __forceinline__ void mma_cols(float* acc, uint64_t da, uint64_t db, uint32_t scale_d) {
+  constexpr int W = N >= 256 ? 256 : N >= 128 ? 128 : N >= 64 ? 64 : N >= 32 ? 32 : 16;
+  WG<W, BF>::template ss<TA, TB>(acc + OFF / 2, da, db, scale_d);
+  if constexpr (N > W) {
+    constexpr uint32_t adv = TB ? (W / 64) * 8192 / 16 : W * 128 / 16;
+    mma_cols<N - W, OFF + W, BF, TA, TB>(acc, da, db + adv, scale_d);
+  }
+}
+
+struct Ring {
+  uint8_t* base;
+  uint64_t* full;
+  uint64_t* empty;
+  int stage_bytes, stages;
+  int stage;
+  uint32_t phase;
+};
+
+template <int CL>
+__device__ __forceinline__ void release_stage(const Ring& ring, int s, int tid, int crank) {
+  if (tid == 0) {
+    mbar_arrive(&ring.empty[s]);
+    if (CL > 1) mbar_arrive_cluster(mapa_shared(smem_u32(&ring.empty[s]), (uint32_t)(crank ^ 1)));
+  }
+}
+
+template <int CL, int BN, int BF, int TA, int TB, int AB = GemmCfg<CL>::kABytes>
+__device__ __forceinline__ void tile_mainloop(float* acc, Ring& ring, int kb0, int kb1, int cw, int tid, int crank) {
+  const uint64_t da_hi = TA ? make_smem_desc_sw128(0, 8192, 1024) : make_smem_desc_sw128(0, 16, 1024);
+  const uint64_t db_hi = TB ? make_smem_desc_sw128(0, 8192, 1024) : make_smem_desc_sw128(0, 16, 1024);
+  constexpr uint32_t a_step = TA ? 128u : 2u, b_step = TB ? 128u : 2u;
+  int prev = -1;
+  for (int kb = kb0; kb < kb1; ++kb) {
+    mbar_wait(&ring.full[ring.stage], ring.phase);
+    const uint32_t sa = smem_u32(ring.base + ring.stage * ring.stage_bytes);
+    const uint64_t da = da_hi + (uint64_t)((sa + cw * 8192) >> 4);
+    const uint64_t db = db_hi + (uint64_t)((sa + AB) >> 4);
+    wgmma_fence();
+#pragma unroll
+    for (int k = 0; k < GEMM_BK / 16; ++k)
+      mma_cols<BN, 0, BF, TA, TB>(acc, da + k * a_step, db + k * b_step, (kb > kb0 || k > 0) ? 1u : 0u);
+    wgmma_commit();
+    wgmma_wait<1>();
+    if (prev >= 0) release_stage<CL>(ring, prev, tid, crank);
+    prev = ring.stage;
+    if (++ring.stage == ring.stages) {
+      ring.stage = 0;
+      ring.phase ^= 1;
+    }
+  }
+  wgmma_wait<0>();
+#pragma unroll
+  for (int i = 0; i < BN / 2; ++i) reg_fence(acc[i]);
+  if (prev >= 0) release_stage<CL>(ring, prev, tid, crank);
+}
+
+template <int CL, bool SPLIT, int BN, int AB = GemmCfg<CL>::kABytes>
+__device__ __forceinline__ void tile_mainloop_any(float* acc, Ring& ring, int bf, int a_mn, int b_mn, int kb0, int kb1, int cw, int tid,
+                                                  int crank) {
+  if constexpr (SPLIT) {
+    tile_mainloop<CL, BN, 0, 0, 0, AB>(acc, ring, kb0, kb1, cw, tid, crank);
+  } else {
+    if constexpr (CL == 1 && BN % 64 == 0) {
+      if (b_mn) {
+        if (bf) {
+          if (a_mn) tile_mainloop<CL, BN, 1, 1, 1, AB>(acc, ring, kb0, kb1, cw, tid, crank);
+          else tile_mainloop<CL, BN, 1, 0, 1, AB>(acc, ring, kb0, kb1, cw, tid, crank);
+        } else {
+          if (a_mn) tile_mainloop<CL, BN, 0, 1, 1, AB>(acc, ring, kb0, kb1, cw, tid, crank);
+          else tile_mainloop<CL, BN, 0, 0, 1, AB>(acc, ring, kb0, kb1, cw, tid, crank);
+        }
+        return;
+      }
+    }
+    if (bf) {
+      if (a_mn) tile_mainloop<CL, BN, 1, 1, 0, AB>(acc, ring, kb0, kb1, cw, tid, crank);
+      else tile_mainloop<CL, BN, 1, 0, 0, AB>(acc, ring, kb0, kb1, cw, tid, crank);
+    } else {
+      if (a_mn) tile_mainloop<CL, BN, 0, 1, 0, AB>(acc, ring, kb0, kb1, cw, tid, crank);
+      else tile_mainloop<CL, BN, 0, 0, 0, AB>(acc, ring, kb0, kb1, cw, tid, crank);
+    }
+  }
+}
+
+struct EpiRow {
+  bool valid;
+  float rsc;
+  const float* resid_row;
+  const float* aux_row;
+  const uint16_t* mask_row;
+  const float* add_row;
+  float* o32_row;
+  float* o32i_row;
+  uint16_t* o16_row;
+  uint16_t* o16p_row;
+  float* pre_row;
+  uint16_t* dact_row;
+};
+
+__device__ __forceinline__ void ld16f(const float* p, float (&v)[16]) {
+#pragma unroll
+  for (int q = 0; q < 4; ++q) {
+    const float4 t4 = reinterpret_cast<const float4*>(p)[q];
+    v[4 * q] = t4.x; v[4 * q + 1] = t4.y; v[4 * q + 2] = t4.z; v[4 * q + 3] = t4.w;
+  }
+}
+
+template <bool FULL, bool SPLIT>
+__device__ __forceinline__ void epi_step(const GemmProblem& pr, const EpiRow& r, float (&v)[16], int n0, bool active, int fmt, int lane,
+                                         long long lo16) {
+  const int pN = pr.N;
+  const int act = pr.act;
+  const int ofmt = pr.out_fmt < 0 ? fmt : pr.out_fmt;
+  const bool vec = FULL ? pr.vec_ok != 0 : true;
+  const bool atomic = (pr.accumulate != 0) || (pr.ksplit > 1);
+  const bool mask_mul = FULL && pr.mask_mul != 0;
+  const float rsc = r.rsc;
+  if (FULL && r.pre_row != nullptr && r.valid) {
+    if (vec) {
+      st_global_256f(r.pre_row + n0, v[0], v[1], v[2], v[3], v[4], v[5], v[6], v[7]);
+      st_global_256f(r.pre_row + n0 + 8, v[8], v[9], v[10], v[11], v[12], v[13], v[14], v[15]);
+    } else {
+#pragma unroll
+      for (int q = 0; q < 4; ++q)
+        if (n0 + 4 * q < pN)
+          *reinterpret_cast<float4*>(r.pre_row + n0 + 4 * q) = make_float4(v[4 * q], v[4 * q + 1], v[4 * q + 2], v[4 * q + 3]);
+    }
+  }
+  if (FULL && act == ACT_GELU && r.dact_row != nullptr) {
+    float dg[16];
+#pragma unroll
+    for (int j = 0; j < 16; ++j) {
+      float gj;
+      gelu_erf_both(v[j], gj, dg[j]);
+      v[j] = gj * rsc;
+    }
+    if (r.valid) {
+      if (vec) {
+        uint32_t w8[8];
+#pragma unroll
+        for (int q = 0; q < 8; ++q) w8[q] = cvt16x2(dg[2 * q], dg[2 * q + 1], ofmt);
+        st_global_256(r.dact_row + n0, w8);
+      } else {
+#pragma unroll
+        for (int j = 0; j < 16; ++j)
+          if (n0 + j < pN) r.dact_row[n0 + j] = cvt16(dg[j], ofmt);
+      }
+    }
+  } else if (act == ACT_GELU) {
+#pragma unroll
+    for (int j = 0; j < 16; ++j) v[j] = gelu_erf(v[j]) * rsc;
+  } else if (act == ACT_RELU) {
+#pragma unroll
+    for (int j = 0; j < 16; ++j) v[j] = fmaxf(v[j], 0.f) * rsc;
+  } else if (act == ACT_QUICKGELU) {
+#pragma unroll
+    for (int j = 0; j < 16; ++j) v[j] = v[j] / (1.f + expf(-1.702f * v[j])) * rsc;
+  } else {
+#pragma unroll
+    for (int j = 0; j < 16; ++j) v[j] *= rsc;
+  }
+  if (vec) {
+    if (r.valid) {
+      if (r.resid_row != nullptr) {
+        float rv[16];
+        ld16f(r.resid_row + n0, rv);
+#pragma unroll
+        for (int j = 0; j < 16; ++j) v[j] += rv[j];
+      }
+      if (FULL && r.aux_row != nullptr) {
+        float av[16];
+        ld16f(r.aux_row + n0, av);
+        if (pr.aux_mode == 1) {
+#pragma unroll
+          for (int j = 0; j < 16; ++j) v[j] *= gelu_erf_grad(av[j]);
+        } else {
+#pragma unroll
+          for (int j = 0; j < 16; ++j) v[j] *= av[j];
+        }
+      }
+      if (FULL && r.mask_row != nullptr) {
+#pragma unroll
+        for (int q = 0; q < 2; ++q) {
+          const uint4 mk = reinterpret_cast<const uint4*>(r.mask_row + n0)[q];
+          const uint32_t w4[4] = {mk.x, mk.y, mk.z, mk.w};
+#pragma unroll
+          for (int e = 0; e < 4; ++e) {
+            if (mask_mul) {
+              v[8 * q + 2 * e] *= ld16((uint16_t)(w4[e] & 0xffff), fmt);
+              v[8 * q + 2 * e + 1] *= ld16((uint16_t)(w4[e] >> 16), fmt);
+            } else {
+              if (!pos16((uint16_t)(w4[e] & 0xffff))) v[8 * q + 2 * e] = 0.f;
+              if (!pos16((uint16_t)(w4[e] >> 16))) v[8 * q + 2 * e + 1] = 0.f;
+            }
+          }
+        }
+      }
+      if (r.o32_row != nullptr) {
+        if (FULL && atomic) {
+#pragma unroll
+          for (int q = 0; q < 4; ++q)
+            red_add_f32x4(r.o32_row + n0 + 4 * q, make_float4(v[4 * q], v[4 * q + 1], v[4 * q + 2], v[4 * q + 3]));
+        } else {
+          st_global_256f(r.o32_row + n0, v[0], v[1], v[2], v[3], v[4], v[5], v[6], v[7]);
+          st_global_256f(r.o32_row + n0 + 8, v[8], v[9], v[10], v[11], v[12], v[13], v[14], v[15]);
+        }
+      }
+      if ((FULL || SPLIT) && r.o32i_row != nullptr) {
+        st_global_256f(r.o32i_row + n0, v[0], v[1], v[2], v[3], v[4], v[5], v[6], v[7]);
+        st_global_256f(r.o32i_row + n0 + 8, v[8], v[9], v[10], v[11], v[12], v[13], v[14], v[15]);
+      }
+      if (r.o16_row != nullptr) {
+        uint32_t w8[8];
+#pragma unroll
+        for (int q = 0; q < 8; ++q) w8[q] = cvt16x2(v[2 * q], v[2 * q + 1], ofmt);
+        st_global_256(r.o16_row + n0, w8);
+        if constexpr (SPLIT) {
+#pragma unroll
+          for (int q = 0; q < 8; ++q) w8[q] = cvt16x2_lo(v[2 * q], v[2 * q + 1]);
+          st_global_256(r.o16_row + lo16 + n0, w8);
+        }
+      }
+      if (r.o16p_row != nullptr) {
+        float p[16];
+#pragma unroll
+        for (int j = 0; j < 16; ++j) p[j] = v[j];
+        if (r.add_row != nullptr) {
+          float av[16];
+          ld16f(r.add_row + n0, av);
+#pragma unroll
+          for (int j = 0; j < 16; ++j) p[j] += av[j];
+        }
+        uint32_t w8[8];
+#pragma unroll
+        for (int q = 0; q < 8; ++q) w8[q] = cvt16x2(p[2 * q], p[2 * q + 1], ofmt);
+        st_global_256(r.o16p_row + n0, w8);
+        if constexpr (SPLIT) {
+#pragma unroll
+          for (int q = 0; q < 8; ++q) w8[q] = cvt16x2_lo(p[2 * q], p[2 * q + 1]);
+          st_global_256(r.o16p_row + lo16 + n0, w8);
+        }
+      }
+    } else {
+#pragma unroll
+      for (int j = 0; j < 16; ++j) v[j] = 0.f;
+    }
+  } else if constexpr (FULL) {
+    const int cs32 = pr.cs32 > 1 ? pr.cs32 : 1;
+#pragma unroll
+    for (int j = 0; j < 16; ++j) {
+      const int n = n0 + j;
+      float x = v[j];
+      if (r.valid && n < pN) {
+        if (r.resid_row != nullptr) x += r.resid_row[n];
+        if (r.aux_row != nullptr) x *= (pr.aux_mode == 1) ? gelu_erf_grad(r.aux_row[n]) : r.aux_row[n];
+        if (r.mask_row != nullptr) {
+          if (mask_mul) x *= ld16(r.mask_row[n], fmt);
+          else if (!pos16(r.mask_row[n])) x = 0.f;
+        }
+        if (r.o32_row != nullptr) {
+          float* dst = r.o32_row + (size_t)n * cs32;
+          if (atomic) atomicAdd(dst, x);
+          else *dst = x;
+        }
+        if (r.o32i_row != nullptr) r.o32i_row[n] = x;
+        if (r.o16_row != nullptr) {
+          r.o16_row[n] = cvt16(x, ofmt);
+          if constexpr (SPLIT) r.o16_row[lo16 + n] = cvt16_lo(x);
+        }
+        if (r.o16p_row != nullptr) {
+          const float xp = x + (r.add_row ? r.add_row[n] : 0.f);
+          r.o16p_row[n] = cvt16(xp, ofmt);
+          if constexpr (SPLIT) r.o16p_row[lo16 + n] = cvt16_lo(xp);
+        }
+      } else {
+        x = 0.f;
+      }
+      v[j] = x;
+    }
+  }
+  if (FULL && pr.colsum != nullptr) {
+    const float sj = halfwarp_colsum16(v, lane);
+    if (active && n0 + (lane & 15) < pN) atomicAdd(pr.colsum + n0 + (lane & 15), sj * pr.colsum_scale);
+  }
+}
+
+template <bool FULL, bool SPLIT, int BN>
+__device__ __forceinline__ void tile_epilogue(const GemmGroup& g, const GemmProblem& pr, const TileInfo& ti, const float* acc, float* ebuf,
+                                              int row0, int tid, int lane) {
+  const int fr = 16 * (tid >> 5) + (lane >> 2);
+  const int fc = 2 * (lane & 3);
+  const int erow = 16 * (tid >> 5) + (lane & 15), ehalf = lane >> 4;
+  const int fmt = g.fmt;
+  const int pM = pr.M, pN = pr.N, rps_in = pr.rps_in;
+  const int m = row0 + erow;
+  int b = 0, l = m;
+  if (rps_in > 0) {
+    b = m / rps_in;
+    l = m - b * rps_in;
+  }
+  const bool is_sep = (rps_in > 0) && (l == rps_in - 1);
+  EpiRow r;
+  r.valid = (m < pM) && !(pr.skip_sep && is_sep);
+  r.rsc = pr.alpha;
+  if (pr.row_scale != nullptr && m < pM) r.rsc *= pr.row_scale[b];
+  if (pr.zero_sep && is_sep) r.rsc = 0.f;
+  const size_t orow = (size_t)((rps_in > 0 ? b * pr.rps_out + l : m) + pr.row_off);
+  r.resid_row = pr.resid ? pr.resid + orow * pr.ld_resid : nullptr;
+  r.aux_row = (FULL && pr.aux32) ? pr.aux32 + orow * pr.ld_aux : nullptr;
+  r.mask_row = (FULL && pr.mask16) ? pr.mask16 + orow * pr.ld_mask : nullptr;
+  r.add_row = pr.addtab ? pr.addtab + (size_t)m * pr.ld_addtab : nullptr;
+  r.o32_row = pr.out32 ? pr.out32 + orow * pr.ld32 : nullptr;
+  r.o32i_row = ((FULL || SPLIT) && pr.out32_id) ? pr.out32_id + (size_t)m * pr.ld32_id : nullptr;
+  r.o16_row = pr.out16 ? pr.out16 + orow * pr.ld16 : nullptr;
+  r.o16p_row = pr.out16p ? pr.out16p + orow * pr.ld16 : nullptr;
+  r.pre_row = (FULL && pr.pre32) ? pr.pre32 + orow * pr.ld_pre : nullptr;
+  r.dact_row = (FULL && pr.dact16) ? pr.dact16 + orow * pr.ld_dact : nullptr;
+  const float* __restrict__ bias = (ti.split == 0) ? pr.bias : nullptr;
+  const int nt0 = ti.n_blk * BN;
+#pragma unroll 1
+  for (int cc = 0; cc < (BN + 31) / 32 && nt0 + cc * 32 < pN; ++cc) {
+#pragma unroll
+    for (int c = 0; c < (BN + 31) / 32; ++c) {
+      if (c == cc) {
+#pragma unroll
+        for (int ii = 0; ii < 4; ++ii) {
+          const int i = 4 * c + ii;
+          if (8 * i < BN) {
+            *reinterpret_cast<float2*>(ebuf + fr * GemmCfg<1>::kEpiStride + 8 * ii + fc) = make_float2(acc[4 * i], acc[4 * i + 1]);
+            *reinterpret_cast<float2*>(ebuf + (fr + 8) * GemmCfg<1>::kEpiStride + 8 * ii + fc) = make_float2(acc[4 * i + 2], acc[4 * i + 3]);
+          }
+        }
+      }
+    }
+    __syncwarp();
+    const int n0 = nt0 + cc * 32 + ehalf * 16;
+    const bool active = cc * 32 + ehalf * 16 < BN && n0 < pN;
+    float v[16];
+    ld16f(ebuf + erow * GemmCfg<1>::kEpiStride + ehalf * 16, v);
+    if (bias != nullptr) {
+#pragma unroll
+      for (int j = 0; j < 16; ++j) v[j] += (n0 + j < pN) ? __ldg(bias + n0 + j) : 0.f;
+    }
+    EpiRow ra = r;
+    ra.valid = r.valid && active;
+    epi_step<FULL, SPLIT>(pr, ra, v, n0, active, fmt, lane, g.lo16);
+    __syncwarp();
+  }
+}
+
+}
diff --git a/univtg_b200/csrc/gemm_pp.cu b/univtg_b200/csrc/gemm_pp.cu
--- /dev/null
+++ b/univtg_b200/csrc/gemm_pp.cu
@@ -0,0 +1,179 @@
+#include "gemm_common.cuh"
+
+namespace uv {
+
+struct PpCfg {
+  static constexpr int kABytes = 64 * 128;
+  static constexpr int kRingBytes = 5 * (kABytes + 256 * 128);
+  static constexpr int kEpiFloats = GemmCfg<1>::kEpiFloats;
+  static constexpr int kBarOff = kRingBytes + kEpiFloats * 4;
+  static constexpr int kTileCountOff = kBarOff + 2 * GemmCfg<1>::kMaxStages * 8;
+  static constexpr int kSmemBytes = 1024  + kBarOff + 256;
+  __host__ __device__ static constexpr int stage_bytes(int bn) { return kABytes + bn * 128; }
+  __host__ __device__ static constexpr int num_stages(int bn) {
+    return kRingBytes / stage_bytes(bn) < GemmCfg<1>::kMaxStages ? kRingBytes / stage_bytes(bn) : GemmCfg<1>::kMaxStages;
+  }
+};
+static_assert(PpCfg::kSmemBytes <= 227 * 1024, "ping-pong GEMM shared memory exceeds the sm_90 opt-in limit");
+
+constexpr int kOrderBar = 3;
+
+__device__ __forceinline__ int tile_kblocks(const GemmGroup& g, int bn, int t) {
+  TileInfo ti;
+  return decode_tile<1, false, 64>(g, bn, t, 0, ti) ? ti.kb1 - ti.kb0 : 0;
+}
+
+__device__ __forceinline__ int grid_ctas() {
+  int n;
+  asm volatile("mov.u32 %0, %%nctaid.x;" : "=r"(n));
+  return n;
+}
+
+__device__ __forceinline__ void ring_skip(Ring& ring, int n) {
+  ring.stage += n;
+  while (ring.stage >= ring.stages) {
+    ring.stage -= ring.stages;
+    ring.phase ^= 1u;
+  }
+}
+
+template <bool FULL, int BN>
+__device__ __forceinline__ void pingpong_tiles(const GemmGroup& g, uint8_t* smem, int cw, int lane) {
+  const int tid = threadIdx.x & 127;
+  uint64_t* bars = reinterpret_cast<uint64_t*>(smem + PpCfg::kBarOff);
+  Ring ring{smem, bars, bars + GemmCfg<1>::kMaxStages, PpCfg::stage_bytes(BN), PpCfg::num_stages(BN), 0, 0u};
+  float* ebuf = reinterpret_cast<float*>(smem + PpCfg::kRingBytes) + cw * 64 * GemmCfg<1>::kEpiStride;
+  float acc[BN / 2];
+#pragma unroll
+  for (int i = 0; i < BN / 2; ++i) acc[i] = 0.f;
+  TileInfo ti;
+  for (int t = blockIdx.x + cw * grid_ctas(); decode_tile<1, false, 64>(g, BN, t, 0, ti); t += 2 * grid_ctas()) {
+    const GemmProblem& pr = g.p[ti.p];
+    const int bf = pr.a_fmt < 0 ? g.fmt : pr.a_fmt;
+    if (t >= grid_ctas()) {
+      ring_skip(ring, tile_kblocks(g, BN, t - grid_ctas()));
+      named_bar_sync(kOrderBar + cw, 256);
+    }
+    if (t < grid_ctas() && cw == 0 && g.dbg != nullptr && ti.kb0 < ti.kb1) {
+      mbar_wait(&ring.full[ring.stage], ring.phase);
+      if (tid == 0) stamp(g.dbg, 3);
+    }
+    tile_mainloop_any<1, false, BN, PpCfg::kABytes>(acc, ring, bf, pr.a_mn, pr.b_mn, ti.kb0, ti.kb1, 0, tid, 0);
+    const int tiles = *reinterpret_cast<const int*>(smem + PpCfg::kTileCountOff);
+    if (t + grid_ctas() < tiles) named_bar_arrive(kOrderBar + (cw ^ 1), 256);
+    tile_epilogue<FULL, false, BN>(g, pr, ti, acc, ebuf, ti.m_blk * 64, tid, lane);
+  }
+}
+
+template <bool FULL>
+__global__ void __launch_bounds__(kGemmThreads, 1) gemm_pingpong_kernel(const __grid_constant__ GemmGroup g) {
+  const int BN = g.bn;
+  const int kStageBytes = PpCfg::stage_bytes(BN);
+  const int kStages = PpCfg::num_stages(BN);
+  extern __shared__ __align__(1024) uint8_t smem_raw[];
+  const uint32_t raw_addr = smem_u32(smem_raw);
+  const uint32_t align_off = (1024u - (raw_addr & 1023u)) & 1023u;
+  uint8_t* smem = smem_raw + align_off;
+
+  uint8_t* stage_base = smem;
+  uint64_t* full_bar = reinterpret_cast<uint64_t*>(smem + PpCfg::kBarOff);
+  uint64_t* empty_bar = full_bar + GemmCfg<1>::kMaxStages;
+
+  const int warp = threadIdx.x >> 5;
+  const int lane = threadIdx.x & 31;
+  const int wg = threadIdx.x >> 7;
+  if (threadIdx.x == 0) stamp(g.dbg, 0);
+
+  if (warp == 8 && lane == 0) {
+    for (int p = 0; p < g.num; ++p) {
+      tma_prefetch_desc(g.p[p].a_mn ? &g.p[p].tm_a : &g.p[p].tm_a64);
+      tma_prefetch_desc(&g.p[p].tm_b);
+    }
+  }
+  if (warp == 0 && lane == 0) {
+    for (int s = 0; s < kStages; ++s) {
+      mbar_init(&full_bar[s], 1);
+      mbar_init(&empty_bar[s], 1);
+    }
+    fence_barrier_init();
+    int total = 0;
+    for (int p = 0; p < g.num; ++p) total += ((g.p[p].M + 63) / 64) * ((g.p[p].N + BN - 1) / BN) * g.p[p].ksplit;
+    *reinterpret_cast<int*>(smem + PpCfg::kTileCountOff) = total;
+  }
+  __syncthreads();
+  pdl_launch_dependents();
+  pdl_wait();
+  if (threadIdx.x == 0) stamp(g.dbg, 1);
+
+  if (wg == 2) {
+    setmaxnreg_dec<40>();
+    if (warp == 8) {
+      int stage = 0;
+      uint32_t phase = 0;
+      TileInfo ti;
+      for (int t = blockIdx.x; decode_tile<1, false, 64>(g, BN, t, 0, ti); t += gridDim.x) {
+        const GemmProblem& pr = g.p[ti.p];
+        const int m0 = ti.m_blk * 64;
+        const int n0 = ti.n_blk * BN;
+        for (int kb = ti.kb0; kb < ti.kb1; ++kb) {
+          const int tap = kb / pr.kblk_per_tap;
+          const int kk = (kb - tap * pr.kblk_per_tap) * GEMM_BK;
+          mbar_wait(&empty_bar[stage], phase ^ 1);
+          uint8_t* sa = stage_base + stage * kStageBytes;
+          uint8_t* sb = sa + PpCfg::kABytes;
+          const int a0 = pr.ca.base0 + m0 * pr.ca.mn0s + tap * pr.ca.tap0 + kk * pr.ca.k0s;
+          const int a1 = pr.ca.base1 + m0 * pr.ca.mn1s + tap * pr.ca.tap1 + kk * pr.ca.k1s;
+          const int b0 = pr.cb.base0 + n0 * pr.cb.mn0s + tap * pr.cb.tap0 + kk * pr.cb.k0s;
+          const int b1 = pr.cb.base1 + n0 * pr.cb.mn1s + tap * pr.cb.tap1 + kk * pr.cb.k1s;
+          if (elect_one()) {
+            mbar_arrive_expect_tx(&full_bar[stage], PpCfg::kABytes + BN * 128);
+            tma_load_2d(sa, pr.a_mn ? &pr.tm_a : &pr.tm_a64, &full_bar[stage], a0, a1);
+            if (!pr.b_mn) {
+              tma_load_2d(sb, &pr.tm_b, &full_bar[stage], b0, b1);
+            } else if (pr.b_3d) {
+              tma_load_3d(sb, &pr.tm_b, &full_bar[stage], 0, b1, b0 >> 6);
+            } else {
+              for (int j = 0; j < BN / 64; ++j) tma_load_2d(sb + j * 8192, &pr.tm_b, &full_bar[stage], b0 + 64 * j, b1);
+            }
+          }
+          __syncwarp();
+          if (++stage == kStages) {
+            stage = 0;
+            phase ^= 1;
+          }
+        }
+      }
+      if (lane == 0) stamp(g.dbg, 2);
+    }
+  } else {
+    setmaxnreg_inc<232>();
+    switch (BN >> 4) {
+#define UV_BN_CASE(k) \
+  case k: pingpong_tiles<FULL, 16 * k>(g, smem, wg, lane); break;
+      UV_BN_CASE(2) UV_BN_CASE(3) UV_BN_CASE(4) UV_BN_CASE(5) UV_BN_CASE(6) UV_BN_CASE(7) UV_BN_CASE(8) UV_BN_CASE(9) UV_BN_CASE(10)
+      UV_BN_CASE(11) UV_BN_CASE(12) UV_BN_CASE(13) UV_BN_CASE(14) UV_BN_CASE(15)
+      case 16: if constexpr (!FULL || 256 <= kPingPongFullMaxBn) pingpong_tiles<FULL, 256>(g, smem, wg, lane); break;
+#undef UV_BN_CASE
+      default: __trap();
+    }
+  }
+
+  __syncthreads();
+  if (threadIdx.x == 0) stamp(g.dbg, 7);
+}
+
+cudaError_t launch_gemm_pingpong(const GemmGroup& g, int grid, bool full, cudaStream_t stream) {
+  static bool attr_set = false;
+  if (!attr_set) {
+    cudaError_t e = cudaFuncSetAttribute(gemm_pingpong_kernel<true>, cudaFuncAttributeMaxDynamicSharedMemorySize, PpCfg::kSmemBytes);
+    if (e == cudaSuccess)
+      e = cudaFuncSetAttribute(gemm_pingpong_kernel<false>, cudaFuncAttributeMaxDynamicSharedMemorySize, PpCfg::kSmemBytes);
+    if (e != cudaSuccess) return e;
+    attr_set = true;
+  }
+  if (full) launch_k(gemm_pingpong_kernel<true>, dim3(grid), dim3(kGemmThreads), PpCfg::kSmemBytes, stream, g);
+  else launch_k(gemm_pingpong_kernel<false>, dim3(grid), dim3(kGemmThreads), PpCfg::kSmemBytes, stream, g);
+  return cudaGetLastError();
+}
+
+}
diff --git a/univtg_b200/csrc/kernels.h b/univtg_b200/csrc/kernels.h
--- a/univtg_b200/csrc/kernels.h
+++ b/univtg_b200/csrc/kernels.h
@@ -20,6 +20,7 @@
 struct GemmProblem {
   CUtensorMap tm_a;
   CUtensorMap tm_b;
+  CUtensorMap tm_a64;
   OperandCoord ca, cb;
   int a_mn, b_mn;
   int b_box_rows;
@@ -64,6 +65,9 @@
   int cs32;
   int skip_sep;
   int b_3d;
+  int a64;
+  const void* b_base;
+  uint64_t b_rows, b_cols, b_ld;
   int vec_ok;
 };
 
@@ -79,6 +83,10 @@
 };
 
 int launch_gemm_group(GemmGroup& g, int bn, int num_sms, cudaStream_t stream, int* used_full = nullptr);
+int set_gemm_schedule(int mode);
+void last_gemm_schedule(int* schedule, int* bn);
+constexpr int kPingPongFullMaxBn = 240;
+cudaError_t launch_gemm_pingpong(const GemmGroup& g, int grid, bool full, cudaStream_t stream);
 struct TileChoice {
   int bn, ksplit;
 };
diff --git a/univtg_b200/csrc/plan.h b/univtg_b200/csrc/plan.h
--- a/univtg_b200/csrc/plan.h
+++ b/univtg_b200/csrc/plan.h
@@ -456,6 +456,19 @@
   return lo ? make_tmap_split(m, base, rows, cols, ld, box_rows, box_cols, (uint64_t)lo) : make_tmap_2d(m, base, rows, cols, ld, box_rows, box_cols);
 }
 
+inline int set_a64(GemmProblem& p, const void* base, uint64_t rows, uint64_t cols, uint64_t ld) {
+  const int rc = make_tmap_2d(&p.tm_a64, base, rows, cols, ld, 64, 64);
+  p.a64 = rc == 0;
+  return rc;
+}
+
+inline void set_b_desc(GemmProblem& p, const void* base, uint64_t rows, uint64_t cols, uint64_t ld) {
+  p.b_base = base;
+  p.b_rows = rows;
+  p.b_cols = cols;
+  p.b_ld = ld;
+}
+
 int setup_gemm(GemmProblem& p, Mat16 A, int a_mn, Mat16 B, int b_mn, int M, int N, int K, int bn, long long lo_a = 0,
                long long lo_b = 0) {
   init_problem(p);
@@ -471,10 +484,12 @@
   int rc = 0;
   if (!a_mn) {
     rc |= make_tmap_op(&p.tm_a, A.p, (uint64_t)A.rows, (uint64_t)A.cols, (uint64_t)A.ld, GEMM_BM, 64, lo_a);
+    if (!lo_a) rc |= set_a64(p, A.p, (uint64_t)A.rows, (uint64_t)A.cols, (uint64_t)A.ld);
   } else {
     rc |= make_tmap_2d(&p.tm_a, A.p, (uint64_t)A.rows, (uint64_t)A.cols, (uint64_t)A.ld, 64, 64);
     p.ca = OperandCoord{0, 1, 0, 0, 0, 0, 0, 1};
   }
+  if (!lo_b) set_b_desc(p, B.p, (uint64_t)B.rows, (uint64_t)B.cols, (uint64_t)B.ld);
   if (!b_mn) {
     rc |= make_tmap_op(&p.tm_b, B.p, (uint64_t)B.rows, (uint64_t)B.cols, (uint64_t)B.ld, (uint32_t)bn, 64, lo_b);
     p.b_box_rows = bn;
@@ -495,7 +510,9 @@
   p.ca = OperandCoord{0, 0, 0, 1, 0, 1, 1, 0};
   p.cb = OperandCoord{0, 0, Cin, 1, 0, 1, 0, 0};
   int r = make_tmap_op(&p.tm_a, X, (uint64_t)Mh + 2, (uint64_t)Cin, (uint64_t)lda, GEMM_BM, 64, lo_a);
+  if (!lo_a) r |= set_a64(p, X, (uint64_t)Mh + 2, (uint64_t)Cin, (uint64_t)lda);
   r |= make_tmap_op(&p.tm_b, Wp, (uint64_t)N, (uint64_t)3 * Cin, (uint64_t)3 * Cin, (uint32_t)bn, 64, lo_b);
+  if (!lo_b) set_b_desc(p, Wp, (uint64_t)N, (uint64_t)3 * Cin, (uint64_t)3 * Cin);
   p.b_box_rows = bn;
   return r;
 }
@@ -510,7 +527,9 @@
   p.ca = OperandCoord{0, 0, 0, 1, 0, 1, 1, 0};
   p.cb = OperandCoord{2 * Cin, 1, -Cin, 0, 0, 0, 0, 1};
   int r = make_tmap_2d(&p.tm_a, dY, (uint64_t)Mh + 2, (uint64_t)Kc, (uint64_t)ldy, GEMM_BM, 64);
+  r |= set_a64(p, dY, (uint64_t)Mh + 2, (uint64_t)Kc, (uint64_t)ldy);
   r |= make_tmap_b_mn(p, Wp, (uint64_t)Kc, (uint64_t)3 * Cin, (uint64_t)3 * Cin, bn);
+  set_b_desc(p, Wp, (uint64_t)Kc, (uint64_t)3 * Cin, (uint64_t)3 * Cin);
   return r;
 }
 int conv_wgrad_problem(GemmProblem& p, int Mh, const uint16_t* dY, int ldy, int Nc, const uint16_t* X, int ldx, int Cin, int t, int bn) {
@@ -524,6 +543,7 @@
   p.cb = OperandCoord{0, 1, 0, 0, t, 0, 0, 1};
   int r = make_tmap_2d(&p.tm_a, dY, (uint64_t)Mh + 2, (uint64_t)Nc, (uint64_t)ldy, 64, 64);
   r |= make_tmap_b_mn(p, X, (uint64_t)Mh + 2, (uint64_t)Cin, (uint64_t)ldx, bn);
+  set_b_desc(p, X, (uint64_t)Mh + 2, (uint64_t)Cin, (uint64_t)ldx);
   return r;
 }
 
diff --git a/univtg_b200/csrc/ptx.cuh b/univtg_b200/csrc/ptx.cuh
--- a/univtg_b200/csrc/ptx.cuh
+++ b/univtg_b200/csrc/ptx.cuh
@@ -121,6 +121,7 @@
   asm volatile("setmaxnreg.dec.sync.aligned.u32 %0;" ::"n"(kRegs));
 }
 UV_DEVINL void named_bar_sync(int id, int count) { asm volatile("bar.sync %0, %1;" ::"r"(id), "r"(count) : "memory"); }
+UV_DEVINL void named_bar_arrive(int id, int count) { asm volatile("bar.arrive %0, %1;" ::"r"(id), "r"(count) : "memory"); }
 
 UV_DEVINL uint64_t make_smem_desc_sw128(uint32_t smem_addr, uint32_t lbo_bytes, uint32_t sbo_bytes) {
   uint64_t d = 0;
@@ -155,7 +156,7 @@
 UV_DEVINL void red_add_f32x4(float* addr, float4 v) {
   asm volatile("red.global.add.v4.f32 [%0], {%1, %2, %3, %4};" ::"l"(addr), "f"(v.x), "f"(v.y), "f"(v.z), "f"(v.w) : "memory");
 }
-UV_DEVINL float warp_colsum16(float (&v)[16], int lane) {
+UV_DEVINL float halfwarp_colsum16(float (&v)[16], int lane) {
 #pragma unroll
   for (int off = 8; off >= 1; off >>= 1) {
     const bool hi = (lane & off) != 0;
@@ -166,7 +167,7 @@
       v[k] = keep + __shfl_xor_sync(0xffffffffu, send, off);
     }
   }
-  return v[0] + __shfl_xor_sync(0xffffffffu, v[0], 16);
+  return v[0];
 }
 UV_DEVINL float warp_max(float v) {
 #pragma unroll
```

Measured after the change: 6520 (median of 6 runs). 2.3% higher.
